# qiskit-community/aqc-research

Hardware: AMD Instinct MI355X
Metric: objective+gradient evals/sec (higher is better)
Workload: dtype f64; 1 GPU; 16-qubit, 40-block cx spin ansatz, state-vector objective+gradient; n_qubits=16, num_thetas=208, gate_groups=56, batch_per_gpu=1024, columns=1, transport=none, records_gathered=1024, launcher=none

## Files before the change

aqc_research_amd/_lib.py:

```python
import ctypes
import os
from ctypes import POINTER, c_char_p, c_double, c_float, c_int, c_int32, c_int64, c_uint8, c_void_p

import numpy as np

_HERE = os.path.dirname(os.path.abspath(__file__))
LIB_PATH = os.environ.get("AQC_HIP_LIB", os.path.join(_HERE, "libaqc_hip.so"))

BUF_Y, BUF_Z, BUF_X, BUF_W, BUF_ZW, BUF_X2 = range(6)
K_APPLY, K_SWEEP, K_COEF, K_FINALIZE, K_MISC, K_SWEEP_LIST, K_APPLY_LIST, K_PROJECT, K_SWEEP_VIRTUAL, K_APPLY_VIRTUAL = range(10)
ENTANGLERS = {"cx": 0, "cz": 1, "cp": 2}

_P = c_void_p
_D = POINTER(c_double)

SIGNATURES = {
    "aqc_version": (c_char_p, []),
    "aqc_last_error": (c_char_p, []),
    "aqc_device_count": (c_int, []),
    "aqc_live_buffers": (c_int, [POINTER(c_int64), POINTER(c_int64)]),
    "aqc_create": (c_int, [c_int, c_int, POINTER(c_int32), c_int, c_int, c_int, POINTER(_P)]),
    "aqc_destroy": (c_int, [_P]),
    "aqc_num_thetas": (c_int, [_P]),
    "aqc_num_gate_groups": (c_int, [_P]),
    "aqc_v_mul_vec": (c_int, [_P, _D, _D, _D]),
    "aqc_vdag_mul_vec": (c_int, [_P, _D, _D, _D]),
    "aqc_grad_dot_vec": (c_int, [_P, _D, _D, _D, c_int, c_int, c_int, _D]),
    "aqc_v_mul_mat": (c_int, [_P, _D, _D, c_int]),
    "aqc_vdag_mul_mat": (c_int, [_P, _D, _D, c_int]),
    "aqc_grad_dot_mat": (c_int, [_P, _D, _D, _D, c_int, _D]),
    "aqc_ws_create": (c_int, [_P, c_int, c_int, c_int, c_int, c_int, POINTER(_P)]),
    "aqc_ws_destroy": (c_int, [_P]),
    "aqc_ws_set_thetas": (c_int, [_P, _D]),
    "aqc_ws_upload": (c_int, [_P, c_int, _D]),
    "aqc_ws_upload_lane": (c_int, [_P, c_int, c_int, _D]),
    "aqc_ws_broadcast": (c_int, [_P, c_int, _D]),
    "aqc_ws_download": (c_int, [_P, c_int, _D]),
    "aqc_ws_download_lane": (c_int, [_P, c_int, c_int, _D]),
    "aqc_ws_copy_lane": (c_int, [_P, c_int, c_int, _P, c_int, c_int]),
    "aqc_ws_set_basis": (c_int, [_P, c_int, POINTER(c_int64)]),
    "aqc_ws_set_combo": (c_int, [_P, c_int, POINTER(c_int64), _D]),
    "aqc_ws_set_identity": (c_int, [_P, c_int]),
    "aqc_ws_apply": (c_int, [_P, c_int, c_int, c_int]),
    "aqc_ws_grad": (c_int, [_P, c_int, c_int, c_int]),
    "aqc_ws_get_grads": (c_int, [_P, _D]),
    "aqc_ws_gather": (c_int, [_P, c_int, POINTER(c_int64), c_int, _D]),
    "aqc_ws_vdot": (c_int, [_P, c_int, c_int, _D]),
    "aqc_ws_sync": (c_int, [_P]),
    "aqc_ws_eval": (c_int, [_P, _P, c_int, _P, c_int, c_int, c_int, c_int, _P]),
    "aqc_ws_grad_from": (c_int, [_P, c_int, c_int, c_int, c_int]),
    "aqc_ws_cd_sweep": (c_int, [_P, _D, _D]),
    "aqc_ws_cd_sweeps": (c_int, [_P, _D, _D, c_int, c_int]),
    "aqc_ws_cd_fits_one_launch": (c_int, [_P]),
    "aqc_ws_cd_minimize": (c_int, [_P, _D, c_int, c_int, c_double, c_double, c_double, c_int, c_int, _D, _D, POINTER(c_int64), POINTER(c_int32),
                           _D]),
    "aqc_zgemm": (c_int, [c_int, c_int, c_int, c_int, c_int, _D, c_int, _D, c_int, _D, c_int]),
    "aqc_gate_1q": (c_int, [c_int, c_int, c_int64, c_int, _D, _D, _D]),
    "aqc_gate_2q": (c_int, [c_int, c_int, c_int64, c_int, c_int, _D, _D, _D]),
    "aqc_xxz_mul_vec": (c_int, [c_int, c_int, c_int, c_double, _D, _D]),
    "aqc_xxz_energy": (c_int, [c_int, c_int, c_int, c_double, _D, _D]),
    "aqc_xxz_evolve": (c_int, [c_int, c_int, c_int, c_int, c_double, _D, _D, _D, POINTER(c_int32)]),
    "aqc_obs_plan": (c_int, [c_int, c_int, POINTER(c_int32), c_int, c_int] + [POINTER(c_int32)] * 6),
    "aqc_obs_rdm": (c_int, [c_int, c_int, c_int, _D, c_int, c_int, POINTER(c_int32), _D]),
    "aqc_mps_create": (c_int, [c_int, c_int, POINTER(c_int32), _D, _D, POINTER(_P)]),
    "aqc_mps_destroy": (c_int, [_P]),
    "aqc_mps_clone": (c_int, [_P, POINTER(_P)]),
    "aqc_mps_num_qubits": (c_int, [_P]),
    "aqc_mps_dims": (c_int, [_P, POINTER(c_int32)]),
    "aqc_mps_discarded_weight": (c_double, [_P]),
    "aqc_mps_export": (c_int, [_P, _D, _D]),
    "aqc_mps_gate1": (c_int, [_P, c_int, _D]),
    "aqc_mps_gate2": (c_int, [_P, c_int, c_int, _D, c_double, c_int]),
    "aqc_mps_dot": (c_int, [_P, _P, _D]),
    "aqc_mps_dot_ops": (c_int, [_P, _P, c_int, POINTER(c_int32), _D, _D]),
    "aqc_svd": (c_int, [c_int, c_int, c_int, _D, _D, _D, _D, POINTER(c_int)]),
    "aqc_svd_batch": (c_int, [c_int, c_int, c_int, c_int, POINTER(c_int32), POINTER(c_int32), _D, _D, _D, _D, POINTER(c_int32), POINTER(c_int32)]),
    "aqc_svd_batch_core_ms": (c_double, []),
    "aqc_mps_apply_circuit": (c_int, [_P, _P, _D, c_int, c_double, c_int]),
    "aqc_mps_fast_dot_gradient": (c_int, [_P, _P, _P, _D, c_double, c_int, c_int, c_int, c_int, _D]),
    "aqc_mpsb_create": (c_int, [c_int, c_int, c_int, POINTER(_P)]),
    "aqc_mpsb_destroy": (c_int, [_P]),
    "aqc_mpsb_gate2_stats": (c_int, [_P, c_int, _D, c_int]),
    "aqc_mpsb_set_targets": (c_int, [_P, POINTER(_P), c_int]),
    "aqc_mpsb_set_lhs": (c_int, [_P, POINTER(_P), c_int]),
    "aqc_mpsb_eval": (c_int, [_P, _P, _D, c_double, c_int, c_int, c_int, c_int, _D, _D, _D, POINTER(c_int32)]),
    "aqc_mpsb_set_lhs_basis": (c_int, [_P, POINTER(c_uint8)]),
    "aqc_mpsb_vh": (c_int, [_P, _P, _D, c_double, c_int, c_int, c_int, _D, _D, POINTER(c_int32)]),
    "aqc_mpsb_grad": (c_int, [_P, _P, c_int, c_int, c_int, _D]),
    "aqc_mpsb_set_bank": (c_int, [_P, POINTER(_P), c_int]),
    "aqc_mpsb_vh_bank": (c_int, [_P, _P, _D, c_double, c_int, c_int, c_int, _D, _D, POINTER(c_int32)]),
    "aqc_mpsb_gradient_of": (c_int, [_P, _P, _D, c_double, c_int, c_int, c_int, c_int, _D]),
    "aqc_mpsb_apply_circuit": (c_int, [_P, _P, _D, c_int, c_double, c_int, _D, POINTER(c_int32)]),
    "aqc_mpsb_export": (c_int, [_P, c_int, POINTER(_P)]),
    "aqc_mps_device": (c_int, [_P]),
    "aqc_gate_dot": (c_int, [c_int, c_int, c_int64, c_int, c_int, c_int, _D, _D, _D]),
    "aqc_ws_mps_upload": (c_int, [_P, c_int, POINTER(c_int32), _D, _D]),
    "aqc_ws_mps_to_vec": (c_int, [_P, c_int, c_int, c_int]),
    "aqc_ws_mps_to_vec_batch": (c_int, [_P, c_int, POINTER(c_int32), c_int, POINTER(c_int32)]),
    "aqc_ws_mps_dot": (c_int, [_P, c_int, c_int, _D]),
    "aqc_ws_theta_bank": (c_int, [_P, _D, c_int]),
    "aqc_ws_use_theta_set": (c_int, [_P, c_int]),
    "aqc_ws_gather_setup": (c_int, [_P, POINTER(c_int64), c_int]),
    "aqc_ws_gather_launch": (c_int, [_P, c_int]),
    "aqc_ws_gather_fetch": (c_int, [_P, _D]),
    "aqc_ws_vdot_launch": (c_int, [_P, c_int, c_int]),
    "aqc_ws_vdot_fetch": (c_int, [_P, _D]),
    "aqc_ws_results_async": (c_int, [_P]),
    "aqc_ws_objective_launch": (c_int, [_P, c_int, c_int, c_int, c_int]),
    "aqc_ws_results_fetch": (c_int, [_P, _D, _D]),
    "aqc_ws_timer_start": (c_int, [_P]),
    "aqc_ws_timer_stop": (c_int, [_P, POINTER(c_float)]),
    "aqc_ws_profile_enable": (c_int, [_P, c_int]),
    "aqc_ws_profile_get": (c_int, [_P, c_int, POINTER(c_int64), POINTER(c_double)]),
    "aqc_ws_profile_reset": (c_int, [_P]),
    "aqc_ws_profile_log": (c_int, [_P, POINTER(c_int32), _D, c_int, POINTER(c_int)]),
    "aqc_ws_plan_stage": (c_int, [_P, c_int, c_int, POINTER(c_int), POINTER(c_int), POINTER(c_int)]),
    "aqc_ws_sparse_counts": (c_int, [_P, POINTER(c_int64)]),
    "aqc_ws_projected_info": (c_int, [_P, POINTER(c_int32)]),
    "aqc_plan_projected": (c_int, [_P, c_int, c_int, POINTER(c_int32)]),
    "aqc_switch_info": (c_int, [c_int] + [POINTER(c_char_p)] * 5),
    "aqc_ws_switch": (c_int, [_P, c_char_p, POINTER(c_int64)]),
    "aqc_ws_plan_skips": (c_int, [_P, c_int, c_int, POINTER(c_int), c_int]),
    "aqc_ws_sweep_r_only_sub": (c_int, [_P]),
    "aqc_ws_plan_info": (c_int, [_P, c_int, POINTER(c_int), POINTER(c_int), POINTER(c_int)]),
    "aqc_ws_kernel_family": (c_int, [_P, c_int]),
    "aqc_ws_plan_substages": (c_int, [_P, c_int]),
    "aqc_ws_lbfgs": (c_int, [_P, _D, c_int, c_int, c_double, c_double, c_double, c_int, c_int, c_int, c_int, _D, _D, _D, POINTER(c_int64),
                     POINTER(c_int64), _D, POINTER(c_int64)]),
    "aqc_ws_lbfgs_mat": (c_int, [_P, _D, c_int, c_int, c_double, c_double, c_double, c_double, c_int, _D, _D, _D, POINTER(c_int64),
                         POINTER(c_int64), POINTER(c_int32)]),
    "aqc_ws_surrogate_eval": (c_int, [_P, _D, c_int, _D, POINTER(c_int64), c_int, c_int, c_int, _D, _D, _D, _D, _D]),
    "aqc_qr": (c_int, [c_int, c_int, c_int, _D, _D, POINTER(c_int32)]),
    "aqc_ws_sketch_target": (c_int, [_P, _D, c_int]),
    "aqc_ws_sketch_generate": (c_int, [_P, c_int, ctypes.c_uint64, c_int64, POINTER(c_int32), _D, POINTER(c_int32)]),
    "aqc_ws_sketch_draw": (c_int, [_P, c_int, ctypes.c_uint64, c_int64, c_int]),
    "aqc_ws_sketch_adam": (c_int, [_P, c_int, _D, c_int, _D, c_double, c_double, c_double, c_double, ctypes.c_uint64, c_int64, POINTER(c_int32),
                           POINTER(c_int32), _D, _D, _D, _D, POINTER(c_int64), POINTER(c_int32)]),
    "aqc_comm_unique_id": (c_int, [ctypes.c_char_p]),
    "aqc_comm_create": (c_int, [ctypes.c_char_p, c_int, c_int, c_int, POINTER(_P)]),
    "aqc_comm_destroy": (c_int, [_P]),
    "aqc_comm_rank": (c_int, [_P]),
    "aqc_comm_size": (c_int, [_P]),
    "aqc_comm_allgather": (c_int, [_P, _D, _D, ctypes.c_size_t]),
    "aqc_comm_allreduce": (c_int, [_P, _D, ctypes.c_size_t, c_int]),
    "aqc_comm_barrier": (c_int, [_P]),
    "aqc_plan_substages": (c_int, [_P, c_int, c_int, c_int, c_int, c_int, POINTER(c_int), POINTER(c_int), c_int]),
    "aqc_plan_query": (
        c_int,
        [_P, c_int, c_int, c_int, c_int, c_int, POINTER(c_int), POINTER(c_int), POINTER(c_int), POINTER(c_int), POINTER(c_int)],
    ),
}

_lib = None


def lib() -> ctypes.CDLL:
    global _lib
    if _lib is None:
        if not os.path.exists(LIB_PATH):
            raise RuntimeError(
                f"{LIB_PATH} not found: build it with `make -C aqc_research_amd/csrc` "
                "(or __graft_entry__.build()); this package has no CPU fallback"
            )
        handle = ctypes.CDLL(LIB_PATH)
        for name, (res, args) in SIGNATURES.items():
            fn = getattr(handle, name)
            fn.restype, fn.argtypes = res, args
        _lib = handle
    return _lib


LANES_REFUSED = 3
SKETCH_KINDS = {"rand": 0, "alt": 1, "eigen": 2}
QR_RANK_DEFICIENT = 1
CD_STATUS = {1: "normal", 2: "early", 3: "timeout"}
CD_ROUTES = {"auto": 0, "persistent": 1, "wide": 2}


class LanesRefused(RuntimeError):
    """The lockstep lanes of the MPS engine cannot do this call (a bond beyond their limit, a lane gone bad, no memory for them) and
    returned nothing; the single-lane engine may.  What callers that have such a route catch in order to take it."""


def check(status: int) -> None:
    if status != 0:
        kind = LanesRefused if status == LANES_REFUSED else RuntimeError
        raise kind("aqc_hip: " + lib().aqc_last_error().decode("utf-8", "replace"))


def dptr(arr: np.ndarray):
    return arr.ctypes.data_as(_D)


def as_c128(a, shape=None, name="array") -> np.ndarray:
    a = np.ascontiguousarray(a, dtype=np.complex128)
    if shape is not None and a.shape != tuple(shape):
        raise ValueError(f"{name}: expected shape {tuple(shape)}, got {a.shape}")
    return a


def as_f64(a, size=None, name="array") -> np.ndarray:
    a = np.ascontiguousarray(a, dtype=np.float64)
    if size is not None and a.size != size:
        raise ValueError(f"{name}: expected {size} values, got {a.size}")
    return a
```

aqc_research_amd/csrc/aqc_api.cpp:

```cpp
#include "aqc_ws.h"

using namespace aqc;

namespace {
thread_local std::string g_error;
}

namespace aqc {

int fail(const char* fmt, ...) {
    char buf[1024];
    va_list ap;
    va_start(ap, fmt);
    vsnprintf(buf, sizeof buf, fmt, ap);
    va_end(ap);
    g_error = buf;
    return 1;
}
int set_error(const std::string& msg) { g_error = msg; return 1; }

int check_buf(const aqc_ws* ws, int buf) {
    if (!ws) return fail("null workspace");
    if (buf < 0 || buf >= AQC_NUM_BUFS) return fail("invalid buffer id %d", buf);
    return 0;
}

int check_block_range(const aqc_ws* ws, int block_from, int block_to) {
    const int nb = ws->ctx->prog.num_blocks;
    if (block_from < 0 || nb == 0) return 0;
    if (!(block_from < block_to && block_to <= nb)) return fail("invalid block_range [%d, %d)", block_from, block_to);
    return 0;
}

int ensure_coef(aqc_ws* ws) {
    if (ws->coef_valid) return 0;
    return fail("thetas have not been uploaded (aqc_ws_set_thetas)");
}

int copy_in(aqc_ws* ws, double2* dst, const double* src, size_t rows) {
    if (ws->pitch == ws->ncols) {
        HIP_OK(hipMemcpyAsync(dst, src, rows * ws->ncols * sizeof(double2), hipMemcpyHostToDevice, ws->stream));
    } else {
        HIP_OK(hipMemsetAsync(dst, 0, rows * ws->pitch * sizeof(double2), ws->stream));
        HIP_OK(hipMemcpy2DAsync(dst, (size_t)ws->pitch * sizeof(double2), src, (size_t)ws->ncols * sizeof(double2),
                                (size_t)ws->ncols * sizeof(double2), rows, hipMemcpyHostToDevice, ws->stream));
    }
    HIP_OK(hipStreamSynchronize(ws->stream));
    return 0;
}
int copy_out(aqc_ws* ws, double* dst, const double2* src, size_t rows) {
    if (ws->pitch == ws->ncols) {
        HIP_OK(hipMemcpyAsync(dst, src, rows * ws->ncols * sizeof(double2), hipMemcpyDeviceToHost, ws->stream));
    } else {
        HIP_OK(hipMemcpy2DAsync(dst, (size_t)ws->ncols * sizeof(double2), src, (size_t)ws->pitch * sizeof(double2),
                                (size_t)ws->ncols * sizeof(double2), rows, hipMemcpyDeviceToHost, ws->stream));
    }
    HIP_OK(hipStreamSynchronize(ws->stream));
    return 0;
}

int results_guard(aqc_ws* ws) {
    if (ws->copy_pending && !ws->capturing) {
        HIP_OK(hipStreamWaitEvent(ws->stream, ws->ev_copied, 0));
        ws->copy_pending = false;
    }
    return 0;
}


}

extern "C" {

const char* aqc_version(void) { return "aqc_hip 0.1.0 (gfx950)"; }
const char* aqc_last_error(void) { return g_error.c_str(); }

int aqc_live_buffers(int64_t* device, int64_t* pinned) {
    if (device) *device = g_live_device.load();
    if (pinned) *pinned = g_live_pinned.load();
    return 0;
}

int aqc_device_count(void) {
    int ndev = 0;
    return hipGetDeviceCount(&ndev) == hipSuccess ? ndev : 0;
}

int aqc_create(int num_qubits, int entangler, const int32_t* blocks, int num_blocks, int trotter, int second_order,
               aqc_ctx** out) {
    if (!out) return fail("out pointer is null");
    *out = nullptr;
    aqc_ctx* ctx = new aqc_ctx();
    const std::string err = build_program(num_qubits, entangler, blocks, num_blocks, trotter != 0, second_order != 0, ctx->prog);
    if (!err.empty()) {
        delete ctx;
        return fail("%s", err.c_str());
    }
    *out = ctx;
    return 0;
}

int aqc_destroy(aqc_ctx* ctx) {
    if (!ctx) return 0;
    for (auto& kv : ctx->oneshot) aqc_ws_destroy(kv.second);
    delete ctx;
    return 0;
}

int aqc_num_thetas(const aqc_ctx* ctx) { return ctx ? ctx->prog.num_thetas() : -1; }
int aqc_num_gate_groups(const aqc_ctx* ctx) { return ctx ? (int)ctx->prog.groups.size() : -1; }

int aqc_plan_query(aqc_ctx* ctx, int ncols, int which, int tile_bits, int low_bits, int stage, int* num_stages,
                   int* bits_out, int* num_bits, int* ops_out, int* num_ops) {
    if (!ctx) return fail("null context");
    if (ncols < 1) return fail("ncols must be positive");
    const int col_bits = ceil_log2(ncols);
    if (tile_bits <= 0) tile_bits = which == 1 ? 12 : 13;
    if (low_bits < 0) low_bits = 3;
    Plan plan = make_plan(ctx->prog, col_bits, tile_bits, low_bits, which == 0);
    if (which == 3) {
        split_substages(ctx->prog, plan, 4, 1 << 20);
        plan = mirror_plan(plan);
    }
    const std::string err = check_plan(ctx->prog, plan);
    if (!err.empty()) return fail("planner produced an invalid plan: %s", err.c_str());
    if (num_stages) *num_stages = (int)plan.stages.size();
    if (stage >= 0) {
        if (stage >= (int)plan.stages.size()) return fail("stage index out of range");
        const Stage& st = plan.stages[stage];
        if (num_bits) *num_bits = (int)st.bits.size();
        if (num_ops) *num_ops = (int)st.ops.size();
        if (bits_out) for (size_t i = 0; i < st.bits.size(); ++i) bits_out[i] = st.bits[i];
        if (ops_out) for (size_t i = 0; i < st.ops.size(); ++i) ops_out[i] = st.ops[i];
    }
    return 0;
}

int aqc_plan_projected(aqc_ctx* ctx, int tile_bits, int low_bits, int32_t* info) {
    if (!ctx || !info) return fail("null argument");
    if (tile_bits <= 0) tile_bits = 12;
    if (low_bits < 0) low_bits = 3;
    const Program& prog = ctx->prog;
    tile_bits = std::min(std::max(tile_bits, 8), std::min(12, prog.n));
    aqc_ws tmp;
    tmp.ctx = ctx;
    tmp.ncols = 1; tmp.col_bits = 0; tmp.nbits = prog.n;
    Plan best = make_plan(prog, 0, tile_bits, low_bits, false);
    for (int lb = low_bits - 1; lb >= 2; --lb) {
        Plan cand = make_plan(prog, 0, tile_bits, lb, false);
        if (cand.stages.size() < best.stages.size()) best = cand;
    }
    lower_plan(prog, best, tmp.sweep, 4, true, true);
    tmp.sw = read_switches();
    tmp.sw.sparse_sweep = 1;
    tmp.inv_mirrored = tmp.sweep.v3 && tmp.sweep.plan.stages.size() >= 2;
    proj_plan(&tmp, low_bits);
    const int rc = aqc_ws_projected_info(&tmp, info);
    tmp.ctx = nullptr;
    return rc;
}

int aqc_plan_substages(aqc_ctx* ctx, int ncols, int which, int tile_bits, int low_bits, int stage, int* num_subs, int* subs_out, int max_subs) {
    if (!ctx || !num_subs) return fail("null argument");
    if (ncols < 1) return fail("ncols must be positive");
    const int col_bits = ceil_log2(ncols);
    if (tile_bits <= 0) tile_bits = 12;
    if (low_bits < 0) low_bits = 3;
    Plan plan = make_plan(ctx->prog, col_bits, tile_bits, low_bits, which == 0);
    split_substages(ctx->prog, plan, 4, 1 << 20);
    if (which == 3) plan = mirror_plan(plan);
    const std::string err = check_plan(ctx->prog, plan);
    if (!err.empty()) return fail("planner produced an invalid plan: %s", err.c_str());
    if (stage < 0 || stage >= (int)plan.stages.size()) return fail("stage index out of range");
    const Stage& st = plan.stages[stage];
    *num_subs = (int)st.subs.size();
    if (subs_out)
        for (int i = 0; i < (int)st.subs.size() && i < max_subs; ++i) {
            for (int j = 0; j < 4; ++j) subs_out[5 * i + j] = j < (int)st.subs[i].bits.size() ? st.subs[i].bits[j] : -1;
            subs_out[5 * i + 4] = (int)st.subs[i].ops.size();
        }
    return 0;
}


static int ws_decide(aqc_ws* ws, int tile_bits_apply, int tile_bits_sweep) {
    aqc_ctx* ctx = ws->ctx;
    const Program& prog = ctx->prog;
    const int batch = ws->batch;
    const Switches& sw = ws->sw = read_switches();
    const int low_bits = (int)sw.low_bits;
    int ka = tile_bits_apply > 0 ? tile_bits_apply : (int)sw.tile_bits_apply;
    int ks = tile_bits_sweep > 0 ? tile_bits_sweep : (int)sw.tile_bits_sweep;
    const int family = (int)sw.kernel_family;
    if (family < 0 || family > 3) return fail("AQC_KERNEL_FAMILY must be 1 (per-group), 2 (register-blocked) or 3 (matrix cores)");
    const bool want_v3 = (family == 3 || family == 0) && ws->nbits >= 8;
    const int force_v2 = family == 3 ? 0 : (family ? family - 1 : -1);
    const size_t big_tiles = (size_t)batch << std::max(0, ws->nbits - 12);
    const bool want_v2 = force_v2 >= 0 ? force_v2 != 0 : big_tiles >= 512;
    auto pick = [&](int kmax) {
        if (want_v3) {
            int k = std::min(12, ws->nbits);
            while (k > 10 && ((size_t)batch << (ws->nbits - k)) < 256) --k;
            const int kmin = std::max(8, prog.n + std::min(ws->col_bits, 3));
            while (ws->col_bits > 0 && k > kmin && ((size_t)batch << (ws->nbits - k)) < 256) --k;
            return k;
        }
        if (want_v2) return std::min(kmax, ws->nbits);
        int k = std::min(11, ws->nbits);
        while (k > 10 && ((size_t)batch << (ws->nbits - k)) < 512) --k;
        return k;
    };
    if (ka <= 0) ka = pick(13);
    if (ks <= 0) ks = pick(12);
    ka = std::min(std::min(ka, 13), ws->nbits);
    ks = std::min(std::min(ks, 12), ws->nbits);
    ws->threads = (int)sw.threads;
    if (ws->threads <= 0) ws->threads = std::min(256, std::max(64, 1 << (std::min(ka, ks) - 2)));
    if (ws->threads < 64 || ws->threads > 512 || ws->threads % 64) return fail("AQC_THREADS must be a multiple of 64 in [64, 512]");

    auto best_plan = [&](int k, bool inverse) {
        Plan best = make_plan(prog, ws->col_bits, k, low_bits, inverse);
        for (int lb = low_bits - 1; lb >= 2; --lb) {
            Plan cand = make_plan(prog, ws->col_bits, k, lb, inverse);
            if (cand.stages.size() < best.stages.size()) best = cand;
        }
        return best;
    };
    if (want_v3) { ka = std::min(std::max(ka, 8), 12); ks = std::max(ks, 8); }
    auto cached = [&](const std::vector<int>& key, DevPlan& out, const std::function<void(HostPlan&)>& lower) {
        std::lock_guard<std::recursive_mutex> lock(ctx->mu);
        auto it = ctx->plan_cache.find(key);
        if (it == ctx->plan_cache.end()) {
            HostPlan fresh;
            lower(fresh);
            it = ctx->plan_cache.emplace(key, std::move(fresh)).first;
        }
        out = it->second;
    };
    auto cached_plan = [&](int which, int k, bool inverse, int reg_bits, bool dots, DevPlan& out) {
        cached({which, ws->col_bits, k, low_bits, reg_bits, (int)dots, (int)want_v3}, out,
               [&](HostPlan& fresh) { lower_plan(prog, best_plan(k, inverse), fresh, reg_bits, dots, want_v3); });
    };
    cached_plan(2, ka, false, (want_v2 || want_v3) ? 4 : 0, false, ws->fwd);
    cached_plan(1, ks, false, want_v3 ? 4 : (want_v2 ? (sw.sweep_reg_bits == 3 ? 3 : 4) : 0), true, ws->sweep);
    ws->inv_mirrored = want_v3 && ka == ks && ws->sweep.v3 && ws->sweep.plan.stages.size() >= 2 && sw.mirror_plan != 0;
    if (ws->inv_mirrored)
        cached({3, ws->col_bits, ks, low_bits, 4, 0, 1}, ws->inv,
               [&](HostPlan& fresh) { lower_plan(prog, mirror_plan(ws->sweep.plan), fresh, 4, false, true, true); });
    else
        cached_plan(0, ka, true, (want_v2 || want_v3) ? 4 : 0, false, ws->inv);
    for (DevPlan* p : {&ws->fwd, &ws->inv, &ws->sweep}) {
        const std::string err = check_plan(prog, p->plan);
        if (!err.empty()) return fail("planner produced an invalid plan: %s", err.c_str());
    }
    proj_plan(ws, low_bits);
    if (sw.verbose && want_v3)
        fprintf(stderr, "aqc_hip: matrix-core kernels, tiles 2^%d (V / V^H, %d workgroups per CU) / 2^%d (sweep, %d per CU), sub-stages %zu / %zu / %zu\n",
                ws->inv.k, mfma_occupancy(ws->inv.k, false), ws->sweep.k, mfma_occupancy(ws->sweep.k, true), ws->fwd.h_subs3.size(),
                ws->inv.h_subs3.size(), ws->sweep.h_subs3.size());
    return 0;
}

struct SlotTables {
    std::vector<int> theta_slots, slot_theta, slot_ntiles;
    int partial_tiles = 1;
};
static SlotTables ws_slot_tables(aqc_ws* ws) {
    const Program& prog = ws->ctx->prog;
    const int T = prog.num_thetas();
    const int G = (int)prog.groups.size();
    ws->nslots = G * kSlotsPerGroup;
    SlotTables t;
    t.partial_tiles = ws->sweep.v3 ? 1 : ws->sweep.ntiles;
    t.theta_slots.assign(2 * (size_t)std::max(T, 1), -1);
    t.slot_ntiles.assign((size_t)std::max(ws->nslots, 1), t.partial_tiles);
    auto feed = [&](int theta, int slot) {
        if (t.theta_slots[2 * theta] < 0) t.theta_slots[2 * theta] = slot; else t.theta_slots[2 * theta + 1] = slot;
    };
    for (int gi = 0; gi < G; ++gi) {
        const GateGroup& g = prog.groups[gi];
        if (g.type == GROUP_FRONT) {
            feed(g.theta0 + 2, gi * kSlotsPerGroup + 0);
            feed(g.theta0 + 1, gi * kSlotsPerGroup + 1);
            feed(g.theta0 + 0, gi * kSlotsPerGroup + 2);
        } else {
            for (int d = 0; d < prog.tpb; ++d) feed(g.theta0 + d, gi * kSlotsPerGroup + d);
        }
    }
    t.slot_theta.assign((size_t)std::max(ws->nslots, 1), -1);
    ws->grads_direct = ws->sweep.v3 && T > 0 && ws->sw.grads_direct != 0;
    for (int th = 0; th < T; ++th) {
        if (t.theta_slots[2 * th] < 0 || t.theta_slots[2 * th + 1] >= 0) { ws->grads_direct = false; break; }
        t.slot_theta[t.theta_slots[2 * th]] = th;
    }
    return t;
}

static int ws_upload_ujobs(aqc_ws* ws) {
    const Program& prog = ws->ctx->prog;
    std::vector<UJob> jobs, route_jobs;
    size_t n_vdag_sweep = 0;
    DevPlan* vsw = ws->proj.ok ? &ws->proj.vsw : nullptr;
    const int nsw = ws->sweep.v3 ? (int)ws->sweep.h_subs3.size() : 0;
    ws->ujobs_mirror = ws->inv_mirrored && ws->inv.v3 && (int)ws->inv.h_subs3.size() == nsw && ws->sw.ubuild_mirror != 0;
    for (DevPlan* p : {&ws->inv, &ws->sweep, vsw, &ws->fwd})
        if (p && p->v3)
            for (size_t i = 0; i < p->h_subs3.size(); ++i) {
                if (p == &ws->inv && ws->ujobs_mirror) continue;
                UJob j{p->d_subs3 + i, p->d_grps, p->d_umat, (int)i, (int)p->h_subs3.size(), p->plan.inverse ? 1 : 0, prog.entangler, nullptr, 0, 0};
                if (p == &ws->sweep && ws->ujobs_mirror) { j.umat_mirror = ws->inv.d_umat; j.mirror_index = nsw - 1 - (int)i; j.mirror_nsubs = nsw; }
// ... 618 lines not shown
```

aqc_research_amd/csrc/aqc_kernels3.hip:

```cpp
#include <hip/hip_runtime.h>

#include <cstring>

#include <type_traits>

#include "aqc_device.h"
#include "aqc_launch.h"
#include "aqc_math.h"

namespace aqc {

typedef double double4_t __attribute__((ext_vector_type(4)));

__host__ __device__ __forceinline__ unsigned swz3(unsigned l) { return l ^ ((l >> 4) & 15u) ^ ((l >> 8) & 15u); }

__device__ __forceinline__ double4_t mfma(double a, double b, double4_t c) {
    return __builtin_amdgcn_mfma_f64_16x16x4f64(a, b, c, 0, 0, 0);
}

struct Acc3 { double4_t k1, k2, k3; };
__device__ __forceinline__ void u_mfma(const cplx (&v)[4], const double (&u0)[4], const double (&u1)[4], const double (&u2)[4], Acc3& t) {
    t.k1 = double4_t{0.0, 0.0, 0.0, 0.0}; t.k2 = t.k1; t.k3 = t.k1;
#pragma unroll
    for (int s = 0; s < 4; ++s) {
        t.k1 = mfma(v[s].x + v[s].y, u0[s], t.k1);
        t.k2 = mfma(v[s].x, u1[s], t.k2);
        t.k3 = mfma(v[s].y, u2[s], t.k3);
    }
}
__device__ __forceinline__ void u_combine(const Acc3& t, cplx (&o)[4]) {
#pragma unroll
    for (int r = 0; r < 4; ++r) {
        o[r].x = t.k1[r] - t.k3[r];
        o[r].y = t.k1[r] + t.k2[r];
    }
}

#ifdef AQC_TUNING
#define AQC_STAMP(slot) do { if (a.stamps && threadIdx.x == 0 && (slot) < kStampSlots) \
    a.stamps[((size_t)blockIdx.y * gridDim.x + blockIdx.x) * kStampSlots + (slot)] = __builtin_amdgcn_s_memtime(); } while (0)
#ifdef AQC_TUNING_NODBG
#define AQC_DBG_AND(x)
#define AQC_DBG_TEST(x) false
#else
#define AQC_DBG_AND(x) && (x)
#define AQC_DBG_TEST(x) (x)
#endif
#else
#define AQC_STAMP(slot) do { } while (0)
#define AQC_DBG_AND(x)
#define AQC_DBG_TEST(x) false
#endif

__host__ __device__ constexpr bool sweep_scratch_double(int k) { return k >= 12 || k <= 9; }
#ifndef AQC_SWEEP_SPREAD
#define AQC_SWEEP_SPREAD 1
#endif
#ifndef AQC_APPLY_SPREAD
#define AQC_APPLY_SPREAD 1
#endif
#ifndef AQC_EXP_APPLY_SKIP
#define AQC_EXP_APPLY_SKIP 0
#endif
constexpr int kApplySkip = AQC_EXP_APPLY_SKIP;
#ifndef AQC_EXP_SWEEP_SKIP
#define AQC_EXP_SWEEP_SKIP 0
#endif
constexpr int kSweepSkip = AQC_EXP_SWEEP_SKIP;
#ifndef AQC_EXP_UBUILD_SKIP
#define AQC_EXP_UBUILD_SKIP 0
#endif
constexpr int kUbuildSkip = AQC_EXP_UBUILD_SKIP;

constexpr int kSweepSpread = AQC_SWEEP_SPREAD, kApplySpread = AQC_APPLY_SPREAD;
template <int K, bool SWEEP = false> struct TileShape {
    static constexpr int kSweepWaves12 = 4;
    static constexpr int kWaves = (SWEEP && K == 12) ? kSweepWaves12 : (K >= 10 ? 4 : (1 << (K - 8)));
    static constexpr int kGroups = 1 << (K - 8);
    static constexpr int kGpw = kGroups / kWaves;
    static constexpr int kLoads = (1 << (K - 6)) / kWaves;
};

struct SubRegs {
    double u0[4], u1[4], u2[4];
    unsigned lane12;
};

template <int GPW>
__device__ __forceinline__ void fetch_sub(SubRegs& x, const DevSub3* subs, const double* umat, int sub_index, int lane, int wave,
                                          int nwaves) {
    const DevSub3* sub = subs + sub_index;
    const double* up = umat + (size_t)sub_index * 12 * 64;
#pragma unroll
    for (int s = 0; s < 4; ++s) {
        x.u0[s] = up[(0 * 4 + s) * 64 + lane];
        x.u1[s] = up[(1 * 4 + s) * 64 + lane];
        x.u2[s] = up[(2 * 4 + s) * 64 + lane];
    }
    x.lane12 = sub->lane12[lane];
}

template <int GPW>
struct SubAddr {
    unsigned a1, a2;
    unsigned k1[GPW][4], k2[GPW][4];
};
typedef unsigned uint8v_t __attribute__((ext_vector_type(8)));
template <int GPW>
__device__ __forceinline__ void fetch_k(SubAddr<GPW>& x, const DevSub3* subs, int sub_index, int wave, int nwaves) {
#pragma unroll
    for (int j = 0; j < GPW; ++j) {
        const uint8v_t kv = *reinterpret_cast<const __attribute__((address_space(4))) uint8v_t*>(
            (const __attribute__((address_space(4))) void*)(const void*)&subs[sub_index].kk[wave + j * nwaves][0]);
#pragma unroll
        for (int s = 0; s < 4; ++s) { x.k1[j][s] = kv[s]; x.k2[j][s] = kv[4 + s]; }
    }
}
template <int GPW>
__device__ __forceinline__ void sub_addr(SubAddr<GPW>& x, const SubRegs& c, unsigned lds_base) {
    x.a1 = ((c.lane12 & 0xffffu) << 4) + lds_base;
    x.a2 = ((c.lane12 >> 16) << 4) + lds_base;
}
typedef double dbl2_t __attribute__((ext_vector_type(2)));
typedef __attribute__((address_space(3))) dbl2_t* lds_cplx_ptr;
__device__ __forceinline__ cplx lds_get(unsigned addr) {
    const dbl2_t v = *reinterpret_cast<lds_cplx_ptr>(addr);
    return make_double2(v.x, v.y);
}
__device__ __forceinline__ void lds_put(unsigned addr, cplx v) { *reinterpret_cast<lds_cplx_ptr>(addr) = dbl2_t{v.x, v.y}; }
__device__ __forceinline__ unsigned lds_address(const void* p) {
    return (unsigned)reinterpret_cast<size_t>((__attribute__((address_space(3))) const char*)p);
}

__device__ __forceinline__ const void* uniform_ptr(const void* p) {
    const unsigned long long v = (unsigned long long)p;
    const unsigned lo = __builtin_amdgcn_readfirstlane((unsigned)v), hi = __builtin_amdgcn_readfirstlane((unsigned)(v >> 32));
    return (const void*)(((unsigned long long)hi << 32) | lo);
}

template <int K, int NV>
__device__ __forceinline__ void load_tiles3(cplx* t0, cplx* t1, const cplx* s0, const cplx* s1, const DevStage& st, unsigned lo, int wave) {
    constexpr int NL = TileShape<K, NV == 2>::kLoads, NW = TileShape<K, NV == 2>::kWaves;
    cplx v0[NL], v1[NL];
#pragma unroll
    for (int i = 0; i < NL; ++i) {
        const unsigned off = lo + st.dhi[wave + i * NW];
        v0[i] = s0[off];
        if (NV == 2) v1[i] = s1[off];
    }
#pragma unroll
    for (int i = 0; i < NL; ++i) {
        const unsigned slot = swz3((unsigned)((wave + i * NW) << 6) | (threadIdx.x & 63u));
        t0[slot] = v0[i];
        if (NV == 2) t1[slot] = v1[i];
    }
}
template <int K, bool SWEEP>
__device__ __forceinline__ void store_tile3(const cplx* tile, cplx* dst, const DevStage& st, unsigned lo, int wave) {
    constexpr int NL = TileShape<K, SWEEP>::kLoads, NW = TileShape<K, SWEEP>::kWaves;
#pragma unroll
    for (int i = 0; i < NL; ++i) {
        const unsigned slot = swz3((unsigned)((wave + i * NW) << 6) | (threadIdx.x & 63u));
        dst[lo + st.dhi[wave + i * NW]] = tile[slot];
    }
}
__device__ __forceinline__ size_t tile_base3(const DevStage& st, unsigned tile) {
    size_t base = 0;
    for (int i0 = 0; i0 < st.nub; i0 += 4) {
        int ub[4];
#pragma unroll
        for (int u = 0; u < 4; ++u) ub[u] = st.ubits[i0 + u];
#pragma unroll
        for (int u = 0; u < 4; ++u)
            if (i0 + u < st.nub) base |= (size_t)((tile >> (i0 + u)) & 1u) << ub[u];
    }
    return base;
}

__device__ __forceinline__ int uniform_load(const int* p) { return __builtin_amdgcn_readfirstlane(*p); }
struct ItemAt { int bl, tile, slot; };
template <bool LIST>
__device__ __forceinline__ ItemAt item_at(const Stage3Args& a, int wi) {
    if (LIST) {
        const TileItem* it = a.items + wi;
        return ItemAt{uniform_load(&it->lane), uniform_load(&it->tile), uniform_load(&it->slot)};
    }
    const int bl = wi / a.ntiles;
    return ItemAt{bl, wi - bl * a.ntiles, 0};
}
template <int K, bool LIST, bool PAIR = false>
__device__ __forceinline__ void apply_mfma_body(const Stage3Args& a0, const Stage3Args& b0, const int wg, const int nwg) {
    using TS = TileShape<K>;
    static_assert(!PAIR || (LIST && K >= 12), "the pair form walks two lists with persistent workgroups");
    extern __shared__ __attribute__((aligned(16))) char smem[];
    const Stage3Args* ca = &a0;
#define a (*ca)
#define st (ca->stage)
    cplx* tw = reinterpret_cast<cplx*>(smem);
    const unsigned lds_base = lds_address(smem);
    if (lds_base & ((16u << K) - 1)) __builtin_trap();
    const int lane = threadIdx.x & 63;
    const int wave = __builtin_amdgcn_readfirstlane((int)(threadIdx.x >> 6));
    constexpr int NL = TS::kLoads, NW = TS::kWaves;
    constexpr bool kPersist = K >= 12;
    int nwork = LIST ? uniform_load(a.nitems) : a.ntiles * a.batch;
    bool second = false;
    if (PAIR && wg >= nwork) { ca = &b0; second = true; nwork = uniform_load(b0.nitems); }
    unsigned lo = st.dlo[lane];
    unsigned lo16 = lo << 4;
    (void)lo16;
    SubRegs cur, nxt;
    SubAddr<TS::kGpw> ad;
    dbl2_t pw[NL];
    int wi = wg + ((kPersist || LIST) ? 0 : (int)blockIdx.y * a.ntiles);
    if (LIST && wi >= nwork) return;
    ItemAt it = item_at<LIST>(a, wi);
    {
        const int bl = it.bl;
        if (st.nsubs > 0) {
            fetch_sub<TS::kGpw>(cur, a.subs, a.umat + (size_t)bl * a.nsubs_total * 12 * 64, st.sub_begin, lane, wave, NW);
            fetch_k<TS::kGpw>(ad, a.subs, st.sub_begin, wave, NW);
        }
        AQC_STAMP(0);
        if (!(kApplySkip & 64)) load_tiles3<K, 1>(tw, nullptr, a.in0 + (size_t)bl * a.lane_stride + tile_base3(st, it.tile), nullptr, st, lo, wave);
    }
    __builtin_amdgcn_s_waitcnt(0x0F70);
    AQC_STAMP(1);
    for (;;) {
    const int bl = it.bl;
    const size_t lane_off = (size_t)bl * a.lane_stride + tile_base3(st, it.tile);
    const double* umat = a.umat + (size_t)bl * a.nsubs_total * 12 * 64;
    int nwi = wi + nwg;
    bool more = kPersist && st.nsubs > 0 && nwi < nwork;
    const Stage3Args* na = ca;
    int nnwork = nwork;
    if (PAIR && !more && !second) {
        na = &b0; nwi = wg; nnwork = uniform_load(b0.nitems);
        more = nwi < nnwork;
    }
    const bool change = PAIR && na != ca;
    const ItemAt nit = more ? item_at<LIST>(*na, nwi) : ItemAt{0, 0, 0};
    const int nbl = nit.bl;
    const size_t next_off = more ? (size_t)nbl * na->lane_stride + tile_base3(na->stage, nit.tile) : 0;
    const unsigned nlo = change ? na->stage.dlo[lane] : lo;
    const unsigned nlo16 = nlo << 4;
    for (int si = 0; si < st.nsubs; ++si) {
        AQC_STAMP(4 + si);
        if (!(kApplySkip & 512)) __syncthreads();
        if (si + 1 < st.nsubs) fetch_sub<TS::kGpw>(nxt, a.subs, umat, st.sub_begin + si + 1, lane, wave, NW);
        else if (more) fetch_sub<TS::kGpw>(nxt, na->subs, na->umat + (size_t)nbl * na->nsubs_total * 12 * 64, na->stage.sub_begin, lane, wave, NW);
        if (kPersist && more && !(kApplySkip & 64)) {
#pragma unroll
            for (int c = 0; c < 4; ++c) {
                if (si == (c < st.nsubs ? c : st.nsubs - 1)) {
#pragma unroll
                    for (int i = c * (NL / 4); i < (c + 1) * (NL / 4); ++i) {
                        const size_t ub = next_off + na->stage.dhi[wave + i * NW];
                        asm volatile("s_nop 4\n\tglobal_load_dwordx4 %0, %1, %2" : "=a"(pw[i]) : "v"(nlo16), "s"(uniform_ptr(na->in0 + ub)) : "memory");
                    }
                }
            }
        }
        sub_addr(ad, cur, lds_base);
        cplx v[2][4];
        Acc3 acc;
#pragma unroll
        for (int s = 0; s < 4; ++s) v[0][s] = lds_get(ad.a1 ^ ad.k1[0][s]);
#pragma unroll
        for (int j = 0; j <= TS::kGpw; ++j) {
            if (j + 1 < TS::kGpw && !(kApplySkip & 2)) {
#pragma unroll
                for (int s = 0; s < 4; ++s) v[(j + 1) & 1][s] = lds_get((kApplySkip & 32) ? ad.a1 : (ad.a1 ^ ad.k1[j + 1][s]));
            }
            __builtin_amdgcn_sched_barrier(0);
            double sv[4];
            cplx o[4];
            if (j < TS::kGpw) {
#pragma unroll
                for (int s = 0; s < 4; ++s) sv[s] = (kApplySkip & (16 | 128)) ? v[j & 1][s].x : v[j & 1][s].x + v[j & 1][s].y;
            }
            if (j > 0) {
                if (kApplySkip & (16 | 256)) {
#pragma unroll
                    for (int r = 0; r < 4; ++r) o[r] = make_double2(acc.k1[r], acc.k2[r]);
                } else u_combine(acc, o);
            }
            unsigned wa[4];
            if (j < TS::kGpw) {
#pragma unroll
                for (int s = 0; s < 4; ++s) asm volatile("" : "+v"(sv[s]));
            }
            if (j > 0) {
#pragma unroll
                for (int r = 0; r < 4; ++r) { wa[r] = (kApplySkip & 32) ? ad.a2 : (ad.a2 ^ ad.k2[j - 1][r]); asm volatile("" : "+v"(wa[r])); }
            }
            __builtin_amdgcn_sched_barrier(0);
            if (j < TS::kGpw) {
                acc.k1 = double4_t{0.0, 0.0, 0.0, 0.0}; acc.k2 = acc.k1; acc.k3 = acc.k1;
#pragma unroll
                for (int s = 0; s < 4; ++s) {
                    if (kApplySkip & 8) continue;
                    acc.k1 = mfma(sv[s], cur.u0[s], acc.k1);
                    acc.k2 = mfma(v[j & 1][s].x, cur.u1[s], acc.k2);
                    acc.k3 = mfma(v[j & 1][s].y, cur.u2[s], acc.k3);
                }
            }
            if (j > 0 && !(kApplySkip & 1)) {
#pragma unroll
                for (int r = 0; r < 4; ++r) lds_put(wa[r], o[r]);
                if (j < TS::kGpw) {
#pragma unroll
                    for (int i = 0; i < 4; ++i) {
                        __builtin_amdgcn_sched_group_barrier(0x008, kApplySpread, 0);
                        __builtin_amdgcn_sched_group_barrier(0x200, 1, 0);
                    }
                }
            }
            __builtin_amdgcn_sched_barrier(0);
        }
        if (si + 1 < st.nsubs || more) {
            cur = nxt;
            if (si + 1 < st.nsubs) fetch_k<TS::kGpw>(ad, a.subs, st.sub_begin + si + 1, wave, NW);
            else fetch_k<TS::kGpw>(ad, na->subs, na->stage.sub_begin, wave, NW);
        }
    }
    AQC_STAMP(4 + st.nsubs);
    __syncthreads();
    AQC_STAMP(2);
    if (!(kApplySkip & 64)) store_tile3<K, false>(tw, a.out0 + lane_off, st, lo, wave);
    AQC_STAMP(3);
    if (!more) break;
    __syncthreads();
    __builtin_amdgcn_s_waitcnt(0x0F70);
#pragma unroll
    for (int i = 0; i < NL; ++i) {
        const unsigned slot = swz3((unsigned)((wave + i * NW) << 6) | (threadIdx.x & 63u));
        asm volatile("ds_write_b128 %0, %1" : : "v"(lds_base + (slot << 4)), "a"(pw[i]) : "memory");
    }
    __builtin_amdgcn_s_waitcnt(0xC07F);
    wi = nwi;
    it = nit;
    if (PAIR) { ca = na; second = second || change; nwork = nnwork; lo = nlo; lo16 = nlo16; }
    }
#undef a
#undef st
}
template <int K, bool LIST = false>
__global__ __launch_bounds__(TileShape<K>::kWaves * 64, 2) void apply_mfma_kernel(const Stage3Args a) {
    apply_mfma_body<K, LIST>(a, a, (int)blockIdx.x, (int)gridDim.x);
}
#ifndef AQC_PAIR_PLAIN_BOUNDARY
#define AQC_PAIR_PLAIN_BOUNDARY 0
#endif
template <int K>
__global__ __launch_bounds__(TileShape<K>::kWaves * 64, 2) void apply_pair_kernel(const Stage3Args a, const Stage3Args b, const int grid_a) {
    if constexpr (K >= 12 && !AQC_PAIR_PLAIN_BOUNDARY) {
        static_assert(sizeof(Stage3Args) % 8 == 0 && alignof(Stage3Args) == 8, "b follows a in the kernel-argument segment without padding");
        const __attribute__((address_space(4))) char* kp = (const __attribute__((address_space(4))) char*)__builtin_amdgcn_kernarg_segment_ptr();
        const Stage3Args* pa = (const Stage3Args*)(const void*)kp;
        const Stage3Args* pb = (const Stage3Args*)(const void*)(kp + sizeof(Stage3Args));
        apply_mfma_body<K, true, true>(*pa, *pb, (int)blockIdx.x, (int)gridDim.x);
    } else if (K >= 12) {
        apply_mfma_body<K, true>(a, a, (int)blockIdx.x, (int)gridDim.x);
        __syncthreads();
        apply_mfma_body<K, true>(b, b, (int)blockIdx.x, (int)gridDim.x);
    } else if ((int)blockIdx.x < grid_a) {
        apply_mfma_body<K, true>(a, a, (int)blockIdx.x, grid_a);
    } else {
        apply_mfma_body<K, true>(b, b, (int)blockIdx.x - grid_a, (int)gridDim.x - grid_a);
    }
}

template <int N>
__device__ __forceinline__ void wait_prefetched(dbl2_t (&pw)[N], dbl2_t (&pz)[N]) {
    asm volatile("s_waitcnt vmcnt(0)" : : : "memory");
#pragma unroll
    for (int i = 0; i < N; ++i) asm volatile("" : "+a"(pw[i]), "+a"(pz[i]));
}
__device__ __forceinline__ unsigned tile_offset3(const DevStage& st, unsigned local) { return st.dlo[local & 63u] | st.dhi[local >> 6]; }
template <int K> struct SweepShape : TileShape<K, true> {};
__device__ __forceinline__ unsigned elem_bit(const DevStage& st, long long e, unsigned local_pos) {
    const unsigned m = local_pos < 6 ? st.dlo[1u << local_pos] : st.dhi[1u << (local_pos - 6)];
    return ((unsigned long long)e & m) ? 1u : 0u;
}
template <int GPW, int NW>
__device__ __forceinline__ void skip_masks(const DevStage& st, unsigned info, long long e0, long long e1, int wave, unsigned& nzmask, unsigned& kneed) {
    nzmask = 0; kneed = 0;
    const unsigned gfresh = info & 15u, kfresh = (info >> 6) & 3u;
#pragma unroll
    for (int k = 0; k < 2; ++k) {
        const long long e = k ? e1 : e0;
        if (e < 0) continue;
        unsigned gb = 0;
#pragma unroll
        for (int i = 0; i < 4; ++i)
            if (gfresh >> i & 1) gb |= elem_bit(st, e, (info >> (8 + 4 * i)) & 15u) << i;
        unsigned kb = 0;
        if (kfresh & 1) kb |= elem_bit(st, e, (info >> 24) & 15u);
        if (kfresh & 2) kb |= elem_bit(st, e, (info >> 28) & 15u) << 1;
#pragma unroll
        for (int j = 0; j < GPW; ++j)
            if ((((unsigned)(wave + j * NW) ^ gb) & gfresh) == 0) nzmask |= 1u << j;
#pragma unroll
        for (unsigned s2 = 0; s2 < 4; ++s2)
            if (((s2 ^ kb) & kfresh) == 0) kneed |= 1u << s2;
    }
}
template <int K, bool LIST, bool SKIPW, bool RLAST>
__device__ __forceinline__ void sweep_mfma_body(const Stage3Args& a, const int wg, const int nwg) {
    using TS = TileShape<K, true>;
    constexpr int kSlots = TS::kWaves > 4 ? 4 : TS::kWaves;
    constexpr unsigned tsize = 1u << K;
    extern __shared__ __attribute__((aligned(16))) char smem[];
    const DevStage& st = a.stage;
    cplx* tw = reinterpret_cast<cplx*>(smem);
    cplx* tz = tw + tsize;
    cplx* scratch = tz + tsize;
    constexpr bool kDouble = sweep_scratch_double(K);
    const unsigned lds_base = lds_address(smem);
    if (lds_base & ((32u << K) - 1)) __builtin_trap();
    const int lane = threadIdx.x & 63;
    const int wave = __builtin_amdgcn_readfirstlane((int)(threadIdx.x >> 6));
    constexpr bool kPersist = K >= 12;
    constexpr int NL = TS::kLoads, NW = TS::kWaves;
    const int nwork = LIST ? uniform_load(a.nitems) : a.ntiles * a.batch;
    const unsigned lo = st.dlo[lane];
    SubRegs cur, nxt;
    SubAddr<TS::kGpw> ad;
    dbl2_t pw[NL], pz[NL];
    unsigned parity = 0;
    AQC_STAMP(0);
    const int chunk = kPersist ? (LIST ? (nwork + nwg - 1) / nwg : a.chunk) : 0;
    const int wi_first = kPersist ? wg * chunk : wg;
    const int wi_end = kPersist ? (wi_first + chunk < nwork ? wi_first + chunk : nwork) : wi_first + 1;
    int wi = wi_first;
    if (wi >= nwork) return;
    const unsigned e16 = threadIdx.x << 4;
    dbl2_t racc;
    static_assert(!kPersist || NL == 4 * TS::kGpw, "the prefetch registers are the first sub-stage's operands");
    const bool reg_first = kPersist && st.nsubs > 0;
    unsigned flo16 = 0;
    ItemAt it = item_at<LIST>(a, wi);
    size_t item_off = (size_t)it.bl * a.lane_stride + tile_base3(st, it.tile);
    {
        const size_t off0 = item_off;
        if (st.nsubs > 0) {
            fetch_sub<TS::kGpw>(cur, a.subs, a.umat + (size_t)it.bl * a.nsubs_total * 12 * 64, st.sub_begin, lane, wave, NW);
            fetch_k<TS::kGpw>(ad, a.subs, st.sub_begin, wave, NW);
        }
        if (reg_first) {
            flo16 = tile_offset3(st, swz3(cur.lane12 & 0xffffu)) << 4;
#pragma unroll
            for (int i = 0; i < ((kSweepSkip & 64) ? 0 : NL); ++i) {
                const size_t ub = off0 + a.first_hi[wave + (i / 4) * NW][i % 4];
                asm volatile("s_nop 4\n\tglobal_load_dwordx4 %0, %1, %2" : "=a"(pw[i]) : "v"(flo16), "s"(uniform_ptr(a.in0 + ub)) : "memory");
                asm volatile("s_nop 4\n\tglobal_load_dwordx4 %0, %1, %2" : "=a"(pz[i]) : "v"(flo16), "s"(uniform_ptr(a.in1 + ub)) : "memory");
            }
        } else {
            load_tiles3<K, 2>(tw, tz, a.in0 + off0, a.in1 + off0, st, lo, wave);
        }
    }
    __builtin_amdgcn_s_waitcnt(0x0F70);
    if (reg_first) wait_prefetched<NL>(pw, pz);
    __syncthreads();
    AQC_STAMP(1);
    for (;;) {
    const int bl = it.bl, tile = it.tile;
    const size_t lane_off = item_off;
    long long se0 = -1, se1 = -1;
    if (SKIPW) {
        const unsigned long long toff = (unsigned long long)tile_base3(st, tile);
        const long long c0 = a.supp[2 * (size_t)bl], c1 = a.supp[2 * (size_t)bl + 1];
        const unsigned lo0 = __builtin_amdgcn_readfirstlane((unsigned)c0), hi0 = __builtin_amdgcn_readfirstlane((unsigned)(c0 >> 32));
        const unsigned lo1 = __builtin_amdgcn_readfirstlane((unsigned)c1), hi1 = __builtin_amdgcn_readfirstlane((unsigned)(c1 >> 32));
        const long long u0 = (long long)(((unsigned long long)hi0 << 32) | lo0), u1 = (long long)(((unsigned long long)hi1 << 32) | lo1);
        if (u0 >= 0 && (((unsigned long long)u0 ^ toff) & st.fresh_nonlocal) == 0) se0 = u0;
        if (u1 >= 0 && (((unsigned long long)u1 ^ toff) & st.fresh_nonlocal) == 0) se1 = u1;
    }
    const double* umat = a.umat + (size_t)bl * a.nsubs_total * 12 * 64;
    const int part = LIST ? it.slot : (kPersist ? wg - (bl * a.ntiles) / chunk : tile);
    const bool seg_first = LIST || !kPersist || wi == wi_first || tile == 0;
    cplx* rpart = a.rpart + (((size_t)bl * a.nsubs_total + st.sub_begin) * a.nparts + part) * 256;
    const int nwi = wi + 1;
    const bool more = reg_first && nwi < wi_end;
    const ItemAt nit = more ? item_at<LIST>(a, nwi) : ItemAt{0, 0, 0};
    const int nbl = nit.bl;
    const size_t next_off = more ? (size_t)nbl * a.lane_stride + tile_base3(st, nit.tile) : 0;
    constexpr unsigned ZOFF = tsize * 16;
    cplx vw[2][4], vz[2][4];
    constexpr bool kEarly = K >= 11;
    if (reg_first) {
        sub_addr(ad, cur, lds_base);
#pragma unroll
        for (int s = 0; s < 4; ++s) { vw[0][s] = make_double2(pw[s].x, pw[s].y); vz[0][s] = make_double2(pz[s].x, pz[s].y); }
    } else if (kEarly && st.nsubs > 0) {
        sub_addr(ad, cur, lds_base);
#pragma unroll
        for (int s = 0; s < 4; ++s) { vw[0][s] = lds_get(ad.a1 ^ ad.k1[0][s]); vz[0][s] = lds_get((ad.a1 | ZOFF) ^ ad.k1[0][s]); }
    }
    auto prefetch = [&](int c) __attribute__((always_inline)) {
#pragma unroll
        for (int i = 0; i < ((kSweepSkip & 64) ? 0 : NL); ++i)
            if (i / (NL / 4) == c) {
                const size_t ub = next_off + a.first_hi[wave + (i / 4) * NW][i % 4];
                asm volatile("s_nop 4\n\tglobal_load_dwordx4 %0, %1, %2" : "=a"(pw[i]) : "v"(flo16), "s"(uniform_ptr(a.in0 + ub)) : "memory");
                asm volatile("s_nop 4\n\tglobal_load_dwordx4 %0, %1, %2" : "=a"(pz[i]) : "v"(flo16), "s"(uniform_ptr(a.in1 + ub)) : "memory");
            }
    };
    const int nmain = RLAST && a.r_only_last && st.nsubs >= 1 && !(kPersist && st.nsubs == 1) ? st.nsubs - 1 : st.nsubs;
    if (!RLAST) {
        for (int si = 0; si < st.nsubs; ++si) {
#define AQC_SS_FROM_REGS (reg_first && si == 0)
#define AQC_SS_RONLY false
#include "aqc_sweep_substage.inc"
#undef AQC_SS_FROM_REGS
#undef AQC_SS_RONLY
        }
    } else {
        if (nmain > 0) {
            const int si = 0;
#define AQC_SS_FROM_REGS reg_first
#define AQC_SS_RONLY false
#include "aqc_sweep_substage.inc"
#undef AQC_SS_FROM_REGS
#undef AQC_SS_RONLY
        }
        for (int si = 1; si < nmain; ++si) {
#define AQC_SS_FROM_REGS false
#define AQC_SS_RONLY false
#include "aqc_sweep_substage.inc"
#undef AQC_SS_FROM_REGS
#undef AQC_SS_RONLY
        }
        if (nmain < st.nsubs) {
            const int si = nmain;
#define AQC_SS_FROM_REGS false
#define AQC_SS_RONLY true
#include "aqc_sweep_substage.inc"
#undef AQC_SS_FROM_REGS
#undef AQC_SS_RONLY
        }
    }
    AQC_STAMP(kStampSlots - 2);
    if (more) wait_prefetched<NL>(pw, pz);
    if (!(kSweepSkip & 64)) {
        if (a.store_out & 1) store_tile3<K, true>(tw, a.out0 + lane_off, st, lo, wave);
        if (a.store_out & 2) store_tile3<K, true>(tz, a.out1 + lane_off, st, lo, wave);
    }
    AQC_STAMP(kStampSlots - 1);
    if (!more) break;
    AQC_STAMP(kStampSlots - 6);
    __syncthreads();
    AQC_STAMP(kStampSlots - 5);
    wi = nwi;
    it = nit;
    item_off = next_off;
    }
    AQC_STAMP(kStampSlots - 4);
}
template <int K, bool LIST = false, bool SKIPW = false, bool RLAST = false>
// ... 285 lines not shown
        for (int s2 = 0; s2 < 4; ++s2) {
            const double re = up[(0 * 4 + s2) * 64 + lane], im = up[(1 * 4 + s2) * 64 + lane] + re;
            Us[(lane & 15) * 16 + 4 * s2 + (lane >> 4)] = make_double2(re, im);
        }
        __syncthreads();
        const int i0 = lane & 15, j0 = lane >> 4;
        cplx acc[4];
#pragma unroll
        for (int m = 0; m < 4; ++m) {
            const int j = j0 + 4 * m;
            double re = 0.0, im = 0.0;
            for (int k = 0; k < 16; ++k) {
                const cplx u = Us[j * 16 + k], r = R[k * 17 + i0];
                re += u.x * r.x - u.y * r.y; im += u.x * r.y + u.y * r.x;
            }
            acc[m] = make_double2(re, im);
        }
        __syncthreads();
#pragma unroll
        for (int m = 0; m < 4; ++m) R[(j0 + 4 * m) * 17 + i0] = acc[m];
        __syncthreads();
#pragma unroll
        for (int m = 0; m < 4; ++m) {
            const int j = j0 + 4 * m;
            double re = 0.0, im = 0.0;
            for (int k = 0; k < 16; ++k) {
                const cplx t = R[j * 17 + k], u = Us[i0 * 16 + k];
                re += t.x * u.x + t.y * u.y; im += t.y * u.x - t.x * u.y;
            }
            acc[m] = make_double2(re, im);
        }
        __syncthreads();
#pragma unroll
        for (int m = 0; m < 4; ++m) R[(j0 + 4 * m) * 17 + i0] = acc[m];
        __syncthreads();
    }
    RG_STAMP(1);
    cplx* out = partial + (size_t)b * nslots;
    auto put = [&](int slot, cplx v) {
        out[slot] = v;
        if (slot_theta) {
            const int t = slot_theta[slot];
            if (t >= 0) {
                grads[(size_t)b * T + t] = v;
                if (mirror) mirror[(size_t)b * T + t] = v;
            }
        }
    };
    const int lo = lane & 15, hi = lane >> 4;
    for (int top = sub.ngrp; top > 0; top -= kGrpChunk) {
        const int base = max(0, top - kGrpChunk), count = top - base;
        __syncthreads();
        if (WAVES == 1 || top != sub.ngrp) stage_groups(gm, grps, sub.grp_begin + base, count, th, ent, lane);
        __syncthreads();
        RG_STAMP(2);
        for (int i = count - 1; i >= 0; --i) {
            const Gm& g = gm[i];
            {
                const int a = lane >> 4, bb = (lane >> 2) & 3, o = lane & 3;
                cplx v = R[grp_index(g, a, o) * 17 + grp_index(g, bb, o)];
                v.x += dpp_mov<0xB1, 0xf>(v.x); v.y += dpp_mov<0xB1, 0xf>(v.y);
                v.x += dpp_mov<0x4E, 0xf>(v.x); v.y += dpp_mov<0x4E, 0xf>(v.y);
                if (o == 0) rho_s[i][a * 4 + bb] = v;
            }
            cplx x[4];
            int idx[4];
#pragma unroll
            for (int l = 0; l < 4; ++l) { idx[l] = grp_index(g, l, hi) * 17 + lo; x[l] = R[idx[l]]; }
            grp_apply<1>(g, ent, x);
#pragma unroll
            for (int l = 0; l < 4; ++l) R[idx[l]] = x[l];
            __syncthreads();
#pragma unroll
            for (int l = 0; l < 4; ++l) { idx[l] = lo * 17 + grp_index(g, l, hi); x[l] = R[idx[l]]; }
            grp_apply<2>(g, ent, x);
#pragma unroll
            for (int l = 0; l < 4; ++l) R[idx[l]] = x[l];
            __syncthreads();
        }
        RG_STAMP(3);
        if (lane < count) {
            const Gm& g = gm[lane];
            const bool on = g.jblock < 0 ? (front != 0) : (g.jblock >= from && g.jblock < to);
            if (on && g.slot0 >= 0) {
                cplx rho[16];
#pragma unroll
                for (int e = 0; e < 16; ++e) rho[e] = rho_s[lane][e];
                if (g.type == 0) {
                    put(g.slot0 + 2, rho_dot<1>(rho, MOP_RZ));
                    rho_unapply<1>(rho, MOP_RZ, g.rc[0], g.rs[0]);
                    put(g.slot0 + 1, rho_dot<1>(rho, MOP_RY));
                    rho_unapply<1>(rho, MOP_RY, g.rc[1], g.rs[1]);
                    put(g.slot0 + 0, rho_dot<1>(rho, MOP_RZ));
                } else {
                    const int ks = ent == 0 ? MOP_RX : MOP_RZ;
                    if (g.flags & 2) rho_unapply<0>(rho, MOP_RZ, kR, kR);
                    put(g.slot0 + 3, rho_dot<0>(rho, ks));
                    rho_unapply<0>(rho, ks, g.rc[3], g.rs[3]);
                    put(g.slot0 + 2, rho_dot<0>(rho, MOP_RY));
                    put(g.slot0 + 1, rho_dot<1>(rho, MOP_RZ));
                    rho_unapply<1>(rho, MOP_RZ, g.rc[1], g.rs[1]);
                    put(g.slot0 + 0, rho_dot<1>(rho, MOP_RY));
                    if (ent == 2) {
                        rho_unapply<0>(rho, MOP_RY, g.rc[2], g.rs[2]);
                        rho_unapply<1>(rho, MOP_RY, g.rc[0], g.rs[0]);
                        put(g.slot0 + 4, make_double2(rho[15].y, -rho[15].x));
                    }
                }
            } else if (slot_theta && g.slot0 >= 0) {
                for (int k = 0; k < 5; ++k) put(g.slot0 + k, make_double2(0.0, 0.0));
            }
        }
        RG_STAMP(4);
    }
}
#ifdef AQC_TUNING
void rgrad_print_stamps(int nsubs) {
    unsigned long long h[32 * 8];
    if (hipMemcpyFromSymbol(h, HIP_SYMBOL(g_rgrad_stamps), sizeof h) != hipSuccess) return;
    double a = 0, b = 0, c = 0, d = 0;
    const int n = nsubs < 32 ? nsubs : 32;
    for (int i = 0; i < n; ++i) { a += h[i * 8 + 1] - h[i * 8]; b += h[i * 8 + 2] - h[i * 8 + 1]; c += h[i * 8 + 3] - h[i * 8 + 2]; d += h[i * 8 + 4] - h[i * 8 + 3]; }
    fprintf(stderr, "aqc_hip stamps: gradient walk (lane 0, %d sub-stages): tile sum %.0f + group decode %.0f + R walk %.0f + rho walk %.0f cycles\n", n, a / n, b / n, c / n, d / n);
}
#endif

void stage3_first_offsets(Stage3Args& a, const DevSub3& first_sub) {
    for (int g = 0; g < 16; ++g)
        for (int s = 0; s < 4; ++s) {
            const unsigned local = swz3(first_sub.kk[g][s] >> 4);
            a.first_hi[g][s] = a.stage.dlo[local & 63u] | a.stage.dhi[local >> 6];
        }
}

int mfma_threads(int k, bool sweep) { return (sweep && k == 12) ? 64 * SweepShape<12>::kWaves : 64 * std::min(4, 1 << std::max(0, k - 8)); }
size_t apply3_lds_bytes(int k) { return (size_t)16 << k; }
size_t sweep3_lds_bytes(int k) {
    return ((size_t)32 << k) + (size_t)(sweep_scratch_double(k) ? 2 : 1) * std::min(4, mfma_threads(k, true) / 64) * 256 * sizeof(cplx);
}

template <typename F>
static hipError_t with_tile_size(int k, F&& f) {
    switch (k) {
        case 8: return f(std::integral_constant<int, 8>{});
        case 9: return f(std::integral_constant<int, 9>{});
        case 10: return f(std::integral_constant<int, 10>{});
        case 11: return f(std::integral_constant<int, 11>{});
        case 12: return f(std::integral_constant<int, 12>{});
        default: return hipErrorInvalidValue;
    }
}
using Stage3Kernel = void (*)(Stage3Args);
using Pair3Kernel = void (*)(Stage3Args, Stage3Args, int);
template <int K> static Stage3Kernel apply_variant(bool list) { return list ? apply_mfma_kernel<K, true> : apply_mfma_kernel<K, false>; }
template <int K> static Stage3Kernel sweep_variant(bool list, bool skipw, bool rlast) {
    if (list) return rlast ? sweep_mfma_kernel<K, true, false, true> : sweep_mfma_kernel<K, true, false, false>;
    if (skipw) return sweep_mfma_kernel<K, false, true, false>;
    return rlast ? sweep_mfma_kernel<K, false, false, true> : sweep_mfma_kernel<K, false, false, false>;
}
template <int K> static Pair3Kernel apply_pair_variant() { return apply_pair_kernel<K>; }
template <int K> static Pair3Kernel sweep_pair_variant(bool rlast_a) { return rlast_a ? sweep_pair_kernel<K, true, false> : sweep_pair_kernel<K, false, false>; }

template <typename F>
static hipError_t big_lds(F kernel) {
    return hipFuncSetAttribute(reinterpret_cast<const void*>(kernel), hipFuncAttributeMaxDynamicSharedMemorySize, 160 * 1024);
}
hipError_t init_kernels3() {
    hipError_t e = hipSuccess;
    for (int k = 8; k <= 12 && e == hipSuccess; ++k)
        e = with_tile_size(k, [](auto kk) {
            constexpr int K = decltype(kk)::value;
            hipError_t e = big_lds(apply_pair_variant<K>());
            for (int f = 0; f < 2 && e == hipSuccess; ++f) e = big_lds(apply_variant<K>(f));
            for (int f = 0; f < 2 && e == hipSuccess; ++f) e = big_lds(sweep_pair_variant<K>(f));
            for (int f = 0; f < 8 && e == hipSuccess; ++f) e = big_lds(sweep_variant<K>(f & 1, f & 2, f & 4));
            return e;
        });
    return e;
}
template <typename... Args>
static hipError_t launch3(void (*kernel)(Args...), dim3 grid, int k, bool sweep, hipStream_t s, const Args&... args) {
    kernel<<<grid, mfma_threads(k, sweep), sweep ? sweep3_lds_bytes(k) : apply3_lds_bytes(k), s>>>(args...);
    return hipGetLastError();
}
int mfma_occupancy(int k, bool sweep) {
    int n = 0;
    const hipError_t e = with_tile_size(k, [&](auto kk) {
        constexpr int K = decltype(kk)::value;
        return sweep ? hipOccupancyMaxActiveBlocksPerMultiprocessor(&n, sweep_variant<K>(false, false, false), mfma_threads(k, true), sweep3_lds_bytes(k))
                     : hipOccupancyMaxActiveBlocksPerMultiprocessor(&n, apply_variant<K>(false), mfma_threads(k, false), apply3_lds_bytes(k));
    });
    return e == hipSuccess ? n : -1;
}
static long persistent_sweep_grid(long sweep_grid) {
    if (sweep_grid > 0) return sweep_grid;
    static int cus[64] = {0};
    int dev = 0;
    if (hipGetDevice(&dev) != hipSuccess || dev < 0 || dev >= 64) return 256;
    if (cus[dev] == 0) {
        int n = 0;
        cus[dev] = (hipDeviceGetAttribute(&n, hipDeviceAttributeMultiprocessorCount, dev) == hipSuccess && n > 0) ? n : 256;
    }
    return cus[dev];
}
static bool stage3_launchable(int k, const Stage3Args& a, bool need_list, bool need_subs) {
    if (a.items ? (!a.nitems || a.max_items < 1) : need_list) return false;
    if (k < 12) return true;
    if (need_subs && a.stage.nsubs <= 0) return false;
    for (int l = 0; l < 64; ++l)
        if (a.stage.dlo[l] >= (1u << 28)) return false;
    return true;
}
hipError_t launch_apply3(int k, hipStream_t s, const Stage3Args& a, const Switches& sw) {
    const bool list = a.items != nullptr;
    const long persist = sw.apply_persist;
    if (!stage3_launchable(k, a, false, list) || (list && k >= 12 && persist <= 0)) return hipErrorInvalidValue;
    const long nwork = list ? (long)a.max_items : (long)a.ntiles * a.batch;
    const dim3 grid = (k >= 12 && persist > 0 && a.stage.nsubs > 0) ? dim3((unsigned)std::min<long>(nwork, persist * persistent_sweep_grid(sw.sweep_grid)))
                                                                     : ((k >= 12 || list) ? dim3((unsigned)nwork) : dim3(a.ntiles, a.batch));
    return with_tile_size(k, [&](auto kk) { return launch3(apply_variant<decltype(kk)::value>(list), grid, k, false, s, a); });
}
static_assert(2 * sizeof(Stage3Args) + 16 <= 3840, "two argument blocks must fit the kernel-argument segment");
hipError_t launch_apply3_pair(int k, hipStream_t s, const Stage3Args& a, const Stage3Args& b, const Switches& sw) {
    const long persist = sw.apply_persist;
    if (!stage3_launchable(k, a, true, true) || !stage3_launchable(k, b, true, true) || (k >= 12 && persist <= 0)) return hipErrorInvalidValue;
    const long longer = std::max(a.max_items, b.max_items);
    const dim3 grid((unsigned)(k >= 12 ? std::min<long>(longer, persist * persistent_sweep_grid(sw.sweep_grid)) : (long)a.max_items + b.max_items));
    return with_tile_size(k, [&](auto kk) { return launch3(apply_pair_variant<decltype(kk)::value>(), grid, k, false, s, a, b, a.max_items); });
}
int sweep3_chunk(int ntiles, int batch, int k, long sweep_grid) {
    if (k < 12) return 0;
    const long nwork = (long)ntiles * batch, g = std::min<long>(nwork, persistent_sweep_grid(sweep_grid));
    return (int)((nwork + g - 1) / g);
}
int sweep3_nparts(int ntiles, int batch, int k, long sweep_grid) {
    const int chunk = sweep3_chunk(ntiles, batch, k, sweep_grid);
    return chunk > 0 ? std::min(ntiles, (ntiles + chunk - 1) / chunk + 1) : ntiles;
}
hipError_t launch_sweep3(int k, hipStream_t s, const Stage3Args& a, const Switches& sw) {
    const bool list = a.items != nullptr;
    if (!stage3_launchable(k, a, false, true)) return hipErrorInvalidValue;
    if (a.nparts < 1 || (!list && (a.nparts != sweep3_nparts(a.ntiles, a.batch, k, sw.sweep_grid) || a.chunk != sweep3_chunk(a.ntiles, a.batch, k, sw.sweep_grid)))) return hipErrorInvalidValue;
    const long nwork = list ? (long)a.max_items : (long)a.ntiles * a.batch;
    const dim3 grid((unsigned)(k >= 12 ? (list ? std::min<long>(nwork, persistent_sweep_grid(sw.sweep_grid)) : (nwork + a.chunk - 1) / a.chunk) : nwork));
    const bool skipw = !list && a.supp != nullptr;
    const bool rlast = !skipw && a.r_only_last != 0;
    return with_tile_size(k, [&](auto kk) { return launch3(sweep_variant<decltype(kk)::value>(list, skipw, rlast), grid, k, true, s, a); });
}

hipError_t launch_sweep3_pair(int k, hipStream_t s, const Stage3Args& a, const Stage3Args& b, const Switches& sw) {
    if (!stage3_launchable(k, a, true, true) || !stage3_launchable(k, b, true, true)) return hipErrorInvalidValue;
    if (a.nparts < 1 || b.nparts < 1 || a.supp || b.supp || b.r_only_last) return hipErrorInvalidValue;
    const long longer = std::max(a.max_items, b.max_items);
    const dim3 grid((unsigned)(k >= 12 ? std::min<long>(longer, persistent_sweep_grid(sw.sweep_grid)) : (long)a.max_items + b.max_items));
    return with_tile_size(k, [&](auto kk) { return launch3(sweep_pair_variant<decltype(kk)::value>(a.r_only_last != 0), grid, k, true, s, a, b, a.max_items); });
}

__device__ __forceinline__ int tile_of_elem(const DevStage& st, long long e) {
    int t = 0;
    for (int i = 0; i < st.nub; ++i) t |= (int)((e >> st.ubits[i]) & 1) << i;
    return t;
}
__device__ __forceinline__ int lane_tiles(const DevStage& st, const long long* supp, int per_lane, const long long* extra, int nextra, int b,
                                          int (&tiles)[kMaxTileCands]) {
    int n = 0;
    auto add = [&](long long e) {
        if (e < 0) return;
        const int t = tile_of_elem(st, e);
        for (int i = 0; i < n; ++i)
            if (tiles[i] == t) return;
        tiles[n++] = t;
    };
    for (int k = 0; supp && k < per_lane; ++k) add(supp[(size_t)b * per_lane + k]);
    for (int k = 0; extra && k < nextra; ++k) add(extra[k]);
    return n;
}
__global__ __launch_bounds__(1024) void tile_items_kernel(const DevStage st, const long long* supp, int per_lane, const long long* extra, int nextra,
                                                          int batch, TileItem* items, int* nitems, int* lane_parts, int* prev_tiles,
                                                          TileItem* clear_items, int* nclear) {
    __shared__ int scan_a[1024], scan_b[1024];
    const int tid = threadIdx.x, per = (batch + 1023) / 1024;
    const int b0 = tid * per, b1 = min(batch, b0 + per);
    int tiles[kMaxTileCands];
    int mine = 0, mine_clear = 0;
    for (int b = b0; b < b1; ++b) {
        const int n = lane_tiles(st, supp, per_lane, extra, nextra, b, tiles);
        mine += n;
        if (prev_tiles)
            for (int k = 0; k < 2; ++k) {
                const int pt = prev_tiles[2 * b + k];
                bool stale = pt >= 0;
                for (int i = 0; i < n; ++i) stale = stale && tiles[i] != pt;
                mine_clear += stale ? 1 : 0;
            }
    }
    scan_a[tid] = mine; scan_b[tid] = mine_clear;
    __syncthreads();
    for (int d = 1; d < 1024; d <<= 1) {
        const int va = tid >= d ? scan_a[tid - d] : 0, vb = tid >= d ? scan_b[tid - d] : 0;
        __syncthreads();
        scan_a[tid] += va; scan_b[tid] += vb;
        __syncthreads();
    }
    int at = scan_a[tid] - mine, at_clear = scan_b[tid] - mine_clear;
    if (tid == 1023) { *nitems = scan_a[tid]; if (nclear) *nclear = scan_b[tid]; }
    for (int b = b0; b < b1; ++b) {
        const int n = lane_tiles(st, supp, per_lane, extra, nextra, b, tiles);
        if (lane_parts) lane_parts[b] = n;
        if (prev_tiles) {
            for (int k = 0; k < 2; ++k) {
                const int pt = prev_tiles[2 * b + k];
                bool stale = pt >= 0;
                for (int i = 0; i < n; ++i) stale = stale && tiles[i] != pt;
                if (stale) clear_items[at_clear++] = TileItem{b, pt, 0, 0};
            }
            prev_tiles[2 * b] = n > 0 ? tiles[0] : -1;
            prev_tiles[2 * b + 1] = n > 1 ? tiles[1] : -1;
        }
        for (int i = 0; i < n; ++i) items[at++] = TileItem{b, tiles[i], i, 0};
    }
}
hipError_t launch_tile_items(const DevStage& stage, const long long* supp, int per_lane, const long long* extra, int nextra, int batch,
                             TileItem* items, int* nitems, int* lane_parts, int* prev_tiles, TileItem* clear_items, int* nclear, hipStream_t s) {
    if ((supp ? per_lane : 0) + (extra ? nextra : 0) > kMaxTileCands || batch < 1) return hipErrorInvalidValue;
    if (prev_tiles && ((supp ? per_lane : 0) > 2 || (extra && nextra > 0) || !clear_items || !nclear)) return hipErrorInvalidValue;
    tile_items_kernel<<<1, 1024, 0, s>>>(stage, supp, per_lane, extra, nextra, batch, items, nitems, lane_parts, prev_tiles, clear_items, nclear);
    return hipGetLastError();
}
__global__ __launch_bounds__(256) void clear_tiles_kernel(const DevStage st, cplx* buf, size_t lane_stride, const TileItem* clear_items, const int* nclear) {
    if ((int)blockIdx.x >= *nclear) return;
    const TileItem it = clear_items[blockIdx.x];
    cplx* dst = buf + (size_t)it.lane * lane_stride + tile_base3(st, (unsigned)it.tile);
    for (unsigned l = threadIdx.x; l < (1u << st.k); l += 256) dst[tile_offset3(st, l)] = make_double2(0.0, 0.0);
}
hipError_t launch_clear_tiles(const DevStage& stage, void* buf, size_t lane_stride, const TileItem* clear_items, const int* nclear, int max_items,
                              hipStream_t s) {
    if (max_items < 1) return hipSuccess;
    clear_tiles_kernel<<<max_items, 256, 0, s>>>(stage, static_cast<cplx*>(buf), lane_stride, clear_items, nclear);
    return hipGetLastError();
}
hipError_t launch_ubuild(const UJob* jobs, int njobs, const double* thetas, int T, int batch, hipStream_t s, double* thetas_copy) {
    if (njobs < 1) return hipSuccess;
    ubuild_kernel<<<dim3(njobs, batch), 64, 0, s>>>(jobs, thetas, T, thetas_copy);
    return hipGetLastError();
}
hipError_t launch_rgrad(const DevSub3* subs, const DevGrp* grps, int entangler, const double* thetas, int T, const void* rpart,
                        int ntiles, int nsubs_total, void* partial, int nslots, int from, int to, int front, int batch, hipStream_t s,
                        const int* slot_theta, void* grads, void* mirror, GatherJob gather, int nparts, int chunk, int sparse_subs,
                        const int* lane_parts, int conj_sub, const double* umat, int nsubs_run, const RgradSecond* second_plan) {
    if (nsubs_total < 1) return hipSuccess;
    if (nsubs_run < 0 || nsubs_run > nsubs_total) nsubs_run = nsubs_total;
    RgradSecond second;
    memset(&second, 0, sizeof second);
    if (second_plan) second = *second_plan;
    const int extra = (gather.count > 0 && gather.buf ? 1 : 0) + second.count;
    if (nsubs_run + extra < 1) return hipSuccess;
    const int tiles_per_lane = ntiles;
    if (nparts <= 0) nparts = ntiles;
    ntiles = nparts;
    if (nparts >= 32 && second.count == 0)
        rgrad_kernel<4><<<dim3(nsubs_run + extra, batch), 256, 0, s>>>(subs, grps, entangler, thetas, T, static_cast<const cplx*>(rpart), ntiles,
                                                                  nsubs_total, static_cast<cplx*>(partial), nslots, from, to, front, slot_theta,
                                                                  static_cast<cplx*>(grads), static_cast<cplx*>(mirror), gather, tiles_per_lane, chunk, sparse_subs, lane_parts, conj_sub, umat, nsubs_run, second);
    else
        rgrad_kernel<1><<<dim3(nsubs_run + extra, batch), 64, 0, s>>>(subs, grps, entangler, thetas, T, static_cast<const cplx*>(rpart), ntiles,
                                                                 nsubs_total, static_cast<cplx*>(partial), nslots, from, to, front, slot_theta,
                                                                 static_cast<cplx*>(grads), static_cast<cplx*>(mirror), gather, tiles_per_lane, chunk, sparse_subs, lane_parts, conj_sub, umat, nsubs_run, second);
    return hipGetLastError();
}

}
```

aqc_research_amd/csrc/aqc_launch.h:

```cpp
#pragma once
#include <string>
#include <hip/hip_runtime.h>

#include <algorithm>
#include <cstddef>

#include "aqc_device.h"
#include "aqc_mps_walk.h"
#include "aqc_switches.h"

namespace aqc {

struct StageArgs {
    const DevStage* stage;
    const DevOp* ops;
    const DevSub* subs;
    const DevMop* mops;
    const double* coef;
    int ncoef;
    const double2* in0;
    const double2* in1;
    double2* out0;
    double2* out1;
    size_t lane_stride;
    double2* partial;
    int nslots, ntiles_max;
    int from, to, front;
    int final_stage;
    int debug;
};

size_t apply_lds_bytes(int k);
size_t sweep_lds_bytes(int k, int threads);
hipError_t init_kernels();
hipError_t launch_apply(int ent, bool inverse, int ntiles, int batch, int threads, int k, hipStream_t s, const StageArgs& a);
hipError_t launch_sweep(int ent, int ntiles, int batch, int threads, int k, hipStream_t s, const StageArgs& a);
hipError_t launch_coef(const double* thetas, double* coef, int n, int nblocks, int tpb, int tail, int batch, hipStream_t s);
hipError_t launch_finalize(const void* partial, const int* theta_slots, const int* slot_ntiles, void* grads, int T,
                           int nslots, int ntiles_max, int n, int tpb, int from, int to, int front, int batch,
                           hipStream_t s, void* mirror = nullptr);
hipError_t launch_scatter_one(void* buf, size_t lane_stride, int batch, const long long* elem, hipStream_t s);
hipError_t launch_scatter_two(void* buf, size_t lane_stride, int batch, const long long* elem, const void* coef, long long* prev, hipStream_t s);
hipError_t launch_set_identity(void* buf, size_t lane_stride, int dim, int pitch, int batch, hipStream_t s);
hipError_t launch_gather(const void* buf, size_t lane_stride, const long long* elem, int count, int batch, void* out,
                         hipStream_t s, void* mirror = nullptr);
hipError_t launch_vdot(const void* a, const void* b, size_t lane_stride, size_t count, int batch, void* part, int nparts,
                       void* out, hipStream_t s);

hipError_t init_kernels2();
hipError_t launch_apply2(int ent, int ntiles, int batch, int k, hipStream_t s, const StageArgs& a);
hipError_t launch_sweep2(int ent, int ntiles, int batch, int k, int reg_bits, hipStream_t s, const StageArgs& a);

struct TileItem { int lane, tile, slot, pad; };
struct Stage3Args {
    DevStage stage;
    const DevSub3* subs;
    const double* umat;
    int nsubs_total;
    const double2* in0;
    const double2* in1;
    double2* out0;
    double2* out1;
    size_t lane_stride;
    double2* rpart;
    int ntiles;
    int batch;
    int chunk, nparts;
    int store_out;
    int r_only_last;
    const long long* supp;
    const TileItem* items;
    const int* nitems;
    int max_items;
    unsigned first_hi[16][4];
    int debug;
    unsigned long long* stamps;
};
constexpr int kStampSlots = 40;
void stage3_first_offsets(Stage3Args& a, const DevSub3& first_sub);
hipError_t init_kernels3();
int mfma_threads(int k, bool sweep);
int mfma_occupancy(int k, bool sweep);
hipError_t launch_apply3(int k, hipStream_t s, const Stage3Args& a, const Switches& sw);
hipError_t launch_sweep3(int k, hipStream_t s, const Stage3Args& a, const Switches& sw);
hipError_t launch_apply3_pair(int k, hipStream_t s, const Stage3Args& a, const Stage3Args& b, const Switches& sw);
hipError_t launch_sweep3_pair(int k, hipStream_t s, const Stage3Args& a, const Stage3Args& b, const Switches& sw);
void rgrad_print_stamps(int nsubs);
int sweep3_chunk(int ntiles, int batch, int k, long sweep_grid);
int sweep3_nparts(int ntiles, int batch, int k, long sweep_grid);
struct ProjMap { const unsigned* tab; int shift; };
struct ProjArgs {
    const double2* y;
    const double2* s;
    double2* out;
    int s_virtual, out_virtual;
    int staged;
    int keep_bits, k_bits, cb;
    ProjMap y_keep, y_k, s_k, s_c, o_keep, o_c;
    size_t lane_stride;
    const TileItem* items;
    const int* nitems;
    const int* lane_parts;
    int nub0, ubits0[32];
    unsigned ff_mask, cb_mask, tf_mask;
    int nvp;
    const unsigned* off_t;
    const unsigned* off_cb;
    const unsigned* it_of_c;
    const unsigned* off_us;
    int us_bits;
    size_t part_stride;
    double2* cpart;
    int cpart_shares;
    int t, ntiles_v;
    double2* vm;
    TileItem* vitems;
    int* vcount;
    int* vlane_parts;
    int batch;
};
hipError_t launch_project_init(const ProjArgs& a, hipStream_t s);
hipError_t launch_project_fused(const ProjArgs& a, const void* mend, void* ctile, void* yout, hipStream_t s, int qb);
hipError_t launch_project_amps(const ProjArgs& a, const long long* gather, int ngather, const long long* supp, void* small, const void* vy, const void* z,
                               hipStream_t s);
hipError_t launch_project(const ProjArgs& a, hipStream_t s);
struct UJob {
    const DevSub3* sub;
    const DevGrp* grps;
    double* umat;
    int index, nsubs;
    int inverse, entangler;
    double* umat_mirror;
    int mirror_index, mirror_nsubs;
};
hipError_t launch_ubuild(const UJob* jobs, int njobs, const double* thetas, int T, int batch, hipStream_t s, double* thetas_copy = nullptr);
struct GatherJob {
    const void* buf; size_t lane_stride; const long long* elem; int count; void* out; void* mirror;
};
struct RgradSecond {
    const DevSub3* subs;
    const DevGrp* grps;
    const double2* rpart;
    const int* lane_parts;
    const double* umat;
    int nparts, nsubs_total, count;
};
hipError_t launch_rgrad(const DevSub3* subs, const DevGrp* grps, int entangler, const double* thetas, int T, const void* rpart,
                        int ntiles, int nsubs_total, void* partial, int nslots, int from, int to, int front, int batch, hipStream_t s,
                        const int* slot_theta = nullptr, void* grads = nullptr, void* mirror = nullptr,
                        GatherJob gather = GatherJob{nullptr, 0, nullptr, 0, nullptr, nullptr},
                        int nparts = 0, int chunk = 0,
                        int sparse_subs = 0, const int* lane_parts = nullptr,
                        int conj_sub = -1, const double* umat = nullptr,
                        int nsubs_run = -1,
                        const RgradSecond* second_plan = nullptr);
constexpr int kMaxTileCands = 72;
hipError_t launch_tile_items(const DevStage& stage, const long long* supp, int per_lane, const long long* extra, int nextra, int batch,
                             TileItem* items, int* nitems, int* lane_parts, int* prev_tiles, TileItem* clear_items, int* nclear, hipStream_t s);
hipError_t launch_clear_tiles(const DevStage& stage, void* buf, size_t lane_stride, const TileItem* clear_items, const int* nclear, int max_items,
                              hipStream_t s);

struct LbState {
    int B, T, S, memory;
    double *x, *g, *f;
    double *d, *slope, *step;
    double *x_new;
    double *Smem, *Ymem, *rho;
    int *active, *done;
    long long* nit;
    double *weight, *fidelity;
    int* max_no;
    double2 *cur_hs, *cur_g0;
    double2 *acc_hs, *acc_g0;
};
hipError_t lb_prepare(const LbState& st, const void* hs, int update, double* f_out, void* raw_hs, void* x2, size_t lane_stride,
                      const long long* index, long long* prev, hipStream_t s);
hipError_t lb_take(const LbState& st, const void* grads, double* g_out, void* raw_g, hipStream_t s);
hipError_t lb_probe(const LbState& st, const void* hs, int* flags, hipStream_t s);
hipError_t lb_commit0(const LbState& st, const void* hs, const void* raw_g, double* f_out, double* g_out, hipStream_t s);
hipError_t lb_active(const LbState& st, double gtol, double fid_thr, int* flags, hipStream_t s);
hipError_t lb_direction(const LbState& st, int count, hipStream_t s);
hipError_t lb_trial(const LbState& st, double* thetas, hipStream_t s);
hipError_t lb_armijo(const LbState& st, double c1, const double* thetas, const double* ft, const void* raw_hs_t, const void* raw_g0_t,
                     int* flags, hipStream_t s);
hipError_t lb_copy_raw(const LbState& st, hipStream_t s);
hipError_t lb_history(const LbState& st, int count, double ftol, const double* f_acc, const double* g_acc, hipStream_t s);
struct LbMat {
    int k;
    double gtol, fobj_thr, fid_thr;
    double *gmax;
    double *ft, *gt, *gmax_t, *fid_t;
    double *f_acc, *g_acc, *gmax_acc, *fid_acc;
    int* status;
    int* flags;
};
enum { kLbNotDone = 1, kLbAnyActive = 2 };
enum { kLbNonFinite = 1 };
hipError_t lb_mat_value(const LbState& st, const LbMat& m, const void* trace, const void* grads, int init, hipStream_t s);
hipError_t lb_mat_direction(const LbState& st, const LbMat& m, int count, hipStream_t s);
hipError_t lb_mat_armijo(const LbState& st, const LbMat& m, double c1, const double* thetas, hipStream_t s);
hipError_t lb_mat_history(const LbState& st, const LbMat& m, int count, double ftol, int last, hipStream_t s);

hipError_t launch_mps_scale(void* g, const double* lam, int rows, int cols, hipStream_t s);
hipError_t launch_zgemm(bool conj_t, bool accum, int M, int N, int K, const void* A, int lda, const void* B, int ldb,
                        void* C, int ldc, hipStream_t s);
hipError_t launch_zgemm_bh(bool conj_t, bool accum, int M, int N, int K, const void* A, int lda, const void* B, int ldb,
                           void* C, int ldc, hipStream_t s);
hipError_t launch_mps_env_dot(const void* e, const void* rc, size_t count, void* out, hipStream_t s);
hipError_t launch_zgemm_batched(bool conj_t, bool accum, int M, int N, int K, const void* A, int lda, const void* B, int ldb,
                                void* C, int ldc, size_t stride_a, size_t stride_b, size_t stride_c, int nbatch, hipStream_t s);
hipError_t launch_zgemm_tables(int M, int N, int K, const void* const* a_tab, int lda, const void* const* b_tab, int ldb, void* const* c_tab, int ldc,
                               size_t stride_a, size_t stride_b, size_t stride_c, int outer, int inner, hipStream_t s, int b_transposed = 0);
hipError_t launch_mps_product(const void* const* t_tab, void* const* out_tab, int n, int count, hipStream_t s);
struct MpsSites {
    int n;
    size_t total;
    size_t offset[65];
    int lam_offset[64];
    int cols[64];
};
hipError_t launch_mps_scale_all(void* t, const double* lam, const MpsSites& sites, hipStream_t s);

struct CdSegHost { int32_t ha, hb, ent, nrot, kind[4], on_b[4], tindex[4]; };
// ... 162 lines not shown
```

aqc_research_amd/csrc/aqc_ws.h:

```cpp
#pragma once
#include <hip/hip_runtime_api.h>

#include <cmath>
#include <cstdarg>
#include <cstdio>
#include <cstdlib>
#include <cstring>
#include <functional>
#include <initializer_list>
#include <map>
#include <memory>
#include <mutex>
#include <string>
#include <type_traits>
#include <vector>

#include "../../include/aqc_hip.h"
#include "aqc_devbuf.h"
#include "aqc_device.h"
#include "aqc_launch.h"
#include "aqc_plan.h"

namespace aqc {

int fail(const char* fmt, ...) __attribute__((format(printf, 1, 2)));

#define HIP_OK(expr)                                                                              \
    do {                                                                                          \
        hipError_t e_ = (expr);                                                                   \
        if (e_ != hipSuccess) return ::aqc::fail("%s failed: %s (%s:%d)", #expr, hipGetErrorString(e_), __FILE__, __LINE__); \
    } while (0)

inline int ceil_log2(int v) {
    int b = 0;
    while ((1 << b) < v) ++b;
    return b;
}

enum ULevel { kUNone = 0, kURoute = 1, kUAll = 2 };

struct HostPlan {
    Plan plan;
    std::vector<DevStage> h_stages;
    std::vector<DevOp> h_ops;
    std::vector<DevSub> h_subs;
    std::vector<DevMop> h_mops;
    int k = 0, ntiles = 0, reg_bits = 0;
    bool v2 = false;
    bool v3 = false;
    std::vector<DevSub3> h_subs3;
    std::vector<DevGrp> h_grps;
    int family() const { return v3 ? 3 : (v2 ? 2 : 1); }
};
static_assert(std::is_copy_constructible<HostPlan>::value && std::is_copy_assignable<HostPlan>::value,
              "a cached plan is copied out of the cache: it owns no device memory (a buffer member would make it move-only)");

struct DevPlan : HostPlan {
    DevBuf<DevStage> d_stages;
    DevBuf<DevOp> d_ops;
    DevBuf<DevSub> d_subs;
    DevBuf<DevMop> d_mops;
    DevBuf<DevSub3> d_subs3;
    DevBuf<DevGrp> d_grps;
    DevBuf<double> d_umat;
    DevBuf<double2> d_rpart;
    int u_level = kUNone;
    DevPlan& operator=(const HostPlan& host) { HostPlan::operator=(host); return *this; }
};

struct ListKey {
    static constexpr int kUnknown = -2, kGatherOnly = -1;
    int buf = kUnknown;
    unsigned long long supp = 0, gather = 0;
    bool operator==(const ListKey& o) const { return buf != kUnknown && buf == o.buf && supp == o.supp && gather == o.gather; }
};

struct EvalRoute {
    int x_buf = AQC_BUF_X;
    bool vdag = false;
    bool new_thetas = false;
    bool gather = false;
    bool gather_rides = false;
    bool grads = false;
    bool support_in_gather_set = false;
    bool sparse = false;
    enum VdagKind { kStages, kRestricted, kProjected } vdag_kind = kStages;
    bool skip_zero_w = false;
    int key_bits() const {
        static_assert(AQC_NUM_BUFS <= 8, "x_buf takes the low three bits");
        return x_buf | (vdag ? 8 : 0) | (gather ? 16 : 0) | (gather_rides ? 32 : 0) | (grads ? 64 : 0) | (sparse ? 128 : 0) |
               (support_in_gather_set ? 256 : 0) | (skip_zero_w ? 512 : 0) | ((int)vdag_kind << 10);
    }
};

struct ProjRoute {
    bool ok = false;
    int t = 0, cb = 0, us = 0, nv = 0, nvp = 0, kv = 0, ntiles_v = 0;
    int first_subs = 0;
    Program vprog;
    std::vector<int> rest;
    DevPlan vsw;
    DevPlan vinv;
    DevBuf<double2> vm;
    DevBuf<double2> vy;
    DevBuf<double2> vme;
    DevBuf<double2> cpart;
    int cpart_shares = 0;
    int vy_copies = 1;
    unsigned l0_mask = 0;
    DevBuf<unsigned> d_tab;
    std::vector<unsigned> h_tab;
    unsigned ff_mask = 0, cb_mask = 0, tf_mask = 0;
    DevBuf<TileItem> d_items;
    DevBuf<int> d_count;
    DevBuf<int> d_lane_parts;
    ListKey init_key;
};

void lower_plan(const Program& prog, const Plan& plan, HostPlan& out, int reg_bits, bool with_dots, bool mfma = false, bool presplit = false, int beam_width = 64);
int upload_plan(DevPlan& p);
Plan mirror_plan(const Plan& plan);

}

using aqc::DevBuf; using aqc::DevPlan; using aqc::HostPlan; using aqc::PinBuf; using aqc::Program; using aqc::UJob;

struct aqc_ctx {
    Program prog;
    std::recursive_mutex mu;
    std::map<std::vector<int>, HostPlan> plan_cache;
    std::map<int, aqc_ws*> oneshot;
};

struct aqc_ws {
    aqc_ctx* ctx = nullptr;
    aqc::Switches sw;
    int device = 0, batch = 1, ncols = 1, pitch = 1, col_bits = 0, nbits = 0, threads = 256;
    size_t lane_elems = 0;
    hipStream_t stream = nullptr;
    DevPlan fwd, inv, sweep;
    double* d_thetas = nullptr;
    DevBuf<double> d_thetas_own;
    DevBuf<double> d_theta_bank;
    int bank_sets = 0, gather_count = 0;
    DevBuf<double> d_coef;
    DevBuf<double2> bufs[AQC_NUM_BUFS];
    PinBuf<double> h_pin;
    size_t pin_thetas = 0, pin_grads = 0, pin_small = 0;
    DevBuf<double2> d_partial;
    DevBuf<double2> d_grads;
    double* mirror_grads = nullptr;
    double* mirror_small = nullptr;
    DevBuf<double2> d_small;
    DevBuf<double2> d_vdot_part;
    DevBuf<double2> d_vdot_out;
    DevBuf<long long> d_index;
    DevBuf<long long> d_tmp_index;
    DevBuf<double2> d_tmp_small;
    DevBuf<long long> d_basis_index;
    DevBuf<long long> d_combo_prev[AQC_NUM_BUFS];
    bool combo_valid[AQC_NUM_BUFS] = {false, false, false, false, false, false};
    std::vector<long long> combo_last_elem[AQC_NUM_BUFS];
    std::vector<double> combo_last_coef[AQC_NUM_BUFS];
    DevBuf<char> d_sur;
    PinBuf<char> h_sur;
    int sur_states = 0;
    DevBuf<double> d_sur_real;
    DevBuf<long long> d_combo_index;
    DevBuf<double2> d_combo_coef;
    DevBuf<int> d_theta_slots;
    DevBuf<int> d_slot_theta;
    bool grads_direct = false;
    DevBuf<int> d_slot_ntiles;
    int nslots = 0, vdot_parts = 0;
    bool coef_valid = false;
    bool need_coef = false;
    std::map<std::vector<long long>, hipGraphExec_t> graphs;
    bool capturing = false;
    DevBuf<UJob> d_ujobs;
    bool ujobs_mirror = false;
    DevBuf<UJob> d_ujobs_route;
    int n_ujobs_route = 0;
    struct MpsSlot {
        std::vector<int> dims;
        std::vector<size_t> offset;
        DevBuf<double2> d_t;
    } mps[AQC_MPS_SLOTS];
    DevBuf<double> d_mps_lam;
    DevBuf<double2> d_mps_scratch;
    struct MpsTabs { std::vector<const void*> host; DevBuf<const void*> dev; unsigned long long tick = 0; };
    DevBuf<aqc::CdSegHost> d_cd_prog;
    int cd_nsteps = 0;
    DevBuf<double> d_cd_thetas;
    DevBuf<double> d_cd_fobj;
    DevBuf<double> d_cd_best;
    DevBuf<double> d_cd_real;
    DevBuf<int> d_cd_int;
    DevBuf<double> d_cd_profile;
    DevBuf<double> d_cd_part;
    MpsTabs mps_tabs[32];
    unsigned long long mps_tabs_tick = 0;
    hipEvent_t ev0 = nullptr, ev1 = nullptr, pev0 = nullptr, pev1 = nullptr;
    hipStream_t copy_stream = nullptr;
    hipEvent_t ev_ready = nullptr, ev_copied = nullptr;
    hipStream_t mps_stream = nullptr;
    hipEvent_t ev_mps_fork = nullptr, ev_mps_join = nullptr;
    bool copy_pending = false;
    const double* theta_host = nullptr;
    bool inv_mirrored = false;
    bool ckpt_valid = false;
    bool w_clean = true;
    unsigned long long supp_version[AQC_NUM_BUFS] = {0, 0, 0, 0, 0, 0};
    DevBuf<aqc::TileItem> d_sw_items;
    DevBuf<aqc::TileItem> d_sw_clear;
    DevBuf<int> d_sw_counts;
    DevBuf<int> d_sw_lane_parts;
    DevBuf<int> d_sw_prev_tiles;
    int sw_lists_built = 0;
    aqc::ListKey sw_items_key;
    DevBuf<double2> w2;
    DevBuf<double2> zw2;
    bool z_full = true;
    DevBuf<aqc::TileItem> d_vd_items;
    unsigned long long gather_gen = 0;
    aqc::ListKey vd_key;
    aqc::ListKey z_key;
    aqc::ProjRoute proj;
    bool proj_y0_ready = false;
    bool z_from_y = false;
    std::vector<long long> h_gather;
    aqc::ListKey projb_key;
    bool projb_ok = false;
    struct Sketch {
        DevBuf<double2> target;
        bool shared = false;
        DevBuf<double2> qr_part;
        DevBuf<double2> qr_rinv;
        DevBuf<double2> tmp;
        DevBuf<int> status;
        DevBuf<int> idx;
        DevBuf<double> adam;
        DevBuf<int> adam_i;
        DevBuf<double> profile;
        bool adam_started = false;
    } sk;
    bool profile = false;
    int64_t prof_count[AQC_NUM_KINDS] = {};
    double prof_ms[AQC_NUM_KINDS] = {};
    std::vector<std::pair<int, float>> prof_log;
};

namespace aqc {

struct ProfScope {
    aqc_ws* ws;
    int kind;
    ProfScope(aqc_ws* w, int k) : ws(w), kind(k) {
        if (ws->profile) (void)hipEventRecord(ws->pev0, ws->stream);
    }
    ~ProfScope() {
        if (!ws->profile) return;
        float ms = 0.f;
        if (hipEventRecord(ws->pev1, ws->stream) == hipSuccess && hipEventSynchronize(ws->pev1) == hipSuccess &&
            hipEventElapsedTime(&ms, ws->pev0, ws->pev1) == hipSuccess) {
            ws->prof_count[kind] += 1;
            ws->prof_ms[kind] += ms;
            if (ws->prof_log.size() < 100000) ws->prof_log.emplace_back(kind, ms);
        }
    }
};

inline int wait_result_copies(aqc_ws* ws) {
// ... 59 lines not shown
```

aqc_research_amd/csrc/aqc_ws_plan.cpp:

```cpp
#include "aqc_ws.h"

#include <algorithm>

using namespace aqc;

namespace aqc {

namespace {
unsigned swz3_host(unsigned l) { return l ^ ((l >> 4) & 15u) ^ ((l >> 8) & 15u); }

void emit_mops(const Program& prog, int gi, int pc, int pt, bool inverse, bool with_dots, std::vector<DevMop>& out) {
    const GateGroup& g = prog.groups[gi];
    const int rec = g.coef * kCoefStride;
    const int konst = (prog.n + prog.num_blocks) * kCoefStride + kLiftOffset;
    const int neg = inverse ? MOPF_NEG_S : 0;
    std::vector<std::pair<int, int>> dots;
    auto rot = [&](int kind, int p, int pair, int flags, int slot) {
        const int coef = pair < 0 ? konst : rec + kLiftOffset + 2 * pair;
        const bool has = with_dots && slot >= 0;
        out.push_back({kind, p, 0, flags, coef, has ? slot : -1, g.jblock, pair < 0 ? -1 : g.theta0 + pair});
        if (has) dots.push_back({slot, kind});
    };
    auto reduce = [&]() {
        if (dots.empty()) return;
        DevMop m = {MOP_REDUCE, -1, -1, 0, -1, -1, g.jblock, -2};
        int kinds = 0;
        for (size_t j = 0; j < dots.size(); ++j) {
            const auto& d = dots[dots.size() - 1 - j];
            kinds |= d.second << (4 * j);
            (j == 0 ? m.slot : j == 1 ? m.p : j == 2 ? m.p2 : m.coef) = d.first;
        }
        m.flags = kinds;
        out.push_back(m);
        dots.clear();
    };
    const int slot0 = gi * kSlotsPerGroup;
    if (g.type == GROUP_FRONT) {
        if (!inverse) {
            rot(MOP_RZ, pc, 2, 0, slot0 + 0);
            rot(MOP_RY, pc, 1, 0, slot0 + 1);
            rot(MOP_RZ, pc, 0, 0, slot0 + 2);
            reduce();
        } else {
            rot(MOP_RZ, pc, 0, neg, -1);
            rot(MOP_RY, pc, 1, neg, -1);
            rot(MOP_RZ, pc, 2, neg, -1);
        }
        return;
    }
    const int ekind = prog.entangler == 0 ? MOP_CX : (prog.entangler == 1 ? MOP_CZ : MOP_CP);
    const int rs = prog.entangler == 0 ? MOP_RX : MOP_RZ;
    if (!inverse) {
        if (g.flags & FLAG_PRE_RZ) rot(MOP_RZ, pc, -1, MOPF_NEG_S, -1);
        const bool cpdot = with_dots && prog.entangler == 2;
        out.push_back({ekind, pc, pt, 0, rec + 8, cpdot ? slot0 + 4 : -1, g.jblock, prog.entangler == 2 ? g.theta0 + 4 : -2});
        if (cpdot) { dots.push_back({slot0 + 4, MOP_CP}); reduce(); }
        rot(MOP_RY, pc, 0, 0, slot0 + 0);
        rot(MOP_RZ, pc, 1, 0, slot0 + 1);
        rot(MOP_RY, pt, 2, 0, slot0 + 2);
        rot(rs, pt, 3, 0, slot0 + 3);
        reduce();
        if (g.flags & FLAG_POST_RZ) rot(MOP_RZ, pt, -1, 0, -1);
    } else {
        if (g.flags & FLAG_POST_RZ) rot(MOP_RZ, pt, -1, MOPF_NEG_S, -1);
        rot(rs, pt, 3, neg, -1);
        rot(MOP_RY, pt, 2, neg, -1);
        rot(MOP_RZ, pc, 1, neg, -1);
        rot(MOP_RY, pc, 0, neg, -1);
        out.push_back({ekind, pc, pt, neg, rec + 8, -1, g.jblock, prog.entangler == 2 ? g.theta0 + 4 : -2});
        if (g.flags & FLAG_PRE_RZ) rot(MOP_RZ, pc, -1, 0, -1);
    }
}

}

void lower_plan(const Program& prog, const Plan& plan, HostPlan& out, int reg_bits, bool with_dots, bool mfma, bool presplit, int beam_width) {
    out.plan = plan;
    out.h_stages.clear();
    out.h_ops.clear();
    out.h_subs.clear();
    out.h_mops.clear();
    out.h_subs3.clear();
    out.h_grps.clear();
    out.reg_bits = reg_bits;
    out.v3 = mfma && reg_bits == 4 && (int)plan.stages.front().bits.size() >= 8;
    out.v2 = !out.v3 && reg_bits > 0 && (int)plan.stages.front().bits.size() >= reg_bits;
    if (out.v3) {
        if (!presplit) split_substages(prog, out.plan, 4, 1 << 30, beam_width);
    } else if (out.v2) {
        int max_ops = reg_bits == 4 ? kMaxOpsPerSub : kMaxOpsPerSub / 2;
        if (prog.entangler == 2) max_ops /= 2;
        split_substages(prog, out.plan, reg_bits, max_ops);
    }
    out.k = (int)plan.stages.front().bits.size();
    out.ntiles = 1 << (plan.nbits - out.k);
    uint64_t touched_global = 0;
    for (const Stage& st : out.plan.stages) {
        DevStage ds;
        memset(&ds, 0, sizeof ds);
        ds.k = (int)st.bits.size();
        ds.nops = (int)st.ops.size();
        ds.op_begin = (int)out.h_ops.size();
        ds.ntiles = 1 << (plan.nbits - ds.k);
        std::vector<int> local_of(plan.nbits, -1);
        for (int j = 0; j < ds.k; ++j) local_of[st.bits[j]] = j;
        for (int b = 0; b < plan.nbits; ++b)
            if (local_of[b] < 0) {
                ds.ubits[ds.nub++] = b;
                if (!(touched_global >> b & 1)) ds.fresh_nonlocal |= 1u << b;
            }
        uint32_t touched_local = 0;
        for (unsigned i = 0; i < 64; ++i) {
            uint32_t off = 0;
            for (int j = 0; j < 6 && j < ds.k; ++j)
                if (i >> j & 1) off |= 1u << st.bits[j];
            ds.dlo[i] = off;
        }
        for (unsigned i = 0; i < 256; ++i) {
            uint32_t off = 0;
            for (int j = 0; j < 8 && 6 + j < ds.k; ++j)
                if (i >> j & 1) off |= 1u << st.bits[6 + j];
            ds.dhi[i] = off;
        }
        for (int gi : st.ops) {
            const GateGroup& g = prog.groups[gi];
            DevOp op;
            op.type = g.type;
            op.p0 = local_of[plan.col_bits + g.q0];
            op.p1 = g.q1 >= 0 ? local_of[plan.col_bits + g.q1] : 0;
            op.flags = g.flags;
            op.coef = g.coef;
            op.slot = gi * kSlotsPerGroup;
            op.jblock = g.jblock;
            op.pad = 0;
            out.h_ops.push_back(op);
        }
        ds.sub_begin = (int)out.h_subs.size();
        ds.nsubs = 0;
        if (out.v2 || out.v3) {
            for (const SubStage& sub : st.subs) {
                DevSub dsub;
                memset(&dsub, 0, sizeof dsub);
                dsub.nbits = (int)sub.bits.size();
                std::vector<int> reg_of(ds.k, -1);
                for (int j = 0; j < dsub.nbits; ++j) { dsub.bits[j] = sub.bits[j]; reg_of[sub.bits[j]] = j; }
                dsub.mop_begin = (int)out.h_mops.size();
                const int grp_begin = (int)out.h_grps.size();
                for (int gi : sub.ops) {
                    const GateGroup& g = prog.groups[gi];
                    const int pc = reg_of[local_of[plan.col_bits + g.q0]];
                    const int pt = g.q1 >= 0 ? reg_of[local_of[plan.col_bits + g.q1]] : 0;
                    emit_mops(prog, gi, pc, pt, plan.inverse, with_dots, out.h_mops);
                    if (out.v3)
                        out.h_grps.push_back({g.type, pc, g.q1 >= 0 ? pt : (pc == 0 ? 1 : 0), g.flags, g.theta0,
                                              with_dots ? gi * kSlotsPerGroup : -1, g.jblock, 0});
                }
                dsub.nmops = (int)out.h_mops.size() - dsub.mop_begin;
                out.h_subs.push_back(dsub);
                ++ds.nsubs;
                if (out.v3) {
                    DevSub3 d3;
                    memset(&d3, 0, sizeof d3);
                    d3.mop_begin = dsub.mop_begin;
                    d3.nmops = dsub.nmops;
                    d3.grp_begin = grp_begin;
                    d3.ngrp = (int)out.h_grps.size() - grp_begin;
                    std::vector<int> cbits;
                    for (int j = 0; j < ds.k; ++j)
                        if (reg_of[j] < 0) cbits.push_back(j);
                    for (int j = 0; j < 4; ++j) d3.bits[j] = dsub.bits[j];
                    auto deposit = [](unsigned v, const int* bits, int nb) {
                        unsigned o = 0;
                        for (int j = 0; j < nb; ++j)
                            if (v >> j & 1) o |= 1u << bits[j];
                        return o;
                    };
                    const int nc = (int)cbits.size();
                    for (unsigned v = 0; v < 16; ++v) {
                        d3.dep_a[v] = (uint16_t)swz3_host(deposit(v, dsub.bits, 4));
                        d3.dep_clo[v] = (uint16_t)swz3_host(deposit(v, cbits.data(), std::min(nc, 4)));
                    }
                    for (unsigned g = 0; g < 64; ++g)
                        d3.dep_chi[g] = nc > 4 && g < (1u << (nc - 4)) ? (uint16_t)swz3_host(deposit(g, cbits.data() + 4, nc - 4)) : 0;
                    for (unsigned l = 0; l < 64; ++l)
                        d3.lane12[l] = (uint32_t)(d3.dep_clo[l & 15] ^ d3.dep_a[l >> 4]) | ((uint32_t)(d3.dep_a[l & 15] ^ d3.dep_clo[l >> 4]) << 16);
                    for (unsigned g = 0; g < 16; ++g)
                        for (unsigned s = 0; s < 4; ++s) {
                            d3.kk[g][s] = (uint32_t)(d3.dep_a[4 * s] ^ d3.dep_chi[g]) << 4;
                            d3.kk[g][4 + s] = (uint32_t)(d3.dep_clo[4 * s] ^ d3.dep_chi[g]) << 4;
                        }
                    {
                        auto fresh = [&](int local_pos) { return !(touched_global >> st.bits[local_pos] & 1) && !(touched_local >> local_pos & 1); };
                        uint32_t info = 0;
                        for (int i = 0; i < 4 && 4 + i < nc; ++i) {
                            if (fresh(cbits[4 + i])) info |= 1u << i;
                            info |= (uint32_t)cbits[4 + i] << (8 + 4 * i);
                        }
                        for (int i = 0; i < dsub.nbits && i < 4; ++i)
                            if (fresh(dsub.bits[i])) info |= 1u << (4 + i);
                        if (dsub.nbits == 4) info |= (uint32_t)dsub.bits[2] << 24 | (uint32_t)dsub.bits[3] << 28;
                        else info &= ~0xC0u;
                        d3.skipinfo = info;
                        for (int i = 0; i < dsub.nbits; ++i) touched_local |= 1u << dsub.bits[i];
                    }
                    out.h_subs3.push_back(d3);
                }
            }
        }
        out.h_stages.push_back(ds);
        for (int b : st.bits) touched_global |= 1ull << b;
    }
}

int upload_plan(DevPlan& p) {
    if (p.d_stages.upload(p.h_stages)) return 1;
    const size_t nops = std::max<size_t>(p.h_ops.size(), 1);
    if (p.d_ops.alloc(nops)) return 1;
    HIP_OK(hipMemset(p.d_ops, 0, nops * sizeof(DevOp)));
    if (!p.h_ops.empty())
        HIP_OK(hipMemcpy(p.d_ops, p.h_ops.data(), p.h_ops.size() * sizeof(DevOp), hipMemcpyHostToDevice));
    if (p.d_subs.upload(p.h_subs) || p.d_mops.upload(p.h_mops)) return 1;
    if (p.v3 && !p.h_subs3.empty() && (p.d_subs3.upload(p.h_subs3) || p.d_grps.upload(p.h_grps))) return 1;
    return 0;
}

Plan mirror_plan(const Plan& plan) {
    Plan out = plan;
    out.inverse = !plan.inverse;
    std::reverse(out.stages.begin(), out.stages.end());
    for (Stage& st : out.stages) {
        std::reverse(st.ops.begin(), st.ops.end());
        std::reverse(st.subs.begin(), st.subs.end());
        for (SubStage& sub : st.subs) std::reverse(sub.ops.begin(), sub.ops.end());
    }
    return out;
}

}
```

aqc_research_amd/csrc/aqc_ws_project.cpp:

```cpp
#include "aqc_ws.h"

#include <algorithm>

using namespace aqc;

namespace aqc {

namespace {
int popc(uint64_t v) { return __builtin_popcountll(v); }
unsigned deposit_bits(unsigned v, const std::vector<int>& bits) {
    unsigned o = 0;
    for (size_t j = 0; j < bits.size(); ++j)
        if (v >> j & 1) o |= 1u << bits[j];
    return o;
}
}

void proj_plan(aqc_ws* ws, int low_bits) {
    ProjRoute& pr = ws->proj;
    pr.ok = false;
    const Program& prog = ws->ctx->prog;
    const DevPlan& p = ws->sweep;
    if (!ws->sw.projected || !ws->sw.sparse_sweep || !ws->inv_mirrored || !p.v3 || ws->col_bits != 0 || ws->ncols != 1 ||
        p.plan.stages.size() < 2 || prog.n > 30)
        return;
    const int n = prog.n;
    uint64_t L0 = 0, T = 0;
    for (int b : p.plan.stages[0].bits) L0 |= 1ull << b;
    pr.rest.clear();
    for (size_t s = 1; s < p.plan.stages.size(); ++s)
        for (int gi : p.plan.stages[s].ops) {
            const GateGroup& g = prog.groups[gi];
            pr.rest.push_back(gi);
            T |= 1ull << g.q0;
            if (g.q1 >= 0) T |= 1ull << g.q1;
        }
    if (pr.rest.empty()) return;
    const uint64_t all = (1ull << n) - 1, F = all & ~L0, Cb = T & L0, Us = L0 & ~T;
    pr.t = popc(T); pr.cb = popc(Cb); pr.us = popc(Us);
    pr.nv = pr.t + pr.cb;
    if ((Us & 15) != 15 || pr.t < 4 || pr.cb > 6 || pr.nv + 2 > n || pr.nv > 20) return;
    pr.nvp = std::max(pr.nv, 8);
    pr.kv = std::min(pr.nvp, p.k);
    pr.ntiles_v = 1 << (pr.nvp - pr.kv);
    pr.first_subs = p.h_stages[0].nsubs;
    std::vector<int> tbits, cbits, usbits;
    std::vector<int> vq(n, -1);
    for (int b = 0; b < n; ++b) {
        if (T >> b & 1) { vq[b] = (int)tbits.size(); tbits.push_back(b); }
        if (Cb >> b & 1) cbits.push_back(b);
        if (Us >> b & 1) usbits.push_back(b);
    }
    pr.vprog = prog;
    for (int gi : pr.rest) {
        GateGroup& g = pr.vprog.groups[gi];
        g.q0 = vq[g.q0];
        if (g.q1 >= 0) g.q1 = vq[g.q1];
    }
    Plan best;
    for (int lb = std::max(low_bits, 2); lb >= 2; --lb) {
        Plan cand = make_plan(pr.vprog, 0, pr.kv, lb, false, &pr.rest, pr.nvp);
        if (best.stages.empty() || cand.stages.size() < best.stages.size()) best = cand;
    }
    lower_plan(pr.vprog, best, pr.vsw, 4, true, true, false, (int)ws->sw.projected_beam);
    if (!pr.vsw.v3 || !check_plan(pr.vprog, pr.vsw.plan, &pr.rest).empty()) return;
    lower_plan(pr.vprog, mirror_plan(pr.vsw.plan), pr.vinv, 4, false, true, true);
    if (!pr.vinv.v3 || pr.vinv.h_subs3.size() != pr.vsw.h_subs3.size()) return;
    for (DevPlan* q : {&pr.vsw, &pr.vinv})
        for (DevStage& ds : q->h_stages) {
            if (ds.nub >= 32) return;
            ds.ubits[ds.nub++] = pr.nvp;
            ds.ntiles *= 2;
        }
    pr.l0_mask = (unsigned)L0;
    pr.ff_mask = (unsigned)(F & ~T);
    pr.cb_mask = (unsigned)Cb;
    pr.tf_mask = (unsigned)(T & F);
    pr.h_tab.clear();
    for (unsigned i = 0; i < (1u << pr.t); ++i) pr.h_tab.push_back(deposit_bits(i, tbits));
    for (unsigned k = 0; k < (1u << pr.us); ++k) pr.h_tab.push_back(deposit_bits(k, usbits));
    for (unsigned c = 0; c < (1u << pr.cb); ++c) pr.h_tab.push_back(deposit_bits(c, cbits));
    for (unsigned c = 0; c < (1u << pr.cb); ++c) {
        const unsigned addr = deposit_bits(c, cbits);
        unsigned it = 0;
        for (size_t j = 0; j < tbits.size(); ++j)
            if (addr >> tbits[j] & 1) it |= 1u << j;
        pr.h_tab.push_back(it);
    }
    pr.ok = true;
    if (ws->sw.verbose)
        fprintf(stderr, "aqc_hip: projected route: the sweep's stages after the first run on %d virtual qubits (%d touched, %d shared with the first "
                "stage) instead of %d: %zu stage(s) of 2^%d tiles, %zu sub-stages\n", pr.nv, pr.t, pr.cb, n, pr.vsw.h_stages.size(), pr.kv,
                pr.vsw.h_subs3.size());
}

int proj_alloc(aqc_ws* ws) {
    ProjRoute& pr = ws->proj;
    if (!pr.ok) return 0;
    const size_t B = (size_t)ws->batch;
    if (upload_plan(pr.vsw) || upload_plan(pr.vinv)) return 1;
    const size_t nsubs = std::max<size_t>(pr.vsw.h_subs3.size(), 1);
    if (pr.vsw.d_umat.alloc(B * nsubs * 12 * 64) || pr.vinv.d_umat.alloc(B * nsubs * 12 * 64)) return 1;
    if (pr.vsw.d_rpart.alloc(B * nsubs * (2 * (size_t)pr.ntiles_v) * 256)) return 1;
    const size_t velems = B * (2ull << pr.nvp), vbytes = sizeof(double2) * velems;
    pr.vy_copies = pr.us > 8 && pr.us <= 10 && pr.cb <= 4 ? 1 << (pr.us - 8) : 1;
    if (pr.vm.alloc(velems) || pr.vy.alloc(velems * pr.vy_copies)) return 1;
    HIP_OK(hipMemsetAsync(pr.vm, 0, vbytes, ws->stream));
    HIP_OK(hipMemsetAsync(pr.vy, 0, vbytes * pr.vy_copies, ws->stream));
    pr.cpart_shares = 0;
    const long want_wgs = ws->sw.projected_fused_wgs;
    if (pr.us <= 10 && pr.cb <= 4 && (long)B < want_wgs) {
        int shares = 1;
        const long cap = ws->sw.projected_fused_max_shares;
        while ((long)B * pr.vy_copies * shares < want_wgs && 2 * shares <= (1 << (pr.t - 4)) && 2 * shares <= cap) shares *= 2;
        if (shares > 1) {
            if (pr.cpart.alloc((size_t)shares * 2 * B * (16ull << pr.us))) return 1;
            pr.cpart_shares = shares;
        }
    }
    if (pr.vme.alloc(velems)) return 1;
    HIP_OK(hipMemsetAsync(pr.vme, 0, vbytes, ws->stream));
    if (pr.d_tab.upload(pr.h_tab) || pr.d_items.alloc(2 * B * pr.ntiles_v) || pr.d_count.alloc(1) || pr.d_lane_parts.alloc(B)) return 1;
    HIP_OK(hipMemsetAsync(pr.d_count, 0, sizeof(int), ws->stream));
    HIP_OK(hipMemsetAsync(pr.d_lane_parts, 0, sizeof(int) * B, ws->stream));
    return 0;
}

bool sweep_route_projected(const aqc_ws* ws, bool sparse) { return sparse && ws->proj.ok; }

static ProjArgs proj_args(aqc_ws* ws);
static int ensure_pattern(aqc_ws* ws, const ProjArgs& a) {
    ProjRoute& pr = ws->proj;
    if (pr.vsw.h_stages.size() == 1 && built_for(ws, pr.init_key, ws->sw_items_key)) return 0;
    ProfScope ps(ws, AQC_K_MISC);
    HIP_OK(launch_project_init(a, ws->stream));
    record_key(ws, pr.init_key, ws->sw_items_key);
    return 0;
}

static ProjArgs proj_args(aqc_ws* ws) {
    ProjRoute& pr = ws->proj;
    ProjArgs a;
    memset(&a, 0, sizeof a);
    a.lane_stride = ws->lane_elems;
    a.items = ws->d_sw_items;
    a.nitems = ws->d_sw_counts;
    a.lane_parts = ws->d_sw_lane_parts;
    const DevStage& s0 = ws->sweep.h_stages[0];
    a.nub0 = s0.nub;
    for (int i = 0; i < s0.nub; ++i) a.ubits0[i] = s0.ubits[i];
    a.ff_mask = pr.ff_mask; a.cb_mask = pr.cb_mask; a.tf_mask = pr.tf_mask;
    a.nvp = pr.nvp;
    a.off_t = pr.d_tab;
    a.off_cb = pr.d_tab + (1u << pr.t) + (1u << pr.us);
    a.it_of_c = a.off_cb + (1u << pr.cb);
    a.off_us = pr.d_tab + (1u << pr.t);
    a.us_bits = pr.us;
    a.t = pr.t; a.cb = pr.cb; a.ntiles_v = pr.ntiles_v;
    a.vm = pr.vm;
    a.vitems = pr.d_items; a.vcount = pr.d_count; a.vlane_parts = pr.d_lane_parts;
    a.batch = ws->batch;
    return a;
}

static ProjArgs y_product(aqc_ws* ws, ProjArgs a, const double2* y) {
    const ProjRoute& pr = ws->proj;
    a.y = y;
    a.s = ws->bufs[AQC_BUF_W];
    a.out = pr.vy;
    a.s_virtual = 0; a.out_virtual = 1;
    a.staged = 1;
    a.keep_bits = pr.t; a.k_bits = pr.us;
    a.y_keep = ProjMap{a.off_t, 0};
    a.y_k = ProjMap{a.off_us, 0};
    a.s_k = ProjMap{a.off_us, 0};
    a.s_c = ProjMap{a.off_cb, 0};
    a.o_keep = ProjMap{nullptr, 0};
    a.o_c = ProjMap{nullptr, pr.t};
    return a;
}

int run_projected_stages(aqc_ws* ws) {
    ProjRoute& pr = ws->proj;
    if (!ws->proj_y0_ready) {
        const ProjArgs a = proj_args(ws);
        if (ensure_pattern(ws, a)) return 1;
        ProfScope ps(ws, AQC_K_PROJECT);
        HIP_OK(launch_project(y_product(ws, a, ws->bufs[AQC_BUF_ZW]), ws->stream));
    }
    for (size_t s = 0; s < pr.vsw.h_stages.size(); ++s) {
        const Stage3Args a = projected_sweep_stage(ws, s);
        ProfScope ps(ws, AQC_K_SWEEP_VIRTUAL);
        HIP_OK(launch_sweep3(pr.kv, ws->stream, a, ws->sw));
    }
    return 0;
}

Stage3Args virtual_stage3_args(aqc_ws* ws, const DevPlan& v, size_t s) {
    const ProjRoute& pr = ws->proj;
    Stage3Args a = stage3_args(ws, v, s);
    a.lane_stride = 2ull << pr.nvp;
    a.ntiles = 2 * pr.ntiles_v;
    a.items = pr.d_items; a.nitems = pr.d_count; a.max_items = 2 * ws->batch * pr.ntiles_v;
    return a;
}
Stage3Args projected_sweep_stage(aqc_ws* ws, size_t s) {
    const ProjRoute& pr = ws->proj;
    Stage3Args a = virtual_stage3_args(ws, pr.vsw, s);
    a.in0 = pr.vm; a.in1 = pr.vy; a.out0 = pr.vm; a.out1 = pr.vy;
    a.store_out = s + 1 < pr.vsw.h_stages.size() ? 3 : 0;
    stage3_sweep_fields(a, pr.vsw, a.ntiles, 0);
    return a;
}

bool projected_pairs(const aqc_ws* ws) {
    const ProjRoute& pr = ws->proj;
    return pr.ok && ws->sw.projected_pairs && !ws->capturing && pr.vsw.h_stages.size() == 1 && pr.vinv.h_stages.size() == 1 &&
           ws->sweep.k == pr.kv && ws->inv.k == pr.kv;
}

RgradSecond projected_rgrad_plan(aqc_ws* ws) {
    ProjRoute& pr = ws->proj;
    DevPlan& v = pr.vsw;
    RgradSecond r;
    memset(&r, 0, sizeof r);
    r.subs = v.d_subs3; r.grps = v.d_grps; r.rpart = v.d_rpart; r.lane_parts = pr.d_lane_parts; r.umat = v.d_umat;
    r.nparts = 2 * pr.ntiles_v;
    r.nsubs_total = r.count = (int)v.h_subs3.size();
    return r;
}

bool vdag_route_projected(aqc_ws* ws, int x_buf) {
    ProjRoute& pr = ws->proj;
    if (!pr.ok || !ws->sw.projected_vdag || ws->capturing || (long long)ws->lane_elems * ws->batch < ws->sw.projected_vdag_min_elems) return false;
    const ListKey key = key_of(ws, x_buf, true);
    if (ws->projb_key == key) return ws->projb_ok;
    ws->projb_key = key;
    ws->projb_ok = false;
    const std::vector<long long>& el = ws->combo_last_elem[x_buf];
    const std::vector<double>& cf = ws->combo_last_coef[x_buf];
    const size_t B = (size_t)ws->batch;
    if (el.size() != 2 * B || cf.size() != 4 * B || (ws->gather_count > 0 && ws->h_gather.size() != (size_t)ws->gather_count)) return false;
    const unsigned fmask = ~pr.l0_mask & (unsigned)((1ull << ws->ctx->prog.n) - 1);
    for (size_t b = 0; b < B; ++b) {
        if (el[2 * b] < 0 || el[2 * b + 1] >= 0 || cf[4 * b] != 1.0 || cf[4 * b + 1] != 0.0) return false;
        const unsigned e = (unsigned)el[2 * b];
        for (long long gl : ws->h_gather) {
            const unsigned d = e ^ (unsigned)gl;
            if ((d & fmask) == 0) continue;
            if ((d & pr.l0_mask) != 0 || (d & pr.ff_mask) != 0) return false;
        }
    }
    ws->projb_ok = true;
    return true;
}

struct VirtualRun { const DevPlan& plan; const double2* src; double2* dst; };
static Stage3Args virtual_apply_stage(aqc_ws* ws, const VirtualRun& v, size_t s) {
    Stage3Args a = virtual_stage3_args(ws, v.plan, s);
    a.in0 = s == 0 ? v.src : v.dst;
    a.out0 = v.dst;
    return a;
}
static int enqueue_couple(aqc_ws* ws, int k, const Stage3Args* real, const VirtualRun* v) {
    if (real && v) {
        ProfScope ps(ws, AQC_K_APPLY_VIRTUAL);
        HIP_OK(launch_apply3_pair(k, ws->stream, *real, virtual_apply_stage(ws, *v, 0), ws->sw));
    } else if (real) {
        ProfScope ps(ws, AQC_K_APPLY_LIST);
        HIP_OK(launch_apply3(k, ws->stream, *real, ws->sw));
    } else {
        for (size_t s = 0; s < v->plan.h_stages.size(); ++s) {
            ProfScope ps(ws, AQC_K_APPLY_VIRTUAL);
            HIP_OK(launch_apply3(ws->proj.kv, ws->stream, virtual_apply_stage(ws, *v, s), ws->sw));
        }
    }
    return 0;
}

int run_vdag_projected(aqc_ws* ws, int x_buf) {
    ProjRoute& pr = ws->proj;
    const DevPlan& p = ws->sweep;
    const DevPlan& iv = ws->inv;
    if (ensure_umat(ws, ws->inv, kURoute)) return 1;
    if (!ws->d_sw_items || !ws->w_clean) return fail("objective by projection without the sparse route's preparation");
    if (ensure_sweep_items(ws, x_buf)) return 1;
    Stage3Args psi = stage3_args(ws, p, 0);
    psi.in0 = ws->bufs[x_buf];
    psi.out0 = ws->bufs[AQC_BUF_W];
    stage3_first_list(ws, psi);
    Stage3Args last = stage3_args(ws, iv, iv.h_stages.size() - 1);
    last.in0 = ws->bufs[AQC_BUF_ZW];
    last.out0 = ws->bufs[AQC_BUF_Z];
    stage3_first_list(ws, last);
    const VirtualRun mend{pr.vsw, pr.vm, pr.vme};
    const VirtualRun y0{pr.vinv, pr.vy, pr.vy};
    const ProjArgs a = proj_args(ws);
    const bool pairs = projected_pairs(ws);

    if (!pairs && enqueue_couple(ws, p.k, &psi, nullptr)) return 1;
    if (ensure_pattern(ws, a)) return 1;
    if (enqueue_couple(ws, p.k, pairs ? &psi : nullptr, &mend)) return 1;
    if (ws->sw.projected_fused && pr.us <= 10 && pr.cb <= 4 && (pr.us <= 8 || pr.vy_copies == 1 << (pr.us - 8))) {
        ProjArgs q = a;
        q.part_stride = (size_t)ws->batch * (2ull << pr.nvp);
        q.cpart = pr.cpart; q.cpart_shares = pr.cpart_shares;
        q.y = ws->bufs[AQC_BUF_Y]; q.s = ws->bufs[AQC_BUF_W];
        ProfScope ps(ws, AQC_K_PROJECT);
        HIP_OK(launch_project_fused(q, pr.vme, ws->bufs[AQC_BUF_ZW], pr.vy, ws->stream, ws->sw.projected_fused_qb == 4 ? 4 : 2));
    } else {
        {
            ProfScope ps(ws, AQC_K_PROJECT);
            HIP_OK(launch_project(y_product(ws, a, ws->bufs[AQC_BUF_Y]), ws->stream));
        }
        ProjArgs q = a;
        q.y = ws->bufs[AQC_BUF_Y]; q.s = pr.vme; q.out = ws->bufs[AQC_BUF_ZW];
        q.s_virtual = 1; q.out_virtual = 0; q.staged = 0;
        q.keep_bits = pr.us; q.k_bits = pr.t;
        q.y_keep = ProjMap{a.off_us, 0}; q.y_k = ProjMap{a.off_t, 0};
        q.s_k = ProjMap{nullptr, 0}; q.s_c = ProjMap{nullptr, pr.t};
        q.o_keep = ProjMap{a.off_us, 0}; q.o_c = ProjMap{a.off_cb, 0};
        ProfScope ps(ws, AQC_K_PROJECT);
        HIP_OK(launch_project(q, ws->stream));
    }
    if (!pairs && enqueue_couple(ws, iv.k, nullptr, &y0)) return 1;
    if (enqueue_couple(ws, iv.k, &last, pairs ? &y0 : nullptr)) return 1;
    vdag_projected_state_after(ws, x_buf);
    return 0;
}

int proj_fix_amplitudes(aqc_ws* ws, int x_buf) {
    ProjRoute& pr = ws->proj;
    if (results_guard(ws)) return 1;
    ProfScope ps(ws, AQC_K_MISC);
    ProjArgs a = proj_args(ws);
    HIP_OK(launch_project_amps(a, ws->d_index, ws->gather_count, ws->d_combo_prev[x_buf], ws->d_small, pr.vy, ws->bufs[AQC_BUF_Z], ws->stream));
    return 0;
}

}
```

aqc_research_amd/engine.py:

```python
import ctypes
from ctypes import byref, c_double, c_float, c_int, c_int32, c_int64, c_void_p
from typing import Optional, Tuple

import numpy as np

from . import _lib
from ._lib import BUF_W, BUF_X, BUF_X2, BUF_Y, BUF_Z, BUF_ZW, K_APPLY, K_COEF, K_FINALIZE, K_MISC, K_SWEEP, check, dptr


def default_device() -> int:
    import os

    for name in ("AQC_DEVICE", "LOCAL_RANK"):
        v = os.environ.get(name, "")
        if v.strip().isdigit():
            return int(v) % max(1, _lib.lib().aqc_device_count()) if name == "LOCAL_RANK" else int(v)
    return 0


def live_buffers() -> tuple:
    dev, pin = c_int64(0), c_int64(0)
    check(_lib.lib().aqc_live_buffers(byref(dev), byref(pin)))
    return dev.value, pin.value


def _structure_key(circ) -> tuple:
    trotter = hasattr(circ, "is_second_order")
    blocks = np.ascontiguousarray(circ.blocks, dtype=np.int32)
    return (int(circ.num_qubits), str(circ.entangler), blocks.shape[1], blocks.tobytes(), trotter,
            bool(circ.is_second_order) if trotter else False)


class HipContext:

    _cache = {}

    def __init__(self, circ):
        L = _lib.lib()
        n, ent, nb, _, trotter, second = key = _structure_key(circ)
        if ent not in _lib.ENTANGLERS:
            raise ValueError(f"unknown entangler {ent!r}")
        blocks = np.ascontiguousarray(circ.blocks, dtype=np.int32)
        handle = c_void_p()
        status = L.aqc_create(n, _lib.ENTANGLERS[ent], blocks.ctypes.data_as(ctypes.POINTER(c_int32)), nb,
                              int(trotter), int(second), byref(handle))
        if status != 0:
            raise ValueError("aqc_hip: " + L.aqc_last_error().decode())
        self.handle = handle
        self.key = key
        self.num_qubits, self.entangler, self.num_blocks = n, ent, nb
        self.trotter, self.second_order = trotter, second
        self.num_thetas = L.aqc_num_thetas(handle)
        self.num_gate_groups = L.aqc_num_gate_groups(handle)
        self._ws = {}

    @classmethod
    def of(cls, circ) -> "HipContext":
        key = _structure_key(circ)
        ctx = cls._cache.get(key)
        if ctx is None:
            if len(cls._cache) >= 64:
                cls._cache.pop(next(iter(cls._cache)))
            ctx = cls._cache[key] = cls(circ)
        return ctx

    def workspace(self, batch: int = 1, ncols: int = 1, device: Optional[int] = None, **kw) -> "Workspace":
        if device is None:
            device = default_device()
        key = (batch, ncols, device, tuple(sorted(kw.items())))
        ws = self._ws.get(key)
        if ws is None:
            ws = self._ws[key] = Workspace(self, batch=batch, ncols=ncols, device=device, **kw)
        return ws

    def plan_projected(self, tile_bits: int = 0, low_bits: int = -1) -> dict:
        c = (ctypes.c_int32 * 16)()
        check(_lib.lib().aqc_plan_projected(self.handle, tile_bits, low_bits, c))
        if not c[0]:
            return {}
        return {"virtual_qubits": int(c[1]), "touched_qubits": int(c[2]), "shared_with_first_stage": int(c[3]), "stages": int(c[4]),
                "substages": int(c[5]), "tile_bits": int(c[6]), "substages_on_the_register": int(c[7]), "summed_bits": int(c[8]),
                "padded_qubits": int(c[9]), "substages_per_stage": [int(c[10 + i]) for i in range(min(int(c[4]), 6))]}

    def plan(self, which: int = 1, ncols: int = 1, tile_bits: int = 0, low_bits: int = -1):
        L = _lib.lib()
        ns = c_int()
        check(L.aqc_plan_query(self.handle, ncols, which, tile_bits, low_bits, -1, byref(ns), None, None, None, None))
        out = []
        bits = (c_int * 64)()
        ops = (c_int * max(1, self.num_gate_groups))()
        for s in range(ns.value):
            nb, no = c_int(), c_int()
            check(L.aqc_plan_query(self.handle, ncols, which, tile_bits, low_bits, s, byref(ns), bits, byref(nb), ops, byref(no)))
            out.append((list(bits[: nb.value]), list(ops[: no.value])))
        return out

    def __del__(self):
        try:
            for ws in self._ws.values():
                ws.close()
            if self.handle:
                _lib.lib().aqc_destroy(self.handle)
                self.handle = None
        except Exception:
            pass


class Workspace:

    def __init__(self, ctx: HipContext, batch: int = 1, ncols: int = 1, device: Optional[int] = None,
                 tile_bits_apply: int = 0, tile_bits_sweep: int = 0):
        device = default_device() if device is None else int(device)
        self.ctx, self.batch, self.ncols, self.device = ctx, int(batch), int(ncols), device
        self.dim = 1 << ctx.num_qubits
        self.T = ctx.num_thetas
        self._L = _lib.lib()
        handle = c_void_p()
        check(self._L.aqc_ws_create(ctx.handle, device, batch, ncols, tile_bits_apply, tile_bits_sweep, byref(handle)))
        self.handle = handle
        self._gather_count = 0
        self._gen = [0] * 6

    def _touch(self, *bufs) -> None:
        for b in bufs:
            self._gen[b] += 1

    def generation(self, buf: int) -> int:
        return self._gen[buf]

    def _shape(self):
        return (self.batch, self.dim) if self.ncols == 1 else (self.batch, self.dim, self.ncols)

    def set_thetas(self, thetas) -> None:
        th = _lib.as_f64(thetas, self.batch * self.T, "thetas")
        check(self._L.aqc_ws_set_thetas(self.handle, dptr(th)))

    def upload(self, buf: int, data, lane: Optional[int] = None) -> None:
        self._touch(buf)
        if lane is None:
            a = _lib.as_c128(data)
            if a.size != self.batch * self.dim * self.ncols:
                raise ValueError(f"expected {self._shape()} complex values, got shape {a.shape}")
            check(self._L.aqc_ws_upload(self.handle, buf, dptr(a)))
        else:
            a = _lib.as_c128(data)
            if a.size != self.dim * self.ncols:
                raise ValueError("lane data has the wrong size")
            check(self._L.aqc_ws_upload_lane(self.handle, buf, lane, dptr(a)))

    def broadcast(self, buf: int, data) -> None:
        self._touch(buf)
        a = _lib.as_c128(data)
        if a.size != self.dim * self.ncols:
            raise ValueError("broadcast data has the wrong size")
        check(self._L.aqc_ws_broadcast(self.handle, buf, dptr(a)))

    def download(self, buf: int, lane: Optional[int] = None, out: Optional[np.ndarray] = None) -> np.ndarray:
        if out is not None:
            want = self._shape() if lane is None else self._shape()[1:]
            if not (isinstance(out, np.ndarray) and out.dtype == np.complex128 and out.flags.c_contiguous
                    and out.flags.writeable and out.size == int(np.prod(want))):
                raise ValueError(f"out must be a writable C-contiguous complex128 array of {int(np.prod(want))} elements")
        if lane is None:
            res = np.empty(self._shape(), dtype=np.complex128) if out is None else out
            check(self._L.aqc_ws_download(self.handle, buf, dptr(res)))
        else:
            res = np.empty(self._shape()[1:], dtype=np.complex128) if out is None else out
            check(self._L.aqc_ws_download_lane(self.handle, buf, lane, dptr(res)))
        return res

    def copy_lane_from(self, src: "Workspace", src_buf: int, src_lane: int, dst_buf: int, dst_lane: int) -> None:
        self._touch(dst_buf)
        check(self._L.aqc_ws_copy_lane(self.handle, dst_buf, dst_lane, src.handle, src_buf, src_lane))

    def set_basis(self, buf: int, index) -> None:
        self._touch(buf)
        idx = np.ascontiguousarray(np.broadcast_to(np.asarray(index, dtype=np.int64), (self.batch,)))
        check(self._L.aqc_ws_set_basis(self.handle, buf, idx.ctypes.data_as(ctypes.POINTER(c_int64))))

    def set_combo(self, buf: int, index, coef) -> None:
        self._touch(buf)
        idx = np.ascontiguousarray(np.asarray(index, dtype=np.int64).reshape(self.batch, 2))
        cf = np.ascontiguousarray(np.asarray(coef, dtype=np.complex128).reshape(self.batch, 2))
        check(self._L.aqc_ws_set_combo(self.handle, buf, idx.ctypes.data_as(ctypes.POINTER(c_int64)), dptr(cf)))

    def set_identity(self, buf: int) -> None:
        self._touch(buf)
        check(self._L.aqc_ws_set_identity(self.handle, buf))

    def apply(self, inverse: bool, src: int = BUF_Y, dst: int = BUF_Z) -> None:
        self._touch(dst)
        check(self._L.aqc_ws_apply(self.handle, int(bool(inverse)), src, dst))

    def grad(self, block_range: Optional[Tuple[int, int]] = None, front_layer: bool = True) -> None:
        self._touch(BUF_W, BUF_ZW)
        lo, hi = (-1, -1) if block_range is None else (int(block_range[0]), int(block_range[1]))
        check(self._L.aqc_ws_grad(self.handle, lo, hi, int(bool(front_layer))))

    def eval(self, thetas=None, vdag: bool = True, gather: bool = False, grad: bool = True, x_buf: int = BUF_X,
             block_range: Optional[Tuple[int, int]] = None, front_layer: bool = True):
        self._touch(*(([BUF_Z] if vdag else []) + ([BUF_W, BUF_ZW] if grad else [])))
        th = None if thetas is None else _lib.as_f64(thetas, self.batch * self.T, "thetas")
        hs = np.empty((self.batch, self._gather_count), dtype=np.complex128) if gather else None
        g = np.empty((self.batch, self.T), dtype=np.complex128) if grad else None
        lo, hi = (-1, -1) if block_range is None else (int(block_range[0]), int(block_range[1]))
        check(self._L.aqc_ws_eval(self.handle, None if th is None else th.ctypes.data, int(bool(vdag)),
                                  None if hs is None else hs.ctypes.data, x_buf, lo, hi, int(bool(front_layer)),
                                  None if g is None else g.ctypes.data))
        return hs, g

    def surrogate_eval(self, thetas, weight: np.ndarray, max_no: np.ndarray, update_state: bool = True,
                       block_range: Optional[Tuple[int, int]] = None, front_layer: bool = True, real_only: bool = False):
        self._touch(BUF_Z, BUF_W, BUF_ZW, BUF_X2)
        th = _lib.as_f64(thetas, self.batch * self.T, "thetas")
        if not (isinstance(weight, np.ndarray) and weight.dtype == np.float64 and weight.flags.c_contiguous and weight.size == self.batch):
            raise ValueError("weight must be a C-contiguous float64 array of one entry per lane")
        if not (isinstance(max_no, np.ndarray) and max_no.dtype == np.int64 and max_no.flags.c_contiguous and max_no.size == self.batch):
            raise ValueError("max_no must be a C-contiguous int64 array of one entry per lane")
        f = np.empty(self.batch)
        fid = np.empty(self.batch) if update_state else None
        hs = np.empty((self.batch, self._gather_count), dtype=np.complex128)
        g = np.empty((self.batch, self.T), dtype=np.float64 if real_only else np.complex128)
        lo, hi = (-1, -1) if block_range is None else (int(block_range[0]), int(block_range[1]))
        check(self._L.aqc_ws_surrogate_eval(self.handle, dptr(th), int(update_state), dptr(weight),
                                            max_no.ctypes.data_as(ctypes.POINTER(c_int64)), lo, hi, int(bool(front_layer)),
                                            dptr(f), None if fid is None else dptr(fid), dptr(hs),
                                            None if real_only else dptr(g), dptr(g) if real_only else None))
        return f, fid, hs, g

    def grad_from(self, x_buf: int, block_range: Optional[Tuple[int, int]] = None, front_layer: bool = True) -> None:
        self._touch(BUF_W, BUF_ZW)
        lo, hi = (-1, -1) if block_range is None else (int(block_range[0]), int(block_range[1]))
        check(self._L.aqc_ws_grad_from(self.handle, x_buf, lo, hi, int(bool(front_layer))))

    def get_grads(self) -> np.ndarray:
# ... 423 lines not shown
```

include/aqc_hip.h:

```cpp
#ifndef AQC_HIP_H
#define AQC_HIP_H

#include <stddef.h>
#include <stdint.h>

#ifdef __cplusplus
extern "C" {
#endif

typedef struct aqc_ctx aqc_ctx;
typedef struct aqc_ws aqc_ws;

enum { AQC_CX = 0, AQC_CZ = 1, AQC_CP = 2 };
enum { AQC_LANES_REFUSED = 3 };
enum { AQC_BUF_Y = 0, AQC_BUF_Z = 1, AQC_BUF_X = 2, AQC_BUF_W = 3, AQC_BUF_ZW = 4, AQC_BUF_X2 = 5, AQC_NUM_BUFS = 6 };
enum { AQC_K_APPLY = 0, AQC_K_SWEEP = 1, AQC_K_COEF = 2, AQC_K_FINALIZE = 3, AQC_K_MISC = 4,
       AQC_K_SWEEP_LIST = 5, AQC_K_APPLY_LIST = 6,
       AQC_K_PROJECT = 7, AQC_K_SWEEP_VIRTUAL = 8,
       AQC_K_APPLY_VIRTUAL = 9,
       AQC_NUM_KINDS = 10 };

const char* aqc_version(void);
const char* aqc_last_error(void);
int aqc_device_count(void);
int aqc_live_buffers(int64_t* device, int64_t* pinned);

int aqc_create(int num_qubits, int entangler, const int32_t* blocks, int num_blocks,
               int trotter, int second_order, aqc_ctx** out);
int aqc_destroy(aqc_ctx* ctx);
int aqc_num_thetas(const aqc_ctx* ctx);
int aqc_num_gate_groups(const aqc_ctx* ctx);

int aqc_v_mul_vec(aqc_ctx* ctx, const double* thetas, const double* vec, double* out);
int aqc_vdag_mul_vec(aqc_ctx* ctx, const double* thetas, const double* vec, double* out);
int aqc_grad_dot_vec(aqc_ctx* ctx, const double* thetas, const double* x, const double* vh_y,
                     int block_from, int block_to, int front_layer, double* grad);
int aqc_v_mul_mat(aqc_ctx* ctx, const double* thetas, double* mat, int ncols);
int aqc_vdag_mul_mat(aqc_ctx* ctx, const double* thetas, double* mat, int ncols);
int aqc_grad_dot_mat(aqc_ctx* ctx, const double* thetas, const double* x_mat, const double* vh_y_mat,
                     int ncols, double* grad);

int aqc_ws_create(aqc_ctx* ctx, int device, int batch, int ncols, int tile_bits_apply,
                  int tile_bits_sweep, aqc_ws** out);
int aqc_ws_destroy(aqc_ws* ws);
int aqc_ws_set_thetas(aqc_ws* ws, const double* thetas );
int aqc_ws_upload(aqc_ws* ws, int buf, const double* src );
int aqc_ws_upload_lane(aqc_ws* ws, int buf, int lane, const double* src);
int aqc_ws_broadcast(aqc_ws* ws, int buf, const double* src );
int aqc_ws_download(aqc_ws* ws, int buf, double* dst);
int aqc_ws_download_lane(aqc_ws* ws, int buf, int lane, double* dst);
int aqc_ws_copy_lane(aqc_ws* dst_ws, int dst_buf, int dst_lane, aqc_ws* src_ws, int src_buf, int src_lane);
int aqc_ws_set_basis(aqc_ws* ws, int buf, const int64_t* index );
int aqc_ws_set_combo(aqc_ws* ws, int buf, const int64_t* index , const double* coef );
int aqc_ws_set_identity(aqc_ws* ws, int buf);
int aqc_ws_apply(aqc_ws* ws, int inverse, int src_buf, int dst_buf);
int aqc_ws_grad(aqc_ws* ws, int block_from, int block_to, int front_layer);
int aqc_ws_get_grads(aqc_ws* ws, double* grads );
int aqc_ws_gather(aqc_ws* ws, int buf, const int64_t* index, int count, double* out);
int aqc_ws_vdot(aqc_ws* ws, int buf_a, int buf_b, double* out );
int aqc_ws_sync(aqc_ws* ws);

int aqc_ws_eval(aqc_ws* ws, const double* thetas , int do_vdag,
                double* gathered , int x_buf, int block_from, int block_to,
                int front_layer, double* grads );
int aqc_ws_grad_from(aqc_ws* ws, int x_buf, int block_from, int block_to, int front_layer);

int aqc_ws_theta_bank(aqc_ws* ws, const double* thetas, int nsets);
int aqc_ws_use_theta_set(aqc_ws* ws, int set_index);
int aqc_ws_gather_setup(aqc_ws* ws, const int64_t* index, int count);
int aqc_ws_gather_launch(aqc_ws* ws, int buf);
int aqc_ws_gather_fetch(aqc_ws* ws, double* out );
int aqc_ws_vdot_launch(aqc_ws* ws, int buf_a, int buf_b);
int aqc_ws_vdot_fetch(aqc_ws* ws, double* out );
int aqc_ws_results_async(aqc_ws* ws);
int aqc_ws_objective_launch(aqc_ws* ws, int x_buf, int block_from, int block_to, int front_layer);
int aqc_ws_results_fetch(aqc_ws* ws, double* small_out , double* grads_out );

enum { AQC_MPS_SLOTS = 64 };
int aqc_ws_mps_upload(aqc_ws* ws, int slot, const int32_t* dims , const double* gammas,
                      const double* lambdas);
int aqc_ws_mps_to_vec(aqc_ws* ws, int slot, int buf, int lane);
int aqc_ws_mps_to_vec_batch(aqc_ws* ws, int count, const int32_t* slots, int buf, const int32_t* lanes);
int aqc_ws_mps_dot(aqc_ws* ws, int slot_a, int slot_b, double* out );

int aqc_zgemm(int device, int conj_trans_a, int M, int N, int K, const double* A, int lda, const double* B, int ldb,
              double* C, int ldc);

int aqc_gate_1q(int device, int n, int64_t ncols, int qubit, const double* gate, const double* src, double* dst);
int aqc_gate_2q(int device, int n, int64_t ncols, int ctrl, int targ, const double* gate, const double* src, double* dst);
int aqc_gate_dot(int device, int n, int64_t ncols, int kind, int q0, int q1, const double* w, const double* z,
                 double* out );

int aqc_xxz_mul_vec(int device, int n, int lanes, double delta, const double* src, double* dst);
int aqc_xxz_energy(int device, int n, int lanes, double delta, const double* src, double* energy );
int aqc_xxz_evolve(int device, int n, int lanes, int shared_src, double delta, const double* times , const double* src,
                   double* dst, int32_t* terms_out);

#define AQC_OBS_TILE_BITS 11
#define AQC_OBS_LOW_BITS 5
#define AQC_OBS_MAX_SUBSETS 16
int aqc_obs_plan(int n, int npairs, const int32_t* pairs, int max_passes, int max_subsets, int32_t* npasses, int32_t* nsubsets,
                 int32_t* pass_bits, int32_t* pass_nsub, int32_t* subsets, int32_t* serves);
int aqc_obs_rdm(int device, int n, int lanes, const double* src, int k, int nsets, const int32_t* qubits, double* out);

typedef struct aqc_mps aqc_mps;
int aqc_mps_create(int device, int n, const int32_t* dims, const double* gammas, const double* lambdas, aqc_mps** out);
int aqc_mps_destroy(aqc_mps* mps);
int aqc_mps_clone(const aqc_mps* src, aqc_mps** out);
int aqc_mps_num_qubits(const aqc_mps* mps);
int aqc_mps_device(const aqc_mps* mps);
int aqc_mps_dims(const aqc_mps* mps, int32_t* dims );
double aqc_mps_discarded_weight(const aqc_mps* mps);
int aqc_mps_export(aqc_mps* mps, double* gammas, double* lambdas);
int aqc_mps_gate1(aqc_mps* mps, int qubit, const double* gate);
int aqc_mps_gate2(aqc_mps* mps, int ctrl, int targ, const double* gate, double trunc_thr, int max_bond);
int aqc_mps_dot(aqc_mps* a, aqc_mps* b, double* out );
int aqc_mps_dot_ops(aqc_mps* a, aqc_mps* b, int nops, const int32_t* qubits, const double* gates, double* out);
typedef struct aqc_circuit {
    int32_t num_qubits, entangler , num_blocks, trotter, second_order;
    const int32_t* blocks;
} aqc_circuit;
int aqc_mps_apply_circuit(aqc_mps* mps, const aqc_circuit* circ, const double* thetas, int inverse, double trunc_thr, int max_bond);
int aqc_mps_fast_dot_gradient(const aqc_circuit* circ, const aqc_mps* lvec, const aqc_mps* vh_phi, const double* thetas,
                              double trunc_thr, int max_bond, int block_from, int block_to, int front_layer, double* grad);
typedef struct aqc_mpsb aqc_mpsb;
int aqc_mpsb_create(int device, int num_qubits, int lanes, aqc_mpsb** out);
int aqc_mpsb_destroy(aqc_mpsb* b);
int aqc_mpsb_gate2_stats(aqc_mpsb* b, int enable, double* out, int reset);
int aqc_mpsb_set_targets(aqc_mpsb* b, aqc_mps* const* handles, int shared);
int aqc_mpsb_set_lhs(aqc_mpsb* b, aqc_mps* const* handles, int shared);
int aqc_mpsb_set_lhs_basis(aqc_mpsb* b, const uint8_t* bits);
int aqc_mpsb_eval(aqc_mpsb* b, const aqc_circuit* circ, const double* thetas, double trunc_thr, int max_bond, int block_from,
                  int block_to, int front_layer, double* h , double* grad ,
                  double* discarded , int32_t* max_bond_out );
int aqc_mpsb_apply_circuit(aqc_mpsb* b, const aqc_circuit* circ, const double* thetas, int inverse, double trunc_thr, int max_bond,
                           double* discarded , int32_t* max_bond_out );
int aqc_mpsb_export(aqc_mpsb* b, int lane, aqc_mps** out);
int aqc_mpsb_vh(aqc_mpsb* b, const aqc_circuit* circ, const double* thetas, double trunc_thr, int max_bond, int half, int num_amps,
                double* amps , double* discarded , int32_t* max_bond_out );
int aqc_mpsb_grad(aqc_mpsb* b, const aqc_circuit* circ, int block_from, int block_to, int front_layer, double* grad );
int aqc_mpsb_set_bank(aqc_mpsb* b, aqc_mps* const* states, int count);
int aqc_mpsb_vh_bank(aqc_mpsb* b, const aqc_circuit* circ, const double* thetas, double trunc_thr, int max_bond, int half, int num_amps,
                     double* amps , double* discarded , int32_t* max_bond_out );
int aqc_mpsb_gradient_of(aqc_mpsb* b, const aqc_circuit* circ, const double* thetas, double trunc_thr, int max_bond, int block_from,
                         int block_to, int front_layer, double* grad );
int aqc_svd(int device, int m, int n, const double* a, double* u, double* s, double* vh, int* sweeps);
int aqc_svd_batch(int device, int count, int m, int n, const int32_t* rows, const int32_t* cols ,
                  const double* a , double* u , double* s ,
                  double* vh , int32_t* sweeps , int32_t* status );
double aqc_svd_batch_core_ms(void);

int aqc_ws_cd_sweep(aqc_ws* ws, double* thetas_io , double* fobj);
int aqc_ws_cd_sweeps(aqc_ws* ws, double* thetas_io , double* fobj , int nsweeps, int max_steps);
int aqc_ws_cd_fits_one_launch(const aqc_ws* ws);
enum { AQC_CD_RUNNING = 0, AQC_CD_NORMAL = 1, AQC_CD_EARLY = 2, AQC_CD_TIMEOUT = 3 };
enum { AQC_CD_ROUTE_AUTO = 0, AQC_CD_ROUTE_PERSISTENT = 1, AQC_CD_ROUTE_WIDE = 2 };
int aqc_ws_cd_minimize(aqc_ws* ws, const double* thetas0 , int maxiter, int chunk, double dtheta_thr, double fobj_thr,
                       double time_limit_s, int route, int max_steps, double* best_thetas, double* best_f, int64_t* nit, int32_t* status,
                       double* profile);

int aqc_ws_timer_start(aqc_ws* ws);
int aqc_ws_timer_stop(aqc_ws* ws, float* elapsed_ms);
int aqc_ws_profile_enable(aqc_ws* ws, int on);
int aqc_ws_profile_get(aqc_ws* ws, int kind, int64_t* launches, double* total_ms);
int aqc_ws_profile_reset(aqc_ws* ws);
int aqc_ws_profile_log(aqc_ws* ws, int32_t* kinds, double* ms, int cap, int* count);
int aqc_ws_plan_stage(aqc_ws* ws, int which, int stage, int* num_subs, int* num_groups, int* bits_out);
int aqc_ws_plan_skips(aqc_ws* ws, int which, int stage, int* out, int max_subs);
int aqc_ws_sweep_r_only_sub(aqc_ws* ws);
int aqc_ws_sparse_counts(aqc_ws* ws, int64_t* counts);
int aqc_ws_projected_info(aqc_ws* ws, int32_t* info);
int aqc_plan_projected(aqc_ctx* ctx, int tile_bits, int low_bits, int32_t* info);
int aqc_switch_info(int index, const char** name, const char** dflt, const char** when, const char** reader, const char** doc);
int aqc_ws_switch(const aqc_ws* ws, const char* name, int64_t* value);
int aqc_ws_plan_info(aqc_ws* ws, int which ,
                     int* num_stages, int* tile_bits, int* num_tiles);
int aqc_ws_plan_substages(aqc_ws* ws, int which);
int aqc_ws_kernel_family(aqc_ws* ws, int which);
int aqc_plan_query(aqc_ctx* ctx, int ncols, int which, int tile_bits, int low_bits, int stage,
                   int* num_stages, int* bits_out, int* num_bits, int* ops_out, int* num_ops);

int aqc_plan_substages(aqc_ctx* ctx, int ncols, int which, int tile_bits, int low_bits, int stage, int* num_subs,
                       int* subs_out , int max_subs);

int aqc_ws_surrogate_eval(aqc_ws* ws, const double* thetas, int update_state, double* weight_io, int64_t* max_no_io,
                          int block_from, int block_to, int front_layer, double* f_out, double* fidelity_out, double* hs_out,
                          double* grads_out, double* grad_real_out);
int aqc_ws_lbfgs(aqc_ws* ws, const double* x0, int maxiter, int memory, double gtol, double ftol, double fid_thr,
                 int max_backtracks, int block_from, int block_to, int front_layer, double* x_out, double* f_out,
                 double* fidelity_out, int64_t* nit_out, int64_t* nfev_out, double* weight_out, int64_t* max_no_out);
int aqc_ws_lbfgs_mat(aqc_ws* ws, const double* x0, int maxiter, int memory, double gtol, double ftol, double fobj_thr,
                     double fidelity_thr, int max_backtracks, double* x_out, double* f_out, double* fidelity_out,
                     int64_t* nit_out, int64_t* nfev_out, int32_t* status_out);

enum { AQC_SKETCH_RAND = 0, AQC_SKETCH_ALT = 1, AQC_SKETCH_EIGEN = 2 };
enum { AQC_QR_OK = 0, AQC_QR_RANK_DEFICIENT = 1 };
int aqc_qr(int device, int m, int k, const double* a, double* q_out, int32_t* status);
int aqc_ws_sketch_target(aqc_ws* ws, const double* U, int shared);
int aqc_ws_sketch_generate(aqc_ws* ws, int kind, uint64_t seed, int64_t iteration, const int32_t* alt_idx, const double* omega,
                           int32_t* status);
int aqc_ws_sketch_draw(aqc_ws* ws, int kind, uint64_t seed, int64_t iteration, int buf);
int aqc_ws_sketch_adam(aqc_ws* ws, int kind, const double* x0, int niter, const double* lr, double beta1, double beta2, double eps,
                       double tol, uint64_t seed, int64_t iter0, const int32_t* reset, const int32_t* alt_idx, double* x_out,
                       double* fobj_profile, double* best_f, double* best_x, int64_t* nit, int32_t* status);

typedef struct aqc_comm aqc_comm;
int aqc_comm_unique_id(char* out128);
int aqc_comm_create(const char* id128, int nranks, int rank, int device, aqc_comm** out);
int aqc_comm_destroy(aqc_comm* comm);
int aqc_comm_rank(const aqc_comm* comm);
int aqc_comm_size(const aqc_comm* comm);
int aqc_comm_allgather(aqc_comm* comm, const double* send, double* recv, size_t count);
int aqc_comm_allreduce(aqc_comm* comm, double* data, size_t count, int op);
int aqc_comm_barrier(aqc_comm* comm);

#ifdef __cplusplus
}
#endif
#endif
```

Before: 1.202 million evals/s.

## Skip structurally-zero substage work in list apply kernels from sparse basis-state inputs

Adds a SKIPZ variant of the MFMA apply kernel. When the input of a list launch is known to be a one- or two-basis-state combination, the kernel precomputes per-substage skip masks from the plan's skip info and runs only the groups and k-slices that can be nonzero. It also reorders spectator bits in the projected virtual plan so that constrained bits fall in the high chunk, and moves the shared skip-mask rules into a common header with a host-side query for inspection. This cuts MFMA and LDS work on the first stage of projected and virtual runs, at the cost of more kernel variants, added register pressure, and uniform mask setup per work item.

```diff
diff --git a/aqc_research_amd/_lib.py b/aqc_research_amd/_lib.py
--- a/aqc_research_amd/_lib.py
+++ b/aqc_research_amd/_lib.py
@@ -118,6 +118,8 @@
     "aqc_ws_sparse_counts": (c_int, [_P, POINTER(c_int64)]),
     "aqc_ws_projected_info": (c_int, [_P, POINTER(c_int32)]),
     "aqc_plan_projected": (c_int, [_P, c_int, c_int, POINTER(c_int32)]),
+    "aqc_plan_skip_masks": (c_int, [_P, c_int, c_int, c_int, c_int64, POINTER(c_int32), POINTER(c_int32), POINTER(c_int32), POINTER(c_int32),
+                                    c_int]),
     "aqc_switch_info": (c_int, [c_int] + [POINTER(c_char_p)] * 5),
     "aqc_ws_switch": (c_int, [_P, c_char_p, POINTER(c_int64)]),
     "aqc_ws_plan_skips": (c_int, [_P, c_int, c_int, POINTER(c_int), c_int]),
diff --git a/aqc_research_amd/csrc/aqc_api.cpp b/aqc_research_amd/csrc/aqc_api.cpp
--- a/aqc_research_amd/csrc/aqc_api.cpp
+++ b/aqc_research_amd/csrc/aqc_api.cpp
@@ -1,4 +1,5 @@
 #include "aqc_ws.h"
+#include "aqc_skip_rule.h"
 
 using namespace aqc;
 
@@ -136,13 +137,11 @@
     return 0;
 }
 
-int aqc_plan_projected(aqc_ctx* ctx, int tile_bits, int low_bits, int32_t* info) {
-    if (!ctx || !info) return fail("null argument");
+static void projected_plans(aqc_ctx* ctx, int tile_bits, int low_bits, aqc_ws& tmp) {
     if (tile_bits <= 0) tile_bits = 12;
     if (low_bits < 0) low_bits = 3;
     const Program& prog = ctx->prog;
     tile_bits = std::min(std::max(tile_bits, 8), std::min(12, prog.n));
-    aqc_ws tmp;
     tmp.ctx = ctx;
     tmp.ncols = 1; tmp.col_bits = 0; tmp.nbits = prog.n;
     Plan best = make_plan(prog, 0, tile_bits, low_bits, false);
@@ -155,7 +154,60 @@
     tmp.sw.sparse_sweep = 1;
     tmp.inv_mirrored = tmp.sweep.v3 && tmp.sweep.plan.stages.size() >= 2;
     proj_plan(&tmp, low_bits);
+}
+
+int aqc_plan_projected(aqc_ctx* ctx, int tile_bits, int low_bits, int32_t* info) {
+    if (!ctx || !info) return fail("null argument");
+    aqc_ws tmp;
+    projected_plans(ctx, tile_bits, low_bits, tmp);
     const int rc = aqc_ws_projected_info(&tmp, info);
+    tmp.ctx = nullptr;
+    return rc;
+}
+
+int aqc_plan_skip_masks(aqc_ctx* ctx, int tile_bits, int low_bits, int list, long long elem, int32_t* head, int32_t* local_bits, int32_t* layout,
+                        int32_t* masks, int max_subs) {
+    if (!ctx || !head || !local_bits || !layout || !masks || list < 0 || list > 1 || elem < 0) return fail("invalid argument");
+    aqc_ws tmp;
+    projected_plans(ctx, tile_bits, low_bits, tmp);
+    const aqc::ProjRoute& pr = tmp.proj;
+    int rc = 0;
+    if (!tmp.sweep.v3 || (list == 1 && !pr.ok)) rc = fail("no such list at this tiling");
+    else {
+        const DevPlan& p = list ? pr.vsw : tmp.sweep;
+        const DevStage& ds = p.h_stages[0];
+        const Stage& st = p.plan.stages[0];
+        const int nw = skip_tile_waves(ds.k), ngroups = 1 << (ds.k - 8);
+        head[0] = ds.nsubs; head[1] = ds.k; head[2] = nw; head[3] = list ? pr.t : 0; head[4] = list ? pr.cb : 0; head[5] = ds.ntiles;
+        std::vector<int> treal, creal;
+        if (list) {
+            const unsigned l0 = pr.l0_mask;
+            for (int b = 0; b < ctx->prog.n; ++b)
+                if ((pr.cb_mask | pr.tf_mask) >> b & 1) { treal.push_back(b); if (l0 >> b & 1) creal.push_back(b); }
+        }
+        for (int j = 0; j < ds.k; ++j) {
+            const int q = st.bits[j];
+            local_bits[j] = !list ? q : (q < pr.t ? treal[q] + ((pr.cb_mask >> treal[q] & 1) ? 256 : 0) : (q < pr.nv ? 512 + creal[q - pr.t] : -1));
+        }
+        for (int i = 0; i < ds.nsubs && i < max_subs; ++i) {
+            const DevSub3& d3 = p.h_subs3[ds.sub_begin + i];
+            int32_t* lay = layout + 12 * i;
+            auto position = [](unsigned slot) { const unsigned l = slot ^ ((slot >> 4) & 15u) ^ ((slot >> 8) & 15u); return l ? __builtin_ctz(l) : -1; };
+            const int nreg = (int)st.subs[i].bits.size(), nc = ds.k - nreg;
+            for (int j = 0; j < 12; ++j) lay[j] = -1;
+            for (int j = 0; j < nreg && j < 4; ++j) lay[j] = position(d3.dep_a[1u << j]);
+            for (int j = 0; j < nc && j < 4; ++j) lay[4 + j] = position(d3.dep_clo[1u << j]);
+            for (int j = 4; j < nc && j < 8; ++j) lay[4 + j] = position(d3.dep_chi[1u << (j - 4)]);
+            for (int g = 0; g < 16; ++g) {
+                unsigned nz = 0, kn = 0, kv[1] = {0};
+                if (g < ngroups) {
+                    if (list) { vskip_masks<1, 1>((uint64_t)d3.pad3[0] | (uint64_t)d3.pad3[1] << 32, elem, g, nz, kv); kn = kv[0]; }
+                    else skip_masks<1, 1>(ds, d3.skipinfo, elem, -1, g, nz, kn);
+                }
+                masks[16 * i + g] = nz ? (int32_t)kn : 0;
+            }
+        }
+    }
     tmp.ctx = nullptr;
     return rc;
 }
diff --git a/aqc_research_amd/csrc/aqc_kernels3.hip b/aqc_research_amd/csrc/aqc_kernels3.hip
--- a/aqc_research_amd/csrc/aqc_kernels3.hip
+++ b/aqc_research_amd/csrc/aqc_kernels3.hip
@@ -7,6 +7,7 @@
 #include "aqc_device.h"
 #include "aqc_launch.h"
 #include "aqc_math.h"
+#include "aqc_skip_rule.h"
 
 namespace aqc {
 
@@ -178,6 +179,13 @@
 }
 
 __device__ __forceinline__ int uniform_load(const int* p) { return __builtin_amdgcn_readfirstlane(*p); }
+__device__ __forceinline__ unsigned const_load(const void* p) {
+    return *reinterpret_cast<const __attribute__((address_space(4))) unsigned*>((const __attribute__((address_space(4))) void*)p);
+}
+__device__ __forceinline__ long long uniform_i64(long long v) {
+    const unsigned lo = __builtin_amdgcn_readfirstlane((unsigned)v), hi = __builtin_amdgcn_readfirstlane((unsigned)((unsigned long long)v >> 32));
+    return (long long)(((unsigned long long)hi << 32) | lo);
+}
 struct ItemAt { int bl, tile, slot; };
 template <bool LIST>
 __device__ __forceinline__ ItemAt item_at(const Stage3Args& a, int wi) {
@@ -188,10 +196,11 @@
     const int bl = wi / a.ntiles;
     return ItemAt{bl, wi - bl * a.ntiles, 0};
 }
-template <int K, bool LIST, bool PAIR = false>
+template <int K, bool LIST, bool PAIR = false, bool SKIPZ = false>
 __device__ __forceinline__ void apply_mfma_body(const Stage3Args& a0, const Stage3Args& b0, const int wg, const int nwg) {
     using TS = TileShape<K>;
     static_assert(!PAIR || (LIST && K >= 12), "the pair form walks two lists with persistent workgroups");
+    static_assert(!SKIPZ || LIST, "only a list launch knows its input tiles as basis states");
     extern __shared__ __attribute__((aligned(16))) char smem[];
     const Stage3Args* ca = &a0;
 #define a (*ca)
@@ -224,12 +233,66 @@
         AQC_STAMP(0);
         if (!(kApplySkip & 64)) load_tiles3<K, 1>(tw, nullptr, a.in0 + (size_t)bl * a.lane_stride + tile_base3(st, it.tile), nullptr, st, lo, wave);
     }
+
     __builtin_amdgcn_s_waitcnt(0x0F70);
     AQC_STAMP(1);
     for (;;) {
     const int bl = it.bl;
     const size_t lane_off = (size_t)bl * a.lane_stride + tile_base3(st, it.tile);
     const double* umat = a.umat + (size_t)bl * a.nsubs_total * 12 * 64;
+    constexpr unsigned kAllGroups = (1u << TS::kGpw) - 1;
+    constexpr unsigned kFull8 = kAllGroups | 15u << 4, kFull20 = kAllGroups | ((1u << (4 * TS::kGpw)) - 1) << 4;
+    unsigned long long hm = 0;
+    bool pattern_in = false;
+    if (SKIPZ) {
+        const long long* supp = (const long long*)uniform_ptr(a.supp);
+        if (supp != nullptr) {
+            pattern_in = const_load(&a.pattern) != 0;
+            const unsigned* sp = (const unsigned*)(supp + 2 * (size_t)bl);
+            const long long u0 = (long long)((unsigned long long)const_load(sp + 1) << 32 | const_load(sp));
+            const long long u1 = (long long)((unsigned long long)const_load(sp + 3) << 32 | const_load(sp + 2));
+            if (pattern_in) {
+                const int slot = (it.tile >> (st.nub - 1)) & 1;
+                const long long e = (slot == 0 && u0 >= 0) ? u0 : u1;
+#pragma unroll
+                for (int i = 0; i < 3; ++i) {
+                    const DevSub3* sub = &a.subs[st.sub_begin + (i < st.nsubs ? i : 0)];
+                    const unsigned long long vinfo = (unsigned long long)const_load(&sub->pad3[1]) << 32 | const_load(&sub->pad3[0]);
+                    unsigned nz, kn[TS::kGpw], m = 0;
+                    vskip_masks<TS::kGpw, NW>(vinfo, e, wave, nz, kn);
+#pragma unroll
+                    for (int j = 0; j < TS::kGpw; ++j) m |= kn[j] << (4 + 4 * j);
+                    m = (m | nz) ^ kFull20;
+                    if (i >= st.nsubs || vinfo == 0 || e < 0) m = 0;
+                    hm |= (unsigned long long)m << (20 * i);
+                }
+            } else {
+                unsigned lm[K];
+#pragma unroll
+                for (int p = 0; p < K; ++p) lm[p] = const_load(p < 6 ? &st.dlo[1u << p] : &st.dhi[1u << (p - 6)]);
+                const unsigned long long toff = (unsigned long long)tile_base3(st, it.tile);
+                const unsigned fresh_nl = const_load(&st.fresh_nonlocal);
+                long long l0 = -1, l1 = -1;
+                if (u0 >= 0 && (((unsigned long long)u0 ^ toff) & fresh_nl) == 0) l0 = 0;
+                if (u1 >= 0 && (((unsigned long long)u1 ^ toff) & fresh_nl) == 0) l1 = 0;
+#pragma unroll
+                for (int p = 0; p < K; ++p) {
+                    if (l0 >= 0 && ((unsigned long long)u0 & lm[p])) l0 |= 1ll << p;
+                    if (l1 >= 0 && ((unsigned long long)u1 & lm[p])) l1 |= 1ll << p;
+                }
+#pragma unroll
+                for (int i = 0; i < 8; ++i) {
+                    const unsigned info = const_load(&a.subs[st.sub_begin + (i < st.nsubs ? i : 0)].skipinfo);
+                    unsigned nz, kn;
+                    skip_masks_local<TS::kGpw, NW>(info, l0, l1, wave, nz, kn);
+                    unsigned m = (nz | kn << 4) ^ kFull8;
+                    if (i >= st.nsubs || !skip_info_sheds(info)) m = 0;
+                    hm |= (unsigned long long)m << (8 * i);
+                }
+            }
+            hm = (unsigned long long)uniform_i64((long long)hm);
+        }
+    }
     int nwi = wi + nwg;
     bool more = kPersist && st.nsubs > 0 && nwi < nwork;
     const Stage3Args* na = ca;
@@ -262,6 +325,50 @@
             }
         }
         sub_addr(ad, cur, lds_base);
+        unsigned nzmask = kAllGroups, kneed[TS::kGpw];
+        bool head = false;
+#pragma unroll
+        for (int j = 0; j < TS::kGpw; ++j) kneed[j] = 15u;
+        if (SKIPZ && hm != 0) {
+            if (pattern_in) {
+                const unsigned m = si < 3 ? (unsigned)(hm >> (20 * si)) & 0xFFFFFu : 0u;
+                head = m != 0;
+                nzmask = (m ^ kFull20) & kAllGroups;
+#pragma unroll
+                for (int j = 0; j < TS::kGpw; ++j) kneed[j] = ((m ^ kFull20) >> (4 + 4 * j)) & 15u;
+            } else {
+                const unsigned m = si < 8 ? (unsigned)(hm >> (8 * si)) & 255u : 0u;
+                head = m != 0;
+                nzmask = (m ^ kFull8) & kAllGroups;
+#pragma unroll
+                for (int j = 0; j < TS::kGpw; ++j) kneed[j] = (m ^ kFull8) >> 4;
+            }
+        }
+        if (SKIPZ && head) {
+#pragma unroll
+            for (int j = 0; j < TS::kGpw; ++j) {
+                if (!(nzmask >> j & 1)) continue;
+                Acc3 hacc;
+                hacc.k1 = double4_t{0.0, 0.0, 0.0, 0.0}; hacc.k2 = hacc.k1; hacc.k3 = hacc.k1;
+                cplx hv[4];
+#pragma unroll
+                for (int s = 0; s < 4; ++s)
+                    if (kneed[j] >> s & 1) hv[s] = lds_get(ad.a1 ^ ad.k1[j][s]);
+#pragma unroll
+                for (int s = 0; s < 4; ++s) {
+                    if (!(kneed[j] >> s & 1)) continue;
+                    double hs = hv[s].x + hv[s].y;
+                    asm volatile("" : "+v"(hs));
+                    hacc.k1 = mfma(hs, cur.u0[s], hacc.k1);
+                    hacc.k2 = mfma(hv[s].x, cur.u1[s], hacc.k2);
+                    hacc.k3 = mfma(hv[s].y, cur.u2[s], hacc.k3);
+                }
+                cplx ho[4];
+                u_combine(hacc, ho);
+#pragma unroll
+                for (int r = 0; r < 4; ++r) lds_put(ad.a2 ^ ad.k2[j][r], ho[r]);
+            }
+        } else {
         cplx v[2][4];
         Acc3 acc;
 #pragma unroll
@@ -317,6 +424,7 @@
                 }
             }
             __builtin_amdgcn_sched_barrier(0);
+        }
         }
         if (si + 1 < st.nsubs || more) {
             cur = nxt;
@@ -345,29 +453,29 @@
 #undef a
 #undef st
 }
-template <int K, bool LIST = false>
+template <int K, bool LIST = false, bool SKIPZ = false>
 __global__ __launch_bounds__(TileShape<K>::kWaves * 64, 2) void apply_mfma_kernel(const Stage3Args a) {
-    apply_mfma_body<K, LIST>(a, a, (int)blockIdx.x, (int)gridDim.x);
+    apply_mfma_body<K, LIST, false, SKIPZ>(a, a, (int)blockIdx.x, (int)gridDim.x);
 }
 #ifndef AQC_PAIR_PLAIN_BOUNDARY
 #define AQC_PAIR_PLAIN_BOUNDARY 0
 #endif
-template <int K>
+template <int K, bool SKIPZ = false>
 __global__ __launch_bounds__(TileShape<K>::kWaves * 64, 2) void apply_pair_kernel(const Stage3Args a, const Stage3Args b, const int grid_a) {
     if constexpr (K >= 12 && !AQC_PAIR_PLAIN_BOUNDARY) {
         static_assert(sizeof(Stage3Args) % 8 == 0 && alignof(Stage3Args) == 8, "b follows a in the kernel-argument segment without padding");
         const __attribute__((address_space(4))) char* kp = (const __attribute__((address_space(4))) char*)__builtin_amdgcn_kernarg_segment_ptr();
         const Stage3Args* pa = (const Stage3Args*)(const void*)kp;
         const Stage3Args* pb = (const Stage3Args*)(const void*)(kp + sizeof(Stage3Args));
-        apply_mfma_body<K, true, true>(*pa, *pb, (int)blockIdx.x, (int)gridDim.x);
+        apply_mfma_body<K, true, true, SKIPZ>(*pa, *pb, (int)blockIdx.x, (int)gridDim.x);
     } else if (K >= 12) {
-        apply_mfma_body<K, true>(a, a, (int)blockIdx.x, (int)gridDim.x);
+        apply_mfma_body<K, true, false, SKIPZ>(a, a, (int)blockIdx.x, (int)gridDim.x);
         __syncthreads();
-        apply_mfma_body<K, true>(b, b, (int)blockIdx.x, (int)gridDim.x);
+        apply_mfma_body<K, true, false, SKIPZ>(b, b, (int)blockIdx.x, (int)gridDim.x);
     } else if ((int)blockIdx.x < grid_a) {
-        apply_mfma_body<K, true>(a, a, (int)blockIdx.x, grid_a);
+        apply_mfma_body<K, true, false, SKIPZ>(a, a, (int)blockIdx.x, grid_a);
     } else {
-        apply_mfma_body<K, true>(b, b, (int)blockIdx.x - grid_a, (int)gridDim.x - grid_a);
+        apply_mfma_body<K, true, false, SKIPZ>(b, b, (int)blockIdx.x - grid_a, (int)gridDim.x - grid_a);
     }
 }
 
@@ -379,33 +487,6 @@
 }
 __device__ __forceinline__ unsigned tile_offset3(const DevStage& st, unsigned local) { return st.dlo[local & 63u] | st.dhi[local >> 6]; }
 template <int K> struct SweepShape : TileShape<K, true> {};
-__device__ __forceinline__ unsigned elem_bit(const DevStage& st, long long e, unsigned local_pos) {
-    const unsigned m = local_pos < 6 ? st.dlo[1u << local_pos] : st.dhi[1u << (local_pos - 6)];
-    return ((unsigned long long)e & m) ? 1u : 0u;
-}
-template <int GPW, int NW>
-__device__ __forceinline__ void skip_masks(const DevStage& st, unsigned info, long long e0, long long e1, int wave, unsigned& nzmask, unsigned& kneed) {
-    nzmask = 0; kneed = 0;
-    const unsigned gfresh = info & 15u, kfresh = (info >> 6) & 3u;
-#pragma unroll
-    for (int k = 0; k < 2; ++k) {
-        const long long e = k ? e1 : e0;
-        if (e < 0) continue;
-        unsigned gb = 0;
-#pragma unroll
-        for (int i = 0; i < 4; ++i)
-            if (gfresh >> i & 1) gb |= elem_bit(st, e, (info >> (8 + 4 * i)) & 15u) << i;
-        unsigned kb = 0;
-        if (kfresh & 1) kb |= elem_bit(st, e, (info >> 24) & 15u);
-        if (kfresh & 2) kb |= elem_bit(st, e, (info >> 28) & 15u) << 1;
-#pragma unroll
-        for (int j = 0; j < GPW; ++j)
-            if ((((unsigned)(wave + j * NW) ^ gb) & gfresh) == 0) nzmask |= 1u << j;
-#pragma unroll
-        for (unsigned s2 = 0; s2 < 4; ++s2)
-            if (((s2 ^ kb) & kfresh) == 0) kneed |= 1u << s2;
-    }
-}
 template <int K, bool LIST, bool SKIPW, bool RLAST>
 __device__ __forceinline__ void sweep_mfma_body(const Stage3Args& a, const int wg, const int nwg) {
     using TS = TileShape<K, true>;
@@ -997,13 +1078,15 @@
 }
 using Stage3Kernel = void (*)(Stage3Args);
 using Pair3Kernel = void (*)(Stage3Args, Stage3Args, int);
-template <int K> static Stage3Kernel apply_variant(bool list) { return list ? apply_mfma_kernel<K, true> : apply_mfma_kernel<K, false>; }
+template <int K> static Stage3Kernel apply_variant(bool list, bool skipz) {
+    return list ? (skipz ? apply_mfma_kernel<K, true, true> : apply_mfma_kernel<K, true, false>) : apply_mfma_kernel<K, false, false>;
+}
 template <int K> static Stage3Kernel sweep_variant(bool list, bool skipw, bool rlast) {
     if (list) return rlast ? sweep_mfma_kernel<K, true, false, true> : sweep_mfma_kernel<K, true, false, false>;
     if (skipw) return sweep_mfma_kernel<K, false, true, false>;
     return rlast ? sweep_mfma_kernel<K, false, false, true> : sweep_mfma_kernel<K, false, false, false>;
 }
-template <int K> static Pair3Kernel apply_pair_variant() { return apply_pair_kernel<K>; }
+template <int K> static Pair3Kernel apply_pair_variant(bool skipz) { return skipz ? apply_pair_kernel<K, true> : apply_pair_kernel<K, false>; }
 template <int K> static Pair3Kernel sweep_pair_variant(bool rlast_a) { return rlast_a ? sweep_pair_kernel<K, true, false> : sweep_pair_kernel<K, false, false>; }
 
 template <typename F>
@@ -1015,8 +1098,9 @@
     for (int k = 8; k <= 12 && e == hipSuccess; ++k)
         e = with_tile_size(k, [](auto kk) {
             constexpr int K = decltype(kk)::value;
-            hipError_t e = big_lds(apply_pair_variant<K>());
-            for (int f = 0; f < 2 && e == hipSuccess; ++f) e = big_lds(apply_variant<K>(f));
+            hipError_t e = hipSuccess;
+            for (int f = 0; f < 2 && e == hipSuccess; ++f) e = big_lds(apply_pair_variant<K>(f));
+            for (int f = 0; f < 4 && e == hipSuccess; ++f) e = big_lds(apply_variant<K>(f & 1, f & 2));
             for (int f = 0; f < 2 && e == hipSuccess; ++f) e = big_lds(sweep_pair_variant<K>(f));
             for (int f = 0; f < 8 && e == hipSuccess; ++f) e = big_lds(sweep_variant<K>(f & 1, f & 2, f & 4));
             return e;
@@ -1033,7 +1117,7 @@
     const hipError_t e = with_tile_size(k, [&](auto kk) {
         constexpr int K = decltype(kk)::value;
         return sweep ? hipOccupancyMaxActiveBlocksPerMultiprocessor(&n, sweep_variant<K>(false, false, false), mfma_threads(k, true), sweep3_lds_bytes(k))
-                     : hipOccupancyMaxActiveBlocksPerMultiprocessor(&n, apply_variant<K>(false), mfma_threads(k, false), apply3_lds_bytes(k));
+                     : hipOccupancyMaxActiveBlocksPerMultiprocessor(&n, apply_variant<K>(false, false), mfma_threads(k, false), apply3_lds_bytes(k));
     });
     return e == hipSuccess ? n : -1;
 }
@@ -1063,7 +1147,7 @@
     const long nwork = list ? (long)a.max_items : (long)a.ntiles * a.batch;
     const dim3 grid = (k >= 12 && persist > 0 && a.stage.nsubs > 0) ? dim3((unsigned)std::min<long>(nwork, persist * persistent_sweep_grid(sw.sweep_grid)))
                                                                      : ((k >= 12 || list) ? dim3((unsigned)nwork) : dim3(a.ntiles, a.batch));
-    return with_tile_size(k, [&](auto kk) { return launch3(apply_variant<decltype(kk)::value>(list), grid, k, false, s, a); });
+    return with_tile_size(k, [&](auto kk) { return launch3(apply_variant<decltype(kk)::value>(list, list && a.supp != nullptr), grid, k, false, s, a); });
 }
 static_assert(2 * sizeof(Stage3Args) + 16 <= 3840, "two argument blocks must fit the kernel-argument segment");
 hipError_t launch_apply3_pair(int k, hipStream_t s, const Stage3Args& a, const Stage3Args& b, const Switches& sw) {
@@ -1071,7 +1155,7 @@
     if (!stage3_launchable(k, a, true, true) || !stage3_launchable(k, b, true, true) || (k >= 12 && persist <= 0)) return hipErrorInvalidValue;
     const long longer = std::max(a.max_items, b.max_items);
     const dim3 grid((unsigned)(k >= 12 ? std::min<long>(longer, persist * persistent_sweep_grid(sw.sweep_grid)) : (long)a.max_items + b.max_items));
-    return with_tile_size(k, [&](auto kk) { return launch3(apply_pair_variant<decltype(kk)::value>(), grid, k, false, s, a, b, a.max_items); });
+    return with_tile_size(k, [&](auto kk) { return launch3(apply_pair_variant<decltype(kk)::value>(a.supp || b.supp), grid, k, false, s, a, b, a.max_items); });
 }
 int sweep3_chunk(int ntiles, int batch, int k, long sweep_grid) {
     if (k < 12) return 0;
diff --git a/aqc_research_amd/csrc/aqc_launch.h b/aqc_research_amd/csrc/aqc_launch.h
--- a/aqc_research_amd/csrc/aqc_launch.h
+++ b/aqc_research_amd/csrc/aqc_launch.h
@@ -69,6 +69,7 @@
     int store_out;
     int r_only_last;
     const long long* supp;
+    int pattern;
     const TileItem* items;
     const int* nitems;
     int max_items;
diff --git a/aqc_research_amd/csrc/aqc_skip_rule.h b/aqc_research_amd/csrc/aqc_skip_rule.h
--- /dev/null
+++ b/aqc_research_amd/csrc/aqc_skip_rule.h
@@ -0,0 +1,120 @@
+#pragma once
+#include <cstdint>
+
+#include "aqc_device.h"
+
+#if defined(__HIPCC__)
+#define AQC_SKIP_FN __host__ __device__ __forceinline__
+#define AQC_SKIP_UNROLL _Pragma("unroll")
+#else
+#define AQC_SKIP_FN inline
+#define AQC_SKIP_UNROLL
+#endif
+
+namespace aqc {
+
+template <class Fresh>
+inline uint32_t skip_info(const int* reg, int nreg, const int* cbits, int nc, Fresh fresh) {
+    uint32_t info = 0;
+    for (int i = 0; i < 4 && 4 + i < nc; ++i) {
+        if (fresh(cbits[4 + i])) info |= 1u << i;
+        info |= (uint32_t)cbits[4 + i] << (8 + 4 * i);
+    }
+    for (int i = 0; i < nreg && i < 4; ++i)
+        if (fresh(reg[i])) info |= 1u << (4 + i);
+    if (nreg == 4) info |= (uint32_t)reg[2] << 24 | (uint32_t)reg[3] << 28;
+    else info &= ~0xC0u;
+    return info;
+}
+AQC_SKIP_FN bool skip_info_sheds(uint32_t info) { return (info & 0xCFu) != 0; }
+
+AQC_SKIP_FN unsigned elem_bit(const DevStage& st, long long e, unsigned local_pos) {
+    const unsigned m = local_pos < 6 ? st.dlo[1u << local_pos] : st.dhi[1u << (local_pos - 6)];
+    return ((unsigned long long)e & m) ? 1u : 0u;
+}
+template <int GPW, int NW, class Bit>
+AQC_SKIP_FN void skip_masks_by(Bit bit, unsigned info, long long e0, long long e1, int wave, unsigned& nzmask, unsigned& kneed) {
+    nzmask = 0; kneed = 0;
+    const unsigned gfresh = info & 15u, kfresh = (info >> 6) & 3u;
+AQC_SKIP_UNROLL
+    for (int k = 0; k < 2; ++k) {
+        const long long e = k ? e1 : e0;
+        if (e < 0) continue;
+        unsigned gb = 0;
+AQC_SKIP_UNROLL
+        for (int i = 0; i < 4; ++i)
+            if (gfresh >> i & 1) gb |= bit(e, (info >> (8 + 4 * i)) & 15u) << i;
+        unsigned kb = 0;
+        if (kfresh & 1) kb |= bit(e, (info >> 24) & 15u);
+        if (kfresh & 2) kb |= bit(e, (info >> 28) & 15u) << 1;
+AQC_SKIP_UNROLL
+        for (int j = 0; j < GPW; ++j)
+            if ((((unsigned)(wave + j * NW) ^ gb) & gfresh) == 0) nzmask |= 1u << j;
+AQC_SKIP_UNROLL
+        for (unsigned s2 = 0; s2 < 4; ++s2)
+            if (((s2 ^ kb) & kfresh) == 0) kneed |= 1u << s2;
+    }
+}
+template <int GPW, int NW>
+AQC_SKIP_FN void skip_masks(const DevStage& st, unsigned info, long long e0, long long e1, int wave, unsigned& nzmask, unsigned& kneed) {
+    skip_masks_by<GPW, NW>([&st](long long e, unsigned pos) { return elem_bit(st, e, pos); }, info, e0, e1, wave, nzmask, kneed);
+}
+AQC_SKIP_FN long long local_index(const DevStage& st, long long e) {
+    if (e < 0) return -1;
+    long long l = 0;
+    for (unsigned pos = 0; pos < (unsigned)st.k; ++pos) l |= (long long)elem_bit(st, e, pos) << pos;
+    return l;
+}
+template <int GPW, int NW>
+AQC_SKIP_FN void skip_masks_local(unsigned info, long long l0, long long l1, int wave, unsigned& nzmask, unsigned& kneed) {
+    skip_masks_by<GPW, NW>([](long long l, unsigned pos) { return (unsigned)(l >> pos) & 1u; }, info, l0, l1, wave, nzmask, kneed);
+}
+
+enum { kVskipFree = 0, kVskipElem = 1, kVskipGroup = 2 };
+template <class Fresh>
+inline uint64_t vskip_info(const int* reg, int nreg, const int* cbits, int nc, const int* local_qubit, int t, const int* tbits, const bool* in_l0,
+                           Fresh fresh) {
+    uint64_t out = 0;
+    auto constraint = [&](int local_pos) -> unsigned {
+        if (!fresh(local_pos)) return kVskipFree << 6;
+        const int q = local_qubit[local_pos];
+        if (q >= t) return kVskipFree << 6;
+        if (!in_l0[q]) return (unsigned)kVskipElem << 6 | (unsigned)tbits[q];
+        int spectator = t;
+        for (int r = 0; r < q; ++r) spectator += in_l0[r];
+        for (int i = 0; i < 4 && 4 + i < nc; ++i)
+            if (local_qubit[cbits[4 + i]] == spectator) return (unsigned)kVskipGroup << 6 | (unsigned)i;
+        return kVskipFree << 6;
+    };
+    for (int i = 0; i < 4 && 4 + i < nc; ++i) out |= (uint64_t)constraint(cbits[4 + i]) << (8 * i);
+    if (nreg == 4) out |= (uint64_t)constraint(reg[2]) << 32 | (uint64_t)constraint(reg[3]) << 40;
+    return out;
+}
+template <int GPW, int NW>
+AQC_SKIP_FN void vskip_masks(uint64_t vinfo, long long e, int wave, unsigned& nzmask, unsigned (&kneed)[GPW]) {
+    nzmask = 0;
+AQC_SKIP_UNROLL
+    for (int j = 0; j < GPW; ++j) {
+        const unsigned g = (unsigned)(wave + j * NW);
+        bool nz = true;
+        unsigned need = 15u;
+AQC_SKIP_UNROLL
+        for (int p = 0; p < 6; ++p) {
+            const unsigned c = (unsigned)(vinfo >> (8 * p)) & 255u, kind = c >> 6, arg = c & 63u;
+            if (kind == kVskipFree) continue;
+            const unsigned want = kind == kVskipElem ? (unsigned)((unsigned long long)e >> arg & 1u) : (g >> arg & 1u);
+            if (p < 4) nz = nz && ((g >> p & 1u) == want);
+            else {
+AQC_SKIP_UNROLL
+                for (unsigned s = 0; s < 4; ++s)
+                    if ((s >> (p - 4) & 1u) != want) need &= ~(1u << s);
+            }
+        }
+        if (nz) nzmask |= 1u << j;
+        kneed[j] = nz ? need : 0u;
+    }
+}
+
+inline int skip_tile_waves(int k) { return k >= 10 ? 4 : 1 << (k - 8); }
+
+}
diff --git a/aqc_research_amd/csrc/aqc_ws.h b/aqc_research_amd/csrc/aqc_ws.h
--- a/aqc_research_amd/csrc/aqc_ws.h
+++ b/aqc_research_amd/csrc/aqc_ws.h
@@ -118,6 +118,7 @@
 };
 
 void lower_plan(const Program& prog, const Plan& plan, HostPlan& out, int reg_bits, bool with_dots, bool mfma = false, bool presplit = false, int beam_width = 64);
+void sub3_tables(DevSub3& d3, const int* reg, const std::vector<int>& cbits);
 int upload_plan(DevPlan& p);
 Plan mirror_plan(const Plan& plan);
 
diff --git a/aqc_research_amd/csrc/aqc_ws_plan.cpp b/aqc_research_amd/csrc/aqc_ws_plan.cpp
--- a/aqc_research_amd/csrc/aqc_ws_plan.cpp
+++ b/aqc_research_amd/csrc/aqc_ws_plan.cpp
@@ -1,4 +1,5 @@
 #include "aqc_ws.h"
+#include "aqc_skip_rule.h"
 
 #include <algorithm>
 
@@ -72,6 +73,29 @@
     }
 }
 
+}
+
+void sub3_tables(DevSub3& d3, const int* reg, const std::vector<int>& cbits) {
+    auto deposit = [](unsigned v, const int* bits, int nb) {
+        unsigned o = 0;
+        for (int j = 0; j < nb; ++j)
+            if (v >> j & 1) o |= 1u << bits[j];
+        return o;
+    };
+    const int nc = (int)cbits.size();
+    for (unsigned v = 0; v < 16; ++v) {
+        d3.dep_a[v] = (uint16_t)swz3_host(deposit(v, reg, 4));
+        d3.dep_clo[v] = (uint16_t)swz3_host(deposit(v, cbits.data(), std::min(nc, 4)));
+    }
+    for (unsigned g = 0; g < 64; ++g)
+        d3.dep_chi[g] = nc > 4 && g < (1u << (nc - 4)) ? (uint16_t)swz3_host(deposit(g, cbits.data() + 4, nc - 4)) : 0;
+    for (unsigned l = 0; l < 64; ++l)
+        d3.lane12[l] = (uint32_t)(d3.dep_clo[l & 15] ^ d3.dep_a[l >> 4]) | ((uint32_t)(d3.dep_a[l & 15] ^ d3.dep_clo[l >> 4]) << 16);
+    for (unsigned g = 0; g < 16; ++g)
+        for (unsigned s = 0; s < 4; ++s) {
+            d3.kk[g][s] = (uint32_t)(d3.dep_a[4 * s] ^ d3.dep_chi[g]) << 4;
+            d3.kk[g][4 + s] = (uint32_t)(d3.dep_clo[4 * s] ^ d3.dep_chi[g]) << 4;
+        }
 }
 
 void lower_plan(const Program& prog, const Plan& plan, HostPlan& out, int reg_bits, bool with_dots, bool mfma, bool presplit, int beam_width) {
@@ -169,38 +193,11 @@
                     for (int j = 0; j < ds.k; ++j)
                         if (reg_of[j] < 0) cbits.push_back(j);
                     for (int j = 0; j < 4; ++j) d3.bits[j] = dsub.bits[j];
-                    auto deposit = [](unsigned v, const int* bits, int nb) {
-                        unsigned o = 0;
-                        for (int j = 0; j < nb; ++j)
-                            if (v >> j & 1) o |= 1u << bits[j];
-                        return o;
-                    };
                     const int nc = (int)cbits.size();
-                    for (unsigned v = 0; v < 16; ++v) {
-                        d3.dep_a[v] = (uint16_t)swz3_host(deposit(v, dsub.bits, 4));
-                        d3.dep_clo[v] = (uint16_t)swz3_host(deposit(v, cbits.data(), std::min(nc, 4)));
-                    }
-                    for (unsigned g = 0; g < 64; ++g)
-                        d3.dep_chi[g] = nc > 4 && g < (1u << (nc - 4)) ? (uint16_t)swz3_host(deposit(g, cbits.data() + 4, nc - 4)) : 0;
-                    for (unsigned l = 0; l < 64; ++l)
-                        d3.lane12[l] = (uint32_t)(d3.dep_clo[l & 15] ^ d3.dep_a[l >> 4]) | ((uint32_t)(d3.dep_a[l & 15] ^ d3.dep_clo[l >> 4]) << 16);
-                    for (unsigned g = 0; g < 16; ++g)
-                        for (unsigned s = 0; s < 4; ++s) {
-                            d3.kk[g][s] = (uint32_t)(d3.dep_a[4 * s] ^ d3.dep_chi[g]) << 4;
-                            d3.kk[g][4 + s] = (uint32_t)(d3.dep_clo[4 * s] ^ d3.dep_chi[g]) << 4;
-                        }
+                    auto fresh = [&](int local_pos) { return !(touched_global >> st.bits[local_pos] & 1) && !(touched_local >> local_pos & 1); };
+                    sub3_tables(d3, dsub.bits, cbits);
                     {
-                        auto fresh = [&](int local_pos) { return !(touched_global >> st.bits[local_pos] & 1) && !(touched_local >> local_pos & 1); };
-                        uint32_t info = 0;
-                        for (int i = 0; i < 4 && 4 + i < nc; ++i) {
-                            if (fresh(cbits[4 + i])) info |= 1u << i;
-                            info |= (uint32_t)cbits[4 + i] << (8 + 4 * i);
-                        }
-                        for (int i = 0; i < dsub.nbits && i < 4; ++i)
-                            if (fresh(dsub.bits[i])) info |= 1u << (4 + i);
-                        if (dsub.nbits == 4) info |= (uint32_t)dsub.bits[2] << 24 | (uint32_t)dsub.bits[3] << 28;
-                        else info &= ~0xC0u;
-                        d3.skipinfo = info;
+                        d3.skipinfo = skip_info(dsub.bits, dsub.nbits, cbits.data(), nc, fresh);
                         for (int i = 0; i < dsub.nbits; ++i) touched_local |= 1u << dsub.bits[i];
                     }
                     out.h_subs3.push_back(d3);
diff --git a/aqc_research_amd/csrc/aqc_ws_project.cpp b/aqc_research_amd/csrc/aqc_ws_project.cpp
--- a/aqc_research_amd/csrc/aqc_ws_project.cpp
+++ b/aqc_research_amd/csrc/aqc_ws_project.cpp
@@ -1,4 +1,5 @@
 #include "aqc_ws.h"
+#include "aqc_skip_rule.h"
 
 #include <algorithm>
 
@@ -66,6 +67,33 @@
     if (!pr.vsw.v3 || !check_plan(pr.vprog, pr.vsw.plan, &pr.rest).empty()) return;
     lower_plan(pr.vprog, mirror_plan(pr.vsw.plan), pr.vinv, 4, false, true, true);
     if (!pr.vinv.v3 || pr.vinv.h_subs3.size() != pr.vsw.h_subs3.size()) return;
+    {
+        const Stage& st0 = pr.vsw.plan.stages[0];
+        const DevStage& ds0 = pr.vsw.h_stages[0];
+        bool in_l0[32];
+        for (int q = 0; q < pr.t; ++q) in_l0[q] = (Cb >> tbits[q] & 1) != 0;
+        uint32_t touched_local = 0;
+        for (int i = 0; i < ds0.nsubs; ++i) {
+            DevSub3& d3 = pr.vsw.h_subs3[ds0.sub_begin + i];
+            const std::vector<int>& reg = st0.subs[i].bits;
+            std::vector<int> cb;
+            for (int j = 0; j < ds0.k; ++j)
+                if (std::find(reg.begin(), reg.end(), j) == reg.end()) cb.push_back(j);
+            auto fresh = [&](int local_pos) { return !(touched_local >> local_pos & 1); };
+            auto constrained = [&](int pos) {
+                const int q = st0.bits[pos];
+                return fresh(pos) && q < pr.t;
+            };
+            if (ws->sw.skip_zero_w > 0 && cb.size() > 4 && std::any_of(cb.begin() + 4, cb.end(), constrained)) {
+                std::stable_partition(cb.begin() + 4, cb.end(), [&](int pos) { return !constrained(pos); });
+                sub3_tables(d3, reg.data(), cb);
+            }
+            const uint64_t vinfo = vskip_info(reg.data(), (int)reg.size(), cb.data(), (int)cb.size(), st0.bits.data(), pr.t, tbits.data(), in_l0, fresh);
+            d3.pad3[0] = (uint32_t)vinfo;
+            d3.pad3[1] = (uint32_t)(vinfo >> 32);
+            for (size_t j = 0; j < st0.subs[i].bits.size(); ++j) touched_local |= 1u << st0.subs[i].bits[j];
+        }
+    }
     for (DevPlan* q : {&pr.vsw, &pr.vinv})
         for (DevStage& ds : q->h_stages) {
             if (ds.nub >= 32) return;
@@ -255,11 +283,12 @@
     return true;
 }
 
-struct VirtualRun { const DevPlan& plan; const double2* src; double2* dst; };
+struct VirtualRun { const DevPlan& plan; const double2* src; double2* dst; const long long* pattern_of; };
 static Stage3Args virtual_apply_stage(aqc_ws* ws, const VirtualRun& v, size_t s) {
     Stage3Args a = virtual_stage3_args(ws, v.plan, s);
     a.in0 = s == 0 ? v.src : v.dst;
     a.out0 = v.dst;
+    if (s == 0 && v.pattern_of) { a.supp = v.pattern_of; a.pattern = 1; }
     return a;
 }
 static int enqueue_couple(aqc_ws* ws, int k, const Stage3Args* real, const VirtualRun* v) {
@@ -289,12 +318,14 @@
     psi.in0 = ws->bufs[x_buf];
     psi.out0 = ws->bufs[AQC_BUF_W];
     stage3_first_list(ws, psi);
+    const long long* supp = ws->sw.skip_zero_w > 0 && ws->combo_valid[x_buf] ? (const long long*)ws->d_combo_prev[x_buf] : nullptr;
+    psi.supp = supp;
     Stage3Args last = stage3_args(ws, iv, iv.h_stages.size() - 1);
     last.in0 = ws->bufs[AQC_BUF_ZW];
     last.out0 = ws->bufs[AQC_BUF_Z];
     stage3_first_list(ws, last);
-    const VirtualRun mend{pr.vsw, pr.vm, pr.vme};
-    const VirtualRun y0{pr.vinv, pr.vy, pr.vy};
+    const VirtualRun mend{pr.vsw, pr.vm, pr.vme, supp};
+    const VirtualRun y0{pr.vinv, pr.vy, pr.vy, nullptr};
     const ProjArgs a = proj_args(ws);
     const bool pairs = projected_pairs(ws);
 
diff --git a/aqc_research_amd/engine.py b/aqc_research_amd/engine.py
--- a/aqc_research_amd/engine.py
+++ b/aqc_research_amd/engine.py
@@ -81,6 +81,16 @@
         return {"virtual_qubits": int(c[1]), "touched_qubits": int(c[2]), "shared_with_first_stage": int(c[3]), "stages": int(c[4]),
                 "substages": int(c[5]), "tile_bits": int(c[6]), "substages_on_the_register": int(c[7]), "summed_bits": int(c[8]),
                 "padded_qubits": int(c[9]), "substages_per_stage": [int(c[10 + i]) for i in range(min(int(c[4]), 6))]}
+
+    def plan_skip_masks(self, vlist: int, elem: int, tile_bits: int = 0, low_bits: int = -1) -> dict:
+        head, local = (ctypes.c_int32 * 8)(), (ctypes.c_int32 * 16)()
+        layout, masks = (ctypes.c_int32 * (12 * 16))(), (ctypes.c_int32 * (16 * 16))()
+        check(_lib.lib().aqc_plan_skip_masks(self.handle, tile_bits, low_bits, vlist, int(elem), head, local, layout, masks, 16))
+        ns, k = int(head[0]), int(head[1])
+        return {"tile_bits": k, "waves": int(head[2]), "touched_qubits": int(head[3]), "spectators": int(head[4]), "tiles": int(head[5]),
+                "local_bits": [int(local[j]) for j in range(k)],
+                "layout": [[int(layout[12 * i + j]) for j in range(12)] for i in range(ns)],
+                "masks": [[int(masks[16 * i + g]) for g in range(1 << (k - 8))] for i in range(ns)]}
 
     def plan(self, which: int = 1, ncols: int = 1, tile_bits: int = 0, low_bits: int = -1):
         L = _lib.lib()
diff --git a/include/aqc_hip.h b/include/aqc_hip.h
--- a/include/aqc_hip.h
+++ b/include/aqc_hip.h
@@ -171,6 +171,8 @@
 int aqc_ws_sparse_counts(aqc_ws* ws, int64_t* counts);
 int aqc_ws_projected_info(aqc_ws* ws, int32_t* info);
 int aqc_plan_projected(aqc_ctx* ctx, int tile_bits, int low_bits, int32_t* info);
+int aqc_plan_skip_masks(aqc_ctx* ctx, int tile_bits, int low_bits, int list, long long elem, int32_t* head, int32_t* local_bits,
+                        int32_t* layout, int32_t* masks, int max_subs);
 int aqc_switch_info(int index, const char** name, const char** dflt, const char** when, const char** reader, const char** doc);
 int aqc_ws_switch(const aqc_ws* ws, const char* name, int64_t* value);
 int aqc_ws_plan_info(aqc_ws* ws, int which ,
```

Result: slower. 1.188 million evals/s (-1.2%).
